# Pyrokine/LineSegmentDetector-SLAM

Measured on AMD Instinct MI355X. Metric: Mpixels/sec LSD (grad+grow+NFA), higher is better.
Workload: dtype f64; 1 GPU; 512 x 2048x2048 u8 occupancy maps per GPU tiled/rolled/flipped from 4 aisle-class fixtures (SURVEY 8d C4), full pipeline incl. lineIm, params 0.3/0.6/22.5/0.7/1024; images_total=512, images_rank0=512, parallelism=single GPU, rccl_gather_in_step=False, steps_in_flight=8, steps_in_flight_asked=8, region_waves_per_image=4, help_across_workgroups=False, last_steps_with_help=0, writeback_map=False

## Files before the change

### include/lsd_hip.h

```cpp
#ifndef LSD_HIP_H
#define LSD_HIP_H
#include <stddef.h>
#include <stdint.h>

#ifdef __cplusplus
extern "C" {
#endif

#define LSD_ABI_VERSION 1

enum {
    LSD_OK = 0,
    LSD_ERR_INVALID = 1,
    LSD_ERR_NO_DEVICE = 2,
    LSD_ERR_HIP = 3,
    LSD_ERR_UNSUPPORTED = 4,
    LSD_ERR_CAPACITY = 5,
    LSD_ERR_NOMEM = 6,
    LSD_ERR_INTERNAL = 7
};

typedef struct lsd_params {
    double sca;
    double sig;
    double angThre;
    double denThre;
    int pseBin;
} lsd_params;

typedef struct lsd_line {
    double k, b, dx, dy, x1, y1, x2, y2, len;
    int orient;
} lsd_line;

typedef struct lsd_ctx lsd_ctx;

int lsd_create(lsd_ctx **out, int device);
void lsd_destroy(lsd_ctx *ctx);
const char *lsd_strerror(int status);
const char *lsd_last_error(const lsd_ctx *ctx);
void lsd_default_params(lsd_params *p);
int lsd_abi_version(void);
void lsd_free(void *p);

int lsd_run(lsd_ctx *ctx, uint8_t *map, int cols, int rows, size_t stride, const lsd_params *p,
            uint8_t *line_im, size_t line_im_stride, lsd_line **lines_out, int *n_lines);

int lsd_run_batch(lsd_ctx *ctx, uint8_t *maps, int n, int cols, int rows, const lsd_params *p,
                  uint8_t *line_ims, lsd_line **lines_out, int *offsets_out);

int lsd_set_host_max_lines(lsd_ctx *ctx, int max_lines);

#define LSD_FLAG_WRITEBACK_MAP 1u
int lsd_enqueue_batch_device(lsd_ctx *ctx, uint8_t *d_maps, int n, int cols, int rows,
                             const lsd_params *p, unsigned flags, uint8_t *d_line_ims,
                             lsd_line *d_lines, int max_lines, int32_t *d_counts, void *stream);
int lsd_reserve(lsd_ctx *ctx, int n, int cols, int rows);
int lsd_synchronize(lsd_ctx *ctx);

void lsd_shard_range(int n_items, int world, int rank, int *lo, int *hi);
int lsd_shard_balanced(const long long *costs, int n_items, int world, int *perm);
int lsd_last_region_cycles(lsd_ctx *ctx, int n, long long *cycles_out);

int lsd_last_sensitivity(lsd_ctx *ctx, int n, int *near_ties);

typedef struct lsd_comm {
    int rank, world;
    int (*all_gather)(void *user, const void *d_send, void *d_recv, size_t bytes_per_rank, void *stream);
    void *user;
} lsd_comm;
int lsd_comm_from_rccl(void *nccl_comm, lsd_comm *out);

int lsd_gather_layout(int n_total, int world, int *per_rank, size_t *counts_words);

int lsd_gather_lines(lsd_ctx *ctx, const lsd_comm *comm, const lsd_line *d_lines, const int32_t *d_counts, int n_local, int max_lines,
                     int n_total, int cap_rows, int32_t *d_counts_all, lsd_line *d_slabs_all, void *stream);
int lsd_gather_unpack(const int32_t *counts_all, const lsd_line *slabs_all, int n_total, int world, int cap_rows, int32_t *offsets_out,
                      lsd_line *lines_out, size_t lines_cap);

int lsd_map_cache(lsd_ctx *ctx, const uint8_t *map, int cols, int rows, size_t stride, double res,
                  double z_occ_max_dis, double *out);
int lsd_enqueue_map_cache_device(lsd_ctx *ctx, const uint8_t *d_maps, int n, int cols, int rows, double res,
                                 double z_occ_max_dis, double *d_out, void *stream);

typedef struct lsd_position { double x, y, ang; } lsd_position;
typedef struct lsd_match_score { lsd_position pos; double score; } lsd_match_score;
int lsd_scan_to_map_match(lsd_ctx *ctx, const double *map_cache, int cols, int rows,
                          const lsd_line *map_lines, int n_map, const lsd_line *scan_lines, int n_scan,
                          const lsd_position *scan_im_points, int n_points, lsd_position lidar_pose, lsd_position last_pose,
                          const int *pairs, int n_pairs, double z_occ_max_dis, double max_esti_dist, lsd_match_score *out);
int lsd_enqueue_scan_to_map_match_device(lsd_ctx *ctx, const double *d_map_cache, int cols, int rows,
                                         const lsd_line *d_map_lines, const lsd_line *d_scan_lines,
                                         const lsd_position *d_scan_im_points, int n_points, lsd_position lidar_pose,
                                         lsd_position last_pose, const int *d_pairs, int n_pairs, double z_occ_max_dis,
                                         double max_esti_dist, lsd_match_score *d_out, void *stream);

typedef struct lsd_polar { double range, angle; } lsd_polar;
typedef struct lsd_map_param { int oriMapCol, oriMapRow; double mapResol, mapOriX, mapOriY; } lsd_map_param;
#define LSD_RDP_MAX_LINES 360
int lsd_feature_scan_batch(lsd_ctx *ctx, const lsd_polar *scans, const int *lens, int n_scans, int stride, lsd_map_param map_param,
                           int region_point_limit, double thre_line, double line_dist_thre_m, lsd_line *lines_out, int *n_lines,
                           lsd_position *pts_out, int pts_cap, int *n_pts, double *lidar_pos, int *im_size);
int lsd_enqueue_feature_scan_batch_device(lsd_ctx *ctx, const lsd_polar *d_scans, const int *d_lens, int n_scans, int stride,
                                          lsd_map_param map_param, int region_point_limit, double thre_line, double line_dist_thre_m,
                                          lsd_line *d_lines_out, int *d_n_lines, lsd_position *d_pts_out, int pts_cap, int *d_n_pts,
                                          double *d_lidar_pos, int *d_im_size, void *stream);

int lsd_enqueue_scan_ingest_device(lsd_ctx *ctx, const lsd_polar *d_raw, int n_scans, int n_beams, const int *d_take,
                                   lsd_polar *d_scans, int *d_lens, int stride, void *stream);
int lsd_enqueue_laserscan_ingest_device(lsd_ctx *ctx, const float *d_ranges, const float *d_angle_min_inc, int n_scans, int n_beams,
                                        const int *d_take, lsd_polar *d_scans, int *d_lens, int stride, void *stream);

typedef struct lsd_fa_state {
    double x[9];
    double P[81];
} lsd_fa_state;
enum { LSD_FA_RESET = 0, LSD_FA_FIRST = 1, LSD_FA_UKF = 2 };
typedef struct lsd_fa_report {
    lsd_position estimate;
    double score;
    lsd_position scan_pose;
    int n_pairs;
    int n_kept;
    int branch;
    int llt;
} lsd_fa_report;
void lsd_fa_initial_state(lsd_fa_state *out);
int lsd_feature_association(lsd_ctx *ctx, const double *map_cache, int cols, int rows, const lsd_line *map_lines, int n_map,
                            const lsd_line *scan_lines, int n_scan, const lsd_position *scan_im_points, int n_points,
                            lsd_position lidar_pose, lsd_position last_pose, lsd_position scan_pose, const lsd_fa_state *in,
                            lsd_fa_state *out, lsd_fa_report *report);
int lsd_enqueue_localize_device(lsd_ctx *ctx, const double *d_map_cache, int cols, int rows, const lsd_line *d_map_lines, int n_map,
                                int n_seq, int frames_pitch, const int *n_frames, const lsd_line *d_lines, const int *d_n_lines,
                                const lsd_position *d_pts, int pts_cap, const int *d_n_pts, const double *d_lidar_pos,
                                const lsd_position *d_odom, double map_resol, const lsd_fa_state *d_init, lsd_fa_state *d_states,
                                lsd_fa_report *d_reports, void *stream);
typedef struct lsd_fa_carry {
    lsd_fa_state state;
    lsd_position odom;
    double ang_sum;
    double ang_count;
    int32_t frames;
    int32_t is_offset;
} lsd_fa_carry;
void lsd_fa_carry_init(lsd_fa_carry *out, const lsd_fa_state *state, lsd_position odom0);
int lsd_enqueue_localize_resume_device(lsd_ctx *ctx, const double *d_map_cache, int cols, int rows, const lsd_line *d_map_lines,
                                       int n_map, int n_seq, int frames_pitch, const int *n_frames, const lsd_line *d_lines,
                                       const int *d_n_lines, const lsd_position *d_pts, int pts_cap, const int *d_n_pts,
                                       const double *d_lidar_pos, const lsd_position *d_odom, double map_resol, lsd_fa_carry *d_carry,
                                       lsd_fa_state *d_states, lsd_fa_report *d_reports, void *stream);
int lsd_enqueue_localize_live_map_device(lsd_ctx *ctx, const double *d_map_cache, int cols, int rows, const lsd_line *d_map_lines,
                                         int map_lines_cap, const int32_t *d_n_map, int n_seq, int frames_pitch, const int *n_frames,
                                         const lsd_line *d_lines, const int *d_n_lines, const lsd_position *d_pts, int pts_cap,
                                         const int *d_n_pts, const double *d_lidar_pos, const lsd_position *d_odom, double map_resol,
                                         const lsd_fa_state *d_init, lsd_fa_state *d_states, lsd_fa_report *d_reports, void *stream);
int lsd_enqueue_localize_resume_live_map_device(lsd_ctx *ctx, const double *d_map_cache, int cols, int rows, const lsd_line *d_map_lines,
                                                int map_lines_cap, const int32_t *d_n_map, int n_seq, int frames_pitch, const int *n_frames,
                                                const lsd_line *d_lines, const int *d_n_lines, const lsd_position *d_pts, int pts_cap,
                                                const int *d_n_pts, const double *d_lidar_pos, const lsd_position *d_odom, double map_resol,
                                                lsd_fa_carry *d_carry, lsd_fa_state *d_states, lsd_fa_report *d_reports, void *stream);
#define LSD_MAX_MAPS 64
typedef struct lsd_map_ref {
    const double   *d_map_cache;
    const lsd_line *d_map_lines;
    const int32_t  *d_n_map;
    int cols, rows, n_map;
    double mapResol, mapOriX, mapOriY;
} lsd_map_ref;
int lsd_enqueue_feature_scan_maps_device(lsd_ctx *ctx, const lsd_polar *d_scans, const int *d_lens, int n_scans, int stride,
                                         const lsd_map_ref *maps, int n_maps, const int32_t *d_map_of, int scans_per_seq,
                                         int region_point_limit, double thre_line, double line_dist_thre_m, lsd_line *d_lines_out,
                                         int *d_n_lines, lsd_position *d_pts_out, int pts_cap, int *d_n_pts, double *d_lidar_pos,
                                         int *d_im_size, void *stream);
int lsd_enqueue_localize_maps_device(lsd_ctx *ctx, const lsd_map_ref *maps, int n_maps, const int32_t *d_map_of, int n_seq,
                                     int frames_pitch, const int *n_frames, const lsd_line *d_lines, const int *d_n_lines,
                                     const lsd_position *d_pts, int pts_cap, const int *d_n_pts, const double *d_lidar_pos,
                                     const lsd_position *d_odom, const lsd_fa_state *d_init, lsd_fa_state *d_states,
                                     lsd_fa_report *d_reports, void *stream);
int lsd_enqueue_localize_resume_maps_device(lsd_ctx *ctx, const lsd_map_ref *maps, int n_maps, const int32_t *d_map_of, int n_seq,
                                            int frames_pitch, const int *n_frames, const lsd_line *d_lines, const int *d_n_lines,
                                            const lsd_position *d_pts, int pts_cap, const int *d_n_pts, const double *d_lidar_pos,
                                            const lsd_position *d_odom, lsd_fa_carry *d_carry, lsd_fa_state *d_states,
                                            lsd_fa_report *d_reports, void *stream);
typedef struct lsd_map_frame { double mapResol, mapOriX, mapOriY; } lsd_map_frame;
int lsd_enqueue_fa_carry_rebase_device(lsd_ctx *ctx, lsd_fa_carry *d_carry, int n_seq, const int32_t *d_key, int32_t key,
                                       lsd_map_frame from, lsd_map_frame to, void *stream);
int lsd_localize(lsd_ctx *ctx, const double *map_cache, int cols, int rows, const lsd_line *map_lines, int n_map, const lsd_polar *scans,
                 const int *lens, int n_frames, int stride, const lsd_position *odom, lsd_map_param map_param, const lsd_fa_state *init,
                 lsd_fa_state *states, lsd_fa_report *reports);
int lsd_debug_fa_fuse(lsd_ctx *ctx, const lsd_match_score *cands, int n, lsd_position last_pose, lsd_position scan_pose,
                      const lsd_fa_state *in, lsd_fa_state *out, lsd_fa_report *report);

int lsd_occupancy_to_map(lsd_ctx *ctx, const int8_t *grid, int cols, int rows, uint8_t *map_out, size_t map_stride);
int lsd_enqueue_occupancy_to_map_device(lsd_ctx *ctx, const int8_t *d_grid, size_t n_cells, uint8_t *d_map, void *stream);

int lsd_enqueue_map_update_device(lsd_ctx *ctx, const int8_t *d_grid, int cols, int rows, double res, double z_occ_max_dis,
                                  const lsd_params *p, uint8_t *d_map, double *d_map_cache, lsd_line *d_lines, int max_lines,
                                  int32_t *d_count, uint8_t *d_line_im, void *stream);
int lsd_reserve_map_update(lsd_ctx *ctx, int cols, int rows);

void lsd_scaled_size(int cols, int rows, double sca, int *w, int *h);

enum { LSD_STAGE_ALL = 0, LSD_STAGE_GAUSS = 1, LSD_STAGE_GRAD = 2, LSD_STAGE_SORT = 3, LSD_STAGE_REGION = 4 };
int lsd_set_stop_after(lsd_ctx *ctx, int stage);
int lsd_set_trace(lsd_ctx *ctx, int on);
int lsd_set_region_waves(lsd_ctx *ctx, int waves);
int lsd_set_region_help(lsd_ctx *ctx, int waves);
int lsd_set_cost_history(lsd_ctx *ctx, int on);
int lsd_debug_set_stamp_budget(lsd_ctx *ctx, unsigned grows);
int lsd_debug_set_tuning(lsd_ctx *ctx, const char *name, int value);

enum { LSD_DBG_GAUSS = 1, LSD_DBG_MAG, LSD_DBG_DEG, LSD_DBG_STATE, LSD_DBG_ORDER, LSD_DBG_ORDER_VAL,
       LSD_DBG_NB, LSD_DBG_MAXGRAD, LSD_DBG_RECS, LSD_DBG_SEEDS, LSD_DBG_NSEED, LSD_DBG_STATS };
int lsd_debug_fetch(lsd_ctx *ctx, int image, int what, void *out, size_t bytes);

int lsd_debug_eval_math(lsd_ctx *ctx, int fn, const double *a, const double *b, double *out0, double *out1, size_t n);

int lsd_debug_calibrate(lsd_ctx *ctx, size_t bytes);

int lsd_last_timings(lsd_ctx *ctx, float ms_out[6]);

#ifdef __cplusplus
}
#endif
#endif
```

### linesegmentdetector-slam_amd/__init__.py

```python
import ctypes as C
import os

import numpy as np

_HERE = os.path.dirname(os.path.abspath(__file__))
LIB_PATH = os.path.join(_HERE, "liblsdhip.so")

LSD_OK, LSD_ERR_INVALID, LSD_ERR_NO_DEVICE, LSD_ERR_HIP, LSD_ERR_UNSUPPORTED, LSD_ERR_CAPACITY, LSD_ERR_NOMEM, LSD_ERR_INTERNAL = range(8)
LSD_FLAG_WRITEBACK_MAP = 1
STAGE_ALL, STAGE_GAUSS, STAGE_GRAD, STAGE_SORT, STAGE_REGION = range(5)
(DBG_GAUSS, DBG_MAG, DBG_DEG, DBG_STATE, DBG_ORDER, DBG_ORDER_VAL, DBG_NB, DBG_MAXGRAD, DBG_RECS, DBG_SEEDS,
 DBG_NSEED, DBG_STATS) = range(1, 13)

lsd_sca, lsd_sig, lsd_angThre, lsd_denThre, pseBin = 0.3, 0.6, 22.5, 0.7, 1024
z_occ_max_dis = 1.0
rdp_leastPoint, rdp_threLine, rdp_leastDist = 3, 0.08, 0.5


class lsd_params(C.Structure):
    _fields_ = [("sca", C.c_double), ("sig", C.c_double), ("angThre", C.c_double), ("denThre", C.c_double),
                ("pseBin", C.c_int)]


class lsd_line(C.Structure):
    _fields_ = [(n, C.c_double) for n in ("k", "b", "dx", "dy", "x1", "y1", "x2", "y2", "len")] + [("orient", C.c_int)]


LINE_DTYPE = np.dtype([("k", "f8"), ("b", "f8"), ("dx", "f8"), ("dy", "f8"), ("x1", "f8"), ("y1", "f8"),
                       ("x2", "f8"), ("y2", "f8"), ("len", "f8"), ("orient", "i4"), ("_pad", "i4")])
SEED_DTYPE = np.dtype([("order_idx", "i4"), ("x", "i4"), ("y", "i4"), ("num", "i4"), ("outcome", "i4"),
                       ("final_num", "i4"), ("logNFA", "f8")])
assert LINE_DTYPE.itemsize == 80 == C.sizeof(lsd_line)


class lsd_map_param(C.Structure):
    _fields_ = [("oriMapCol", C.c_int), ("oriMapRow", C.c_int), ("mapResol", C.c_double), ("mapOriX", C.c_double), ("mapOriY", C.c_double)]


LSD_MAX_MAPS = 64


class lsd_map_ref(C.Structure):
    _fields_ = [("d_map_cache", C.c_void_p), ("d_map_lines", C.c_void_p), ("d_n_map", C.c_void_p), ("cols", C.c_int), ("rows", C.c_int),
                ("n_map", C.c_int), ("mapResol", C.c_double), ("mapOriX", C.c_double), ("mapOriY", C.c_double)]


MAP_REF_DTYPE = np.dtype([("d_map_cache", "u8"), ("d_map_lines", "u8"), ("d_n_map", "u8"), ("cols", "i4"), ("rows", "i4"), ("n_map", "i4"),
                          ("_pad", "i4"), ("mapResol", "f8"), ("mapOriX", "f8"), ("mapOriY", "f8")])
assert MAP_REF_DTYPE.itemsize == 64 == C.sizeof(lsd_map_ref)


class lsd_map_frame(C.Structure):
    _fields_ = [("mapResol", C.c_double), ("mapOriX", C.c_double), ("mapOriY", C.c_double)]


class lsd_position(C.Structure):
    _fields_ = [("x", C.c_double), ("y", C.c_double), ("ang", C.c_double)]


POS_DTYPE = np.dtype([("x", "f8"), ("y", "f8"), ("ang", "f8")])
SCORE_DTYPE = np.dtype([("x", "f8"), ("y", "f8"), ("ang", "f8"), ("score", "f8")])

FA_STATE_DTYPE = np.dtype([("x", "f8", (9,)), ("P", "f8", (81,))])
FA_REPORT_DTYPE = np.dtype([("estimate", POS_DTYPE), ("score", "f8"), ("scan_pose", POS_DTYPE), ("n_pairs", "i4"), ("n_kept", "i4"),
                            ("branch", "i4"), ("llt", "i4")])
assert FA_STATE_DTYPE.itemsize == 720 and FA_REPORT_DTYPE.itemsize == 72
FA_RESET, FA_FIRST, FA_UKF = range(3)
FA_CARRY_DTYPE = np.dtype([("state", FA_STATE_DTYPE), ("odom", POS_DTYPE), ("ang_sum", "f8"), ("ang_count", "f8"), ("frames", "i4"),
                           ("is_offset", "i4")])
assert FA_CARRY_DTYPE.itemsize == 768


ALL_GATHER_FN = C.CFUNCTYPE(C.c_int, C.c_void_p, C.c_void_p, C.c_void_p, C.c_size_t, C.c_void_p)


class lsd_comm(C.Structure):
    _fields_ = [("rank", C.c_int), ("world", C.c_int), ("all_gather", ALL_GATHER_FN), ("user", C.c_void_p)]


class LsdError(RuntimeError):
    def __init__(self, status, msg, partial=None):
        super().__init__("lsd_hip status %d: %s" % (status, msg))
        self.status = status
        self.partial = partial


_vp, _i, _sz, _dbl = C.c_void_p, C.c_int, C.c_size_t, C.c_double
_pi, _ppar = C.POINTER(C.c_int), C.POINTER(lsd_params)
_localize_args = [_vp, _vp, _i, _i, _vp, _i, _i, _i, _vp, _vp, _vp, _vp, _i, _vp, _vp, _vp, _dbl, _vp, _vp, _vp, _vp]
_maps_args = [_vp, _vp, _i, _vp] + _localize_args[6:16] + _localize_args[17:]
_live_map_args = _localize_args[:6] + [_vp] + _localize_args[6:]
_ABI = {
    "lsd_create": (_i, [C.POINTER(_vp), _i]),
    "lsd_destroy": (None, [_vp]),
    "lsd_strerror": (C.c_char_p, [_i]),
    "lsd_last_error": (C.c_char_p, [_vp]),
    "lsd_default_params": (None, [_ppar]),
    "lsd_abi_version": (_i, []),
    "lsd_free": (None, [_vp]),
    "lsd_run": (_i, [_vp, _vp, _i, _i, _sz, _ppar, _vp, _sz, C.POINTER(_vp), _pi]),
    "lsd_run_batch": (_i, [_vp, _vp, _i, _i, _i, _ppar, _vp, C.POINTER(_vp), _pi]),
    "lsd_enqueue_batch_device": (_i, [_vp, _vp, _i, _i, _i, _ppar, C.c_uint, _vp, _vp, _i, _vp, _vp]),
    "lsd_reserve": (_i, [_vp, _i, _i, _i]),
    "lsd_synchronize": (_i, [_vp]),
    "lsd_scaled_size": (None, [_i, _i, _dbl, _pi, _pi]),
    "lsd_set_stop_after": (_i, [_vp, _i]),
    "lsd_set_trace": (_i, [_vp, _i]),
    "lsd_set_region_waves": (_i, [_vp, _i]),
    "lsd_set_region_help": (_i, [_vp, _i]),
    "lsd_debug_set_stamp_budget": (_i, [_vp, C.c_uint]),
    "lsd_set_cost_history": (_i, [_vp, _i]),
    "lsd_debug_set_tuning": (_i, [_vp, C.c_char_p, _i]),
    "lsd_set_host_max_lines": (_i, [_vp, _i]),
    "lsd_debug_fetch": (_i, [_vp, _i, _i, _vp, _sz]),
    "lsd_last_timings": (_i, [_vp, C.POINTER(C.c_float)]),
    "lsd_map_cache": (_i, [_vp, _vp, _i, _i, _sz, _dbl, _dbl, _vp]),
    "lsd_enqueue_map_cache_device": (_i, [_vp, _vp, _i, _i, _i, _dbl, _dbl, _vp, _vp]),
    "lsd_occupancy_to_map": (_i, [_vp, _vp, _i, _i, _vp, _sz]),
    "lsd_enqueue_occupancy_to_map_device": (_i, [_vp, _vp, _sz, _vp, _vp]),
    "lsd_scan_to_map_match": (_i, [_vp, _vp, _i, _i, _vp, _i, _vp, _i, _vp, _i, lsd_position, lsd_position, _vp, _i, _dbl, _dbl, _vp]),
    "lsd_enqueue_scan_to_map_match_device": (_i, [_vp, _vp, _i, _i, _vp, _vp, _vp, _i, lsd_position, lsd_position, _vp, _i, _dbl, _dbl, _vp, _vp]),
    "lsd_feature_scan_batch": (_i, [_vp, _vp, _vp, _i, _i, lsd_map_param, _i, _dbl, _dbl, _vp, _vp, _vp, _i, _vp, _vp, _vp]),
    "lsd_enqueue_feature_scan_batch_device": (_i, [_vp, _vp, _vp, _i, _i, lsd_map_param, _i, _dbl, _dbl, _vp, _vp, _vp, _i, _vp, _vp, _vp, _vp]),
    "lsd_shard_range": (None, [_i, _i, _i, _pi, _pi]),
    "lsd_gather_layout": (_i, [_i, _i, _pi, C.POINTER(_sz)]),
    "lsd_comm_from_rccl": (_i, [_vp, C.POINTER(lsd_comm)]),
    "lsd_gather_lines": (_i, [_vp, C.POINTER(lsd_comm), _vp, _vp, _i, _i, _i, _i, _vp, _vp, _vp]),
    "lsd_gather_unpack": (_i, [_vp, _vp, _i, _i, _i, _vp, _vp, _sz]),
    "lsd_shard_balanced": (_i, [_vp, _i, _i, _vp]),
    "lsd_last_region_cycles": (_i, [_vp, _i, _vp]),
    "lsd_last_sensitivity": (_i, [_vp, _i, _vp]),
    "lsd_fa_initial_state": (None, [_vp]),
    "lsd_feature_association": (_i, [_vp, _vp, _i, _i, _vp, _i, _vp, _i, _vp, _i, lsd_position, lsd_position, lsd_position, _vp, _vp, _vp]),
    "lsd_enqueue_localize_device": (_i, _localize_args),
    "lsd_localize": (_i, [_vp, _vp, _i, _i, _vp, _i, _vp, _vp, _i, _i, _vp, lsd_map_param, _vp, _vp, _vp]),
    "lsd_debug_fa_fuse": (_i, [_vp, _vp, _i, lsd_position, lsd_position, _vp, _vp, _vp]),
    "lsd_fa_carry_init": (None, [_vp, _vp, lsd_position]),
    "lsd_enqueue_localize_resume_device": (_i, _localize_args),
    "lsd_enqueue_localize_live_map_device": (_i, _live_map_args),
    "lsd_enqueue_localize_resume_live_map_device": (_i, _live_map_args),
    "lsd_enqueue_feature_scan_maps_device": (_i, [_vp, _vp, _vp, _i, _i, _vp, _i, _vp, _i, _i, _dbl, _dbl, _vp, _vp, _vp, _i, _vp, _vp, _vp, _vp]),
    "lsd_enqueue_localize_maps_device": (_i, _maps_args),
    "lsd_enqueue_localize_resume_maps_device": (_i, _maps_args),
    "lsd_enqueue_fa_carry_rebase_device": (_i, [_vp, _vp, _i, _vp, C.c_int32, lsd_map_frame, lsd_map_frame, _vp]),
    "lsd_enqueue_map_update_device": (_i, [_vp, _vp, _i, _i, _dbl, _dbl, _ppar, _vp, _vp, _vp, _i, _vp, _vp, _vp]),
    "lsd_reserve_map_update": (_i, [_vp, _i, _i]),
    "lsd_enqueue_scan_ingest_device": (_i, [_vp, _vp, _i, _i, _vp, _vp, _vp, _i, _vp]),
    "lsd_enqueue_laserscan_ingest_device": (_i, [_vp, _vp, _vp, _i, _i, _vp, _vp, _vp, _i, _vp]),
    "lsd_debug_calibrate": (_i, [_vp, _sz]),
    "lsd_debug_eval_math": (_i, [_vp, _i, _vp, _vp, _vp, _vp, _sz]),
}
EXPORTED_SYMBOLS = list(_ABI)
del _vp, _i, _sz, _dbl, _pi, _ppar, _localize_args, _live_map_args, _maps_args

_lib = None


def load_library(path=None):
    global _lib
    if _lib is not None and path is None:
        return _lib
    p = path or os.environ.get("LSD_HIP_LIB") or LIB_PATH
    try:
        import torch
    except ImportError:
        pass
    if not os.path.exists(p):
        raise ImportError("liblsdhip.so is not built (%s); run `python -c 'import __graft_entry__ as g; g.build()'` "
                          "-- there is no CPU fallback" % p)
    L = C.CDLL(p)
    for name, (restype, argtypes) in _ABI.items():
        try:
            fn = getattr(L, name)
        except AttributeError:
            if not os.environ.get("LSD_HIP_LIB"):
                raise
            continue
        fn.restype, fn.argtypes = restype, argtypes
    if path is None:
        _lib = L
    return L


def shard_range(n_items, world, rank):
    lo, hi = C.c_int(), C.c_int()
    load_library().lsd_shard_range(n_items, world, rank, C.byref(lo), C.byref(hi))
    return lo.value, hi.value


def shard_balanced(costs, world):
    c = np.ascontiguousarray(costs, np.int64)
    perm = np.zeros(len(c), np.int32)
    st = load_library().lsd_shard_balanced(c.ctypes.data, len(c), world, perm.ctypes.data)
    if st != LSD_OK:
        raise LsdError(st, load_library().lsd_strerror(st).decode())
    return perm


def gather_layout(n_total, world):
    per, words = C.c_int(), C.c_size_t()
    st = load_library().lsd_gather_layout(n_total, world, C.byref(per), C.byref(words))
    if st != LSD_OK:
        raise LsdError(st, load_library().lsd_strerror(st).decode())
    return per.value, words.value


def gather_unpack(counts_all, slabs_all, n_total, world, cap_rows):
    L = load_library()
    ca = np.ascontiguousarray(counts_all, np.int32)
    sl = np.ascontiguousarray(slabs_all).view(np.uint8).reshape(-1, 80)
    offs = np.zeros(n_total + 1, np.int32)
    per, _ = gather_layout(n_total, world)
    total = int(ca.reshape(world, per + 2)[:, :per].sum())
    lines = np.zeros(max(total, 1), LINE_DTYPE)
    st = L.lsd_gather_unpack(ca.ctypes.data, sl.ctypes.data, n_total, world, cap_rows, offs.ctypes.data, lines.ctypes.data, len(lines))
    if st in (LSD_ERR_CAPACITY, LSD_ERR_INTERNAL):
        raise LsdError(st, L.lsd_strerror(st).decode(), partial=(offs, lines[:offs[-1]]))
    if st != LSD_OK:
        raise LsdError(st, L.lsd_strerror(st).decode())
    return offs, lines[:offs[-1]]


def make_params(sca=lsd_sca, sig=lsd_sig, angThre=lsd_angThre, denThre=lsd_denThre, pseBin=pseBin):
    return lsd_params(float(sca), float(sig), float(angThre), float(denThre), int(pseBin))


def scaled_size(cols, rows, sca=lsd_sca):
    w, h = C.c_int(), C.c_int()
    load_library().lsd_scaled_size(cols, rows, sca, C.byref(w), C.byref(h))
    return w.value, h.value


class Context:

    def __init__(self, device=0):
        self.L = load_library()
        h = C.c_void_p()
        st = self.L.lsd_create(C.byref(h), int(device))
        if st != LSD_OK:
            raise LsdError(st, self.L.lsd_strerror(st).decode())
        self.h = h
        self.device = device

    def close(self):
        if getattr(self, "h", None):
            self.L.lsd_destroy(self.h)
            self.h = None

    def __del__(self):
        try:
            self.close()
        except Exception:
            pass

    def _chk(self, st, allow=()):
        if st != LSD_OK and st not in allow:
            raise LsdError(st, self.L.lsd_strerror(st).decode() + " / " + self.L.lsd_last_error(self.h).decode())
        return st

    def _take_lines(self, lines_p, n):
        lines = np.zeros(n if lines_p else 0, LINE_DTYPE)
        if len(lines):
            C.memmove(lines.ctypes.data, lines_p, 80 * len(lines))
            lines["_pad"] = 0
        self.L.lsd_free(lines_p)
        return lines

    def run(self, map_u8, params=None, want_lineim=True):
        assert map_u8.dtype == np.uint8 and map_u8.ndim == 2
        rows, cols = map_u8.shape
        p = params or make_params()
        line_im = np.zeros((rows, cols), np.uint8) if want_lineim else None
        lines_p, n = C.c_void_p(), C.c_int()
        st = self.L.lsd_run(self.h, map_u8.ctypes.data, cols, rows, map_u8.strides[0], C.byref(p),
                            line_im.ctypes.data if want_lineim else None, cols, C.byref(lines_p), C.byref(n))
        lines = self._take_lines(lines_p, n.value)
        self._chk(st)
        return lines, line_im

    def run_batch(self, maps_u8, params=None, want_lineim=True):
        assert maps_u8.dtype == np.uint8 and maps_u8.ndim == 3 and maps_u8.flags.c_contiguous
        n, rows, cols = maps_u8.shape
        p = params or make_params()
        line_ims = np.zeros((n, rows, cols), np.uint8) if want_lineim else None
        lines_p = C.c_void_p()
        offs = (C.c_int * (n + 1))()
        st = self.L.lsd_run_batch(self.h, maps_u8.ctypes.data, n, cols, rows, C.byref(p),
                                  line_ims.ctypes.data if want_lineim else None, C.byref(lines_p), offs)
        offsets = np.frombuffer(offs, np.int32).copy()
        lines = self._take_lines(lines_p, int(offsets[-1]))
        self._chk(st)
        return lines, offsets, line_ims

    def enqueue_device(self, d_maps, n, cols, rows, d_lines, max_lines, d_counts, d_line_ims=None, params=None,
                       flags=0, stream=None):
        p = params or make_params()
        return self._chk(self.L.lsd_enqueue_batch_device(self.h, d_maps, n, cols, rows, C.byref(p), flags, d_line_ims,
                                                         d_lines, max_lines, d_counts, stream))

    def gather_lines(self, comm, d_lines, d_counts, n_local, max_lines, n_total, cap_rows, d_counts_all, d_slabs_all, stream=None):
        return self._chk(self.L.lsd_gather_lines(self.h, C.byref(comm), d_lines, d_counts, n_local, max_lines, n_total, cap_rows,
                                                 d_counts_all, d_slabs_all, stream))

    def map_cache(self, map_u8, res, z_occ_max_dis=1.0):
        assert map_u8.dtype == np.uint8 and map_u8.ndim == 2
        rows, cols = map_u8.shape
        out = np.zeros((rows, cols), np.float64)
        self._chk(self.L.lsd_map_cache(self.h, map_u8.ctypes.data, cols, rows, map_u8.strides[0], float(res),
                                       float(z_occ_max_dis), out.ctypes.data))
        return out

    def enqueue_map_cache_device(self, d_maps, n, cols, rows, res, z_occ_max_dis, d_out, stream=None):
        return self._chk(self.L.lsd_enqueue_map_cache_device(self.h, d_maps, n, cols, rows, float(res),
                                                             float(z_occ_max_dis), d_out, stream))

    def scan_to_map_match(self, map_cache, map_lines, scan_lines, scan_im_points, lidar_pose, last_pose, pairs,
                          z_occ=1.0, max_esti_dist=60.0):
        mc = np.ascontiguousarray(map_cache, np.float64)
        rows, cols = mc.shape
        ml = np.ascontiguousarray(map_lines, LINE_DTYPE); sl = np.ascontiguousarray(scan_lines, LINE_DTYPE)
        pts = np.ascontiguousarray(scan_im_points).view(np.float64).reshape(-1, 3)
        pr = np.ascontiguousarray(pairs, np.int32).reshape(-1, 2)
        out = np.zeros((len(pr), 4), SCORE_DTYPE)
        self._chk(self.L.lsd_scan_to_map_match(self.h, mc.ctypes.data, cols, rows, ml.ctypes.data, len(ml), sl.ctypes.data, len(sl),
                                               pts.ctypes.data, len(pts), _pos(lidar_pose), _pos(last_pose), pr.ctypes.data, len(pr),
                                               float(z_occ), float(max_esti_dist), out.ctypes.data))
        return out

    def feature_scan_batch(self, scans, lens, map_param, region_point_limit=rdp_leastPoint, thre_line=rdp_threLine,
                           line_dist_thre_m=rdp_leastDist, pts_cap=4096):
        sc = np.ascontiguousarray(scans, np.float64)
        n, stride = sc.shape[0], sc.shape[1]
        ln = np.ascontiguousarray(lens, np.int32)
        lines = np.zeros((n, 360), LINE_DTYPE); pts = np.zeros((n, pts_cap, 3), np.float64)
        nl = np.zeros(n, np.int32); npt = np.zeros(n, np.int32); lp = np.zeros((n, 2), np.float64); sz = np.zeros((n, 2), np.int32)
        mp = _map_param(map_param)
        st = self.L.lsd_feature_scan_batch(self.h, sc.ctypes.data, ln.ctypes.data, n, stride, mp, int(region_point_limit), float(thre_line),
                                           float(line_dist_thre_m), lines.ctypes.data, nl.ctypes.data, pts.ctypes.data, pts_cap,
                                           npt.ctypes.data, lp.ctypes.data, sz.ctypes.data)
        if st != LSD_ERR_CAPACITY:
            self._chk(st)
        out = []
        for i in range(n):
            nl[i] = min(int(nl[i]), 360)
            if npt[i] > pts_cap:
                raise RuntimeError("scan %d marks %d pixels, more than pts_cap" % (i, npt[i]))
            p = pts[i, :npt[i]].copy()
            im = np.zeros((max(int(sz[i, 1]), 0), max(int(sz[i, 0]), 0)), np.uint8)
            if len(p):
                im[p[:, 1].astype(int), p[:, 0].astype(int)] = 255
            out.append(dict(linesInfo=lines[i, :nl[i]].copy(), len_linesInfo=int(nl[i]), scanImPoint=p, lidarPos=(float(lp[i, 0]), float(lp[i, 1])),
                            lineIm=im))
        if st == LSD_ERR_CAPACITY:
            raise LsdError(st, self.L.lsd_strerror(st).decode(), partial=out)
        return out

    def enqueue_scan_ingest_device(self, d_raw, n_scans, n_beams, d_take, d_scans, d_lens, stride, stream=None):
        return self._chk(self.L.lsd_enqueue_scan_ingest_device(self.h, d_raw, int(n_scans), int(n_beams), d_take, d_scans, d_lens, int(stride),
                                                               stream))

    def enqueue_laserscan_ingest_device(self, d_ranges, d_angle_min_inc, n_scans, n_beams, d_take, d_scans, d_lens, stride, stream=None):
        return self._chk(self.L.lsd_enqueue_laserscan_ingest_device(self.h, d_ranges, d_angle_min_inc, int(n_scans), int(n_beams), d_take,
                                                                    d_scans, d_lens, int(stride), stream))

    @staticmethod
    def fa_initial_state():
        st = np.zeros(1, FA_STATE_DTYPE)
        load_library().lsd_fa_initial_state(st.ctypes.data)
        return st[0]

    def feature_association(self, map_cache, map_lines, scan_lines, scan_im_points, lidar_pose, last_pose, scan_pose, state):
        mc = np.ascontiguousarray(map_cache, np.float64)
        rows, cols = mc.shape
        ml, sl = np.ascontiguousarray(map_lines, LINE_DTYPE), np.ascontiguousarray(scan_lines, LINE_DTYPE)
        pts = np.ascontiguousarray(scan_im_points, np.float64).reshape(-1, 3)
        st_in = fa_state(state)
        st_out = np.zeros(1, FA_STATE_DTYPE); rep = np.zeros(1, FA_REPORT_DTYPE)
        self._chk(self.L.lsd_feature_association(self.h, mc.ctypes.data, cols, rows, ml.ctypes.data, len(ml), sl.ctypes.data, len(sl),
                                                 pts.ctypes.data, len(pts), _pos(lidar_pose), _pos(last_pose), _pos(scan_pose),
                                                 st_in.ctypes.data, st_out.ctypes.data, rep.ctypes.data))
        return st_out[0], rep[0]

    def debug_fa_fuse(self, cands, last_pose, scan_pose, state):
        cd = np.ascontiguousarray(np.asarray(cands, np.float64).reshape(-1, 4))
        st_in = fa_state(state)
        st_out = np.zeros(1, FA_STATE_DTYPE); rep = np.zeros(1, FA_REPORT_DTYPE)
        self._chk(self.L.lsd_debug_fa_fuse(self.h, cd.ctypes.data, len(cd), _pos(last_pose), _pos(scan_pose), st_in.ctypes.data,
                                           st_out.ctypes.data, rep.ctypes.data))
        return st_out[0], rep[0]

    def localize(self, map_cache, map_lines, scans, lens, odom, map_param, init=None):
        mc = np.ascontiguousarray(map_cache, np.float64)
        rows, cols = mc.shape
        ml = np.ascontiguousarray(map_lines, LINE_DTYPE)
        sc = np.ascontiguousarray(scans, np.float64)
        n, stride = sc.shape[0], sc.shape[1]
        ln = np.ascontiguousarray(lens, np.int32)
        od = np.ascontiguousarray(odom, np.float64).reshape(-1, 3)
        if len(od) != n + 1:
            raise LsdError(LSD_ERR_INVALID, "odom must have one row more than there are frames")
        mp = _map_param(map_param)
        ini = None if init is None else fa_state(init)
        states = np.zeros(n, FA_STATE_DTYPE); reps = np.zeros(n, FA_REPORT_DTYPE)
        self._chk(self.L.lsd_localize(self.h, mc.ctypes.data, cols, rows, ml.ctypes.data, len(ml), sc.ctypes.data, ln.ctypes.data, n, stride,
                                      od.ctypes.data, mp, None if ini is None else ini.ctypes.data, states.ctypes.data, reps.ctypes.data))
        return states, reps

    def enqueue_localize_device(self, d_map_cache, cols, rows, d_map_lines, n_map, n_seq, frames_pitch, n_frames, d_lines, d_n_lines, d_pts,
                                pts_cap, d_n_pts, d_lidar_pos, d_odom, map_resol, d_init, d_states, d_reports, stream=None):
        nf = np.ascontiguousarray(n_frames, np.int32)
        return self._chk(self.L.lsd_enqueue_localize_device(self.h, d_map_cache, cols, rows, d_map_lines, n_map, n_seq, frames_pitch,
                                                            nf.ctypes.data, d_lines, d_n_lines, d_pts, pts_cap, d_n_pts, d_lidar_pos, d_odom,
                                                            float(map_resol), d_init, d_states, d_reports, stream))

    @staticmethod
    def fa_carry_init(state=None, odom0=(0.0, 0.0, 0.0)):
        c = np.zeros(1, FA_CARRY_DTYPE)
        st = None if state is None else fa_state(state)
        load_library().lsd_fa_carry_init(c.ctypes.data, None if st is None else st.ctypes.data, _pos(odom0))
        return c[0]

    def enqueue_localize_resume_device(self, d_map_cache, cols, rows, d_map_lines, n_map, n_seq, frames_pitch, n_frames, d_lines, d_n_lines,
                                       d_pts, pts_cap, d_n_pts, d_lidar_pos, d_odom, map_resol, d_carry, d_states, d_reports, stream=None):
        nf = np.ascontiguousarray(n_frames, np.int32)
        return self._chk(self.L.lsd_enqueue_localize_resume_device(self.h, d_map_cache, cols, rows, d_map_lines, n_map, n_seq, frames_pitch,
                                                                   nf.ctypes.data, d_lines, d_n_lines, d_pts, pts_cap, d_n_pts, d_lidar_pos,
                                                                   d_odom, float(map_resol), d_carry, d_states, d_reports, stream))

    def enqueue_localize_live_map_device(self, d_map_cache, cols, rows, d_map_lines, map_lines_cap, d_n_map, n_seq, frames_pitch, n_frames,
                                         d_lines, d_n_lines, d_pts, pts_cap, d_n_pts, d_lidar_pos, d_odom, map_resol, d_init, d_states,
                                         d_reports, stream=None):
        nf = np.ascontiguousarray(n_frames, np.int32)
        return self._chk(self.L.lsd_enqueue_localize_live_map_device(self.h, d_map_cache, cols, rows, d_map_lines, map_lines_cap, d_n_map,
                                                                     n_seq, frames_pitch, nf.ctypes.data, d_lines, d_n_lines, d_pts, pts_cap,
                                                                     d_n_pts, d_lidar_pos, d_odom, float(map_resol), d_init, d_states,
                                                                     d_reports, stream))

    def enqueue_localize_resume_live_map_device(self, d_map_cache, cols, rows, d_map_lines, map_lines_cap, d_n_map, n_seq, frames_pitch,
                                                n_frames, d_lines, d_n_lines, d_pts, pts_cap, d_n_pts, d_lidar_pos, d_odom, map_resol,
                                                d_carry, d_states, d_reports, stream=None):
        nf = np.ascontiguousarray(n_frames, np.int32)
        return self._chk(self.L.lsd_enqueue_localize_resume_live_map_device(self.h, d_map_cache, cols, rows, d_map_lines, map_lines_cap,
                                                                            d_n_map, n_seq, frames_pitch, nf.ctypes.data, d_lines, d_n_lines,
                                                                            d_pts, pts_cap, d_n_pts, d_lidar_pos, d_odom, float(map_resol),
                                                                            d_carry, d_states, d_reports, stream))

    def enqueue_feature_scan_maps_device(self, d_scans, d_lens, n_scans, stride, maps, d_map_of, scans_per_seq, d_lines_out, d_n_lines,
                                         d_pts_out, pts_cap, d_n_pts, d_lidar_pos, d_im_size, region_point_limit=rdp_leastPoint,
                                         thre_line=rdp_threLine, line_dist_thre_m=rdp_leastDist, stream=None):
        tab = map_table(maps)
        return self._chk(self.L.lsd_enqueue_feature_scan_maps_device(self.h, d_scans, d_lens, int(n_scans), int(stride), tab.ctypes.data,
                                                                     len(tab), d_map_of, int(scans_per_seq), int(region_point_limit),
                                                                     float(thre_line), float(line_dist_thre_m), d_lines_out, d_n_lines,
                                                                     d_pts_out, int(pts_cap), d_n_pts, d_lidar_pos, d_im_size, stream))

    def enqueue_localize_maps_device(self, maps, d_map_of, n_seq, frames_pitch, n_frames, d_lines, d_n_lines, d_pts, pts_cap, d_n_pts,
                                     d_lidar_pos, d_odom, d_init, d_states, d_reports, stream=None):
        tab, nf = map_table(maps), np.ascontiguousarray(n_frames, np.int32)
        return self._chk(self.L.lsd_enqueue_localize_maps_device(self.h, tab.ctypes.data, len(tab), d_map_of, int(n_seq), int(frames_pitch),
                                                                 nf.ctypes.data, d_lines, d_n_lines, d_pts, int(pts_cap), d_n_pts, d_lidar_pos,
                                                                 d_odom, d_init, d_states, d_reports, stream))

    def enqueue_localize_resume_maps_device(self, maps, d_map_of, n_seq, frames_pitch, n_frames, d_lines, d_n_lines, d_pts, pts_cap, d_n_pts,
                                            d_lidar_pos, d_odom, d_carry, d_states, d_reports, stream=None):
        tab, nf = map_table(maps), np.ascontiguousarray(n_frames, np.int32)
        return self._chk(self.L.lsd_enqueue_localize_resume_maps_device(self.h, tab.ctypes.data, len(tab), d_map_of, int(n_seq),
                                                                        int(frames_pitch), nf.ctypes.data, d_lines, d_n_lines, d_pts,
                                                                        int(pts_cap), d_n_pts, d_lidar_pos, d_odom, d_carry, d_states,
                                                                        d_reports, stream))

    def enqueue_fa_carry_rebase_device(self, d_carry, n_seq, d_key, key, frame_from, frame_to, stream=None):
        f, t = map_frame(frame_from), map_frame(frame_to)
        if not d_carry or int(n_seq) <= 0:
            raise LsdError(LSD_ERR_INVALID, "a null carry, or n_seq <= 0")
        return self._chk(self.L.lsd_enqueue_fa_carry_rebase_device(self.h, d_carry, int(n_seq), d_key, int(key), f, t, stream))

    def enqueue_map_update_device(self, d_grid, cols, rows, res, z_occ_max_dis, d_map, d_map_cache, d_lines, max_lines, d_count,
                                  d_line_im=None, params=None, stream=None):
        p = params or make_params()
        return self._chk(self.L.lsd_enqueue_map_update_device(self.h, d_grid, cols, rows, float(res), float(z_occ_max_dis), C.byref(p), d_map,
                                                              d_map_cache, d_lines, max_lines, d_count, d_line_im, stream))

    def reserve_map_update(self, cols, rows):
        self._chk(self.L.lsd_reserve_map_update(self.h, cols, rows))

    def occupancy_to_map(self, grid_i8):
        assert grid_i8.dtype == np.int8 and grid_i8.ndim == 2 and grid_i8.flags.c_contiguous
        rows, cols = grid_i8.shape
        out = np.zeros((rows, cols), np.uint8)
        self._chk(self.L.lsd_occupancy_to_map(self.h, grid_i8.ctypes.data, cols, rows, out.ctypes.data, out.strides[0]))
        return out

    def enqueue_occupancy_to_map_device(self, d_grid, n_cells, d_map, stream=None):
        return self._chk(self.L.lsd_enqueue_occupancy_to_map_device(self.h, d_grid, n_cells, d_map, stream))

    def reserve(self, n, cols, rows):
        self._chk(self.L.lsd_reserve(self.h, n, cols, rows))

    def synchronize(self):
        self._chk(self.L.lsd_synchronize(self.h))

    def fetch_stats_block(self, n):
        a = np.zeros((n, 48), np.int64)
        self._chk(self.L.lsd_debug_fetch(self.h, 0, DBG_STATS, a.ctypes.data, a.nbytes))
        return a

    def last_region_cycles(self, n):
        a = np.zeros(n, np.int64)
        self._chk(self.L.lsd_last_region_cycles(self.h, n, a.ctypes.data))
        return a

    def last_sensitivity(self, n):
        a = np.zeros(n, np.int32)
        self._chk(self.L.lsd_last_sensitivity(self.h, n, a.ctypes.data))
        return a

    def timings(self):
        ms = (C.c_float * 6)()
        self._chk(self.L.lsd_last_timings(self.h, ms))
        return dict(zip(("gauss", "gradient", "sort", "region", "lines", "total"), [float(x) for x in ms]))

    def set_stop_after(self, stage):
        self._chk(self.L.lsd_set_stop_after(self.h, stage))

    def set_trace(self, on):
        self._chk(self.L.lsd_set_trace(self.h, 1 if on else 0))

    def set_host_max_lines(self, max_lines):
        self._chk(self.L.lsd_set_host_max_lines(self.h, max_lines))

    def set_cost_history(self, on):
        self._chk(self.L.lsd_set_cost_history(self.h, 1 if on else 0))

    def debug_set_tuning(self, name, value):
        self._chk(self.L.lsd_debug_set_tuning(self.h, name.encode(), int(value)))

    def debug_set_stamp_budget(self, grows):
        self._chk(self.L.lsd_debug_set_stamp_budget(self.h, grows))

    def set_region_waves(self, waves):
        self._chk(self.L.lsd_set_region_waves(self.h, waves))

    def set_region_help(self, waves):
        self._chk(self.L.lsd_set_region_help(self.h, waves))

    def fetch(self, image, what, shape_wh):
        w, h = shape_wh
        npx = w * h

        def get(kind, dtype, count):
            a = np.zeros(max(count, 1), dtype)
            self._chk(self.L.lsd_debug_fetch(self.h, image, kind, a.ctypes.data, a.nbytes))
            return a[:count]

        if what in (DBG_GAUSS, DBG_MAG, DBG_DEG):
            return get(what, np.float64, npx).reshape(h, w)
        if what == DBG_STATE:
            return get(what, np.uint32, npx).reshape(h, w)
        if what == DBG_NB:
            return int(get(what, np.int32, 1)[0])
        if what == DBG_NSEED:
            return int(get(what, np.int32, 1)[0])
        if what == DBG_MAXGRAD:
            return float(get(what, np.float64, 1)[0])
        if what == DBG_ORDER:
            return get(what, np.uint32, npx)[:self.fetch(image, DBG_NB, shape_wh)]
        if what == DBG_ORDER_VAL:
            return get(what, np.uint16, npx)[:self.fetch(image, DBG_NB, shape_wh)]
        if what == DBG_STATS:
            v = get(what, np.int64, 48)
            d = dict(zip(("grow_calls", "grown_px", "nfa_calls", "rrr_calls", "rrr_passes", "rrr_sentinel_drops",
                          "rrr_oob_reads", "cycles_refill", "cycles_total", "cycles_grow", "cycles_rect",
                          "cycles_nfa", "cycles_mark", "small_bails", "wait_noslot", "seeds", "exact_angle_evals",
                          "tile_fetches", "batches", "cycles_tiles", "spec_redos", "spec_discards", "cycles_wait", "small_steps",
                          "refill_rounds", "cycles_eval", "cycles_sums", "cycles_refine", "cycles_small", "cycles_select", "cycles_commit",
                          "wait_noseed", "requeued_ahead", "cycles_eval_at_cursor", "depth_end", "nfa_min_abs_enc", "nfa_min_gap_enc", "help_exports", "help_evals", "near_ties",
                          "wd_commit", "wd_next", "wd_nseeds", "wd_state", "wd_nbig", "wd_lock", "wd_pend", "wd_wave"),
                         [int(x) for x in v]))
            d["set_answers"], d["sets_founded"] = int(v[41]), int(v[42])
            d["cycles_nfa_count"], d["nfa_tail_iters"] = int(v[43]), int(v[44])
            d["nfa_bracket_misses"] = int(v[40])
            for k in ("nfa_min_abs", "nfa_min_gap"):
                enc = d.pop(k + "_enc")
                d[k] = float("inf") if enc == 0 else float(np.array([0x7ff0000000000000 - enc], np.uint64).view(np.float64)[0])
            return d
        if what == DBG_SEEDS:
            ns = self.fetch(image, DBG_NSEED, shape_wh)
            return get(what, SEED_DTYPE, ns)
        raise ValueError(what)

    def eval_math(self, fn, a, b=None):
        a = np.ascontiguousarray(a, np.float64)
        b = None if b is None else np.ascontiguousarray(b, np.float64)
        o0, o1 = np.zeros_like(a), np.zeros_like(a)
        self._chk(self.L.lsd_debug_eval_math(self.h, fn, a.ctypes.data, None if b is None else b.ctypes.data,
                                             o0.ctypes.data, o1.ctypes.data, a.size))
        return o0, o1

    def fetch_recs(self, image, count):
        a = np.zeros(max(count * 12, 1), np.float64)
        self._chk(self.L.lsd_debug_fetch(self.h, image, DBG_RECS, a.ctypes.data, a.nbytes))
        return a[:count * 12].reshape(count, 12)


class structLSD:

    def __init__(self, lineIm, linesInfo):
        self.lineIm = lineIm
        self.linesInfo = linesInfo
        self.len_linesInfo = len(linesInfo)


_default_ctx = None


def default_context():
    global _default_ctx
    if _default_ctx is None:
        _default_ctx = Context(0)
    return _default_ctx


def myLineSegmentDetector(MapGray, oriMapCol, oriMapRow, sca, sig, angThre, denThre, pseBin, ctx=None):
    if MapGray.shape != (oriMapRow, oriMapCol):
        raise LsdError(LSD_ERR_INVALID, "MapGray must be oriMapRow x oriMapCol")
    ctx = ctx or default_context()
    lines, line_im = ctx.run(MapGray, make_params(sca, sig, angThre, denThre, pseBin))
    return structLSD(line_im, lines)


def createMapCache(MapGray, res, ctx=None):
    return (ctx or default_context()).map_cache(MapGray, res, z_occ_max_dis)


ignoreScanLength, scanToMapDiff, maxEstiDist = 40, 0.35, 60


def match_pairs(map_lines, scan_lines):
    pairs = []
    for cs in range(len(scan_lines)):
        ls = float(scan_lines["len"][cs])
        if ls < ignoreScanLength:
            continue
        ld = ls * scanToMapDiff
        for cm in range(len(map_lines)):
            lm = float(map_lines["len"][cm])
            if lm < ls - ld or lm > ls + ld:
                continue
            pairs.append((cm, cs))
    return np.array(pairs, np.int32).reshape(-1, 2)


def FeatureScan(mapParam, lidarPointPolar, RegionPointLimitNumber=rdp_leastPoint, threLine=rdp_threLine, lineDistThreM=rdp_leastDist, ctx=None):
    own = ctx is None
    ctx = ctx or Context(0)
    try:
        sc = np.ascontiguousarray(lidarPointPolar, np.float64).reshape(1, -1, 2)
        return ctx.feature_scan_batch(sc, [sc.shape[1]], mapParam, RegionPointLimitNumber, threLine, lineDistThreM)[0]
    finally:
        if own:
            ctx.close()


def ScanToMapMatch(mapCache, mapLinesInfo, scanLinesInfo, scanImPoint, lidarPose, lastPose, ctx=None):
    pairs = match_pairs(mapLinesInfo, scanLinesInfo)
    if len(pairs) == 0:
        return np.zeros(0, SCORE_DTYPE)
    sc = (ctx or default_context()).scan_to_map_match(mapCache, mapLinesInfo, scanLinesInfo, scanImPoint, lidarPose, lastPose, pairs,
                                                      z_occ_max_dis, maxEstiDist).ravel()
    keep = sc[sc["score"] < 3]
    return keep[np.argsort(keep["score"], kind="stable")]


def _pos(p):
    return lsd_position(float(p[0]), float(p[1]), float(p[2]) if len(p) > 2 else 0.0)


def _map_param(mp):
    return lsd_map_param(int(mp[0]), int(mp[1]), float(mp[2]), float(mp[3]), float(mp[4]))


def map_frame(frame):
    if isinstance(frame, lsd_map_frame):
        v = (frame.mapResol, frame.mapOriX, frame.mapOriY)
    else:
        v = tuple(float(x) for x in frame)
        if len(v) == 5:
            v = v[2:]
    if len(v) != 3:
        raise LsdError(LSD_ERR_INVALID, "a map frame is (mapResol, mapOriX, mapOriY)")
    if not (np.isfinite(v[0]) and v[0] > 0 and np.isfinite(v[1]) and np.isfinite(v[2])):
        raise LsdError(LSD_ERR_INVALID, "a map frame needs a finite mapResol > 0 and a finite origin, not %r" % (v,))
    return lsd_map_frame(*v)


def map_ref(d_map_cache, cols, rows, d_map_lines, n_map, map_param, d_n_map=0):
    r = np.zeros(1, MAP_REF_DTYPE)[0]
    r["d_map_cache"], r["d_map_lines"], r["d_n_map"] = int(d_map_cache or 0), int(d_map_lines or 0), int(d_n_map or 0)
    r["cols"], r["rows"], r["n_map"] = int(cols), int(rows), int(n_map)
    r["mapResol"], r["mapOriX"], r["mapOriY"] = float(map_param[2]), float(map_param[3]), float(map_param[4])
    return r


def map_table(maps):
    if isinstance(maps, np.ndarray) and maps.dtype == MAP_REF_DTYPE:
        return np.ascontiguousarray(maps).reshape(-1)
    return np.array(list(maps), MAP_REF_DTYPE).reshape(-1)


def fa_state(state):
    if isinstance(state, np.void) or (isinstance(state, np.ndarray) and state.dtype == FA_STATE_DTYPE):
        return np.ascontiguousarray(np.asarray(state, FA_STATE_DTYPE).reshape(1))
    x, P = state
    st = np.zeros(1, FA_STATE_DTYPE)
    st["x"][0] = np.asarray(x, np.float64).reshape(9)
    st["P"][0] = np.asarray(P, np.float64).reshape(9, 9).ravel(order="F")
    return st


def load_odom(path_or_rows):
    rows = np.loadtxt(path_or_rows).reshape(-1, 3) if isinstance(path_or_rows, str) else np.asarray(path_or_rows, np.float64).reshape(-1, 3)
    od = np.concatenate([rows, rows[-1:]], 0)
    od[0, 0] = 0.0
    return od


def lidar_frames(lidar):
    lid = np.asarray(lidar, np.float64)
    scans = np.zeros_like(lid)
    lens = np.zeros(len(lid), np.int32)
    for f in range(len(lid)):
        keep = lid[f][lid[f, :, 0] != np.inf]
        scans[f, :len(keep)] = keep
        lens[f] = len(keep)
    return scans, lens


def FeatureAssociation(mapCache, mapLinesInfo, scanLinesInfo, scanImPoint, lidarPose, lastPose, kalman_x, kalman_P, ScanPose, ctx=None):
    st, rep = (ctx or default_context()).feature_association(mapCache, mapLinesInfo, scanLinesInfo, scanImPoint, lidarPose, lastPose, ScanPose,
                                                             (kalman_x, kalman_P))
    return st["x"].copy(), st["P"].reshape(9, 9, order="F").copy(), rep


def replay_log(map_u8, map_param, lidar, odom, ctx=None):
    cx = ctx or default_context()
    m = np.ascontiguousarray(map_u8, np.uint8).copy()
    mapCache = cx.map_cache(m, float(map_param[2]), z_occ_max_dis)
    LSD = myLineSegmentDetector(m, m.shape[1], m.shape[0], lsd_sca, lsd_sig, lsd_angThre, lsd_denThre, pseBin, ctx=cx)
    scans, lens = lidar_frames(lidar)
    return cx.localize(mapCache, LSD.linesInfo, scans, lens, odom, map_param)


def lidar_frames_batch(lidar):
    lid = np.asarray(lidar, np.float64)
    keep = lid[..., 0] != np.inf
    order = np.argsort(~keep, axis=-1, kind="stable")
    scans = np.take_along_axis(lid, order[..., None], axis=-2)
    lens = keep.sum(-1).astype(np.int32)
    scans[np.arange(lid.shape[-2]) >= lens[..., None]] = 0.0
    return scans, lens


def _cuda_stream(stream):
    import torch
    if stream is None:
        return torch.cuda.current_stream()
    if not isinstance(stream, torch.cuda.Stream):
        raise LsdError(LSD_ERR_INVALID, "stream must be a torch.cuda.Stream (or None: the current stream)")
    return stream


def _occupancy_grid(d_grid, cols, rows, device):
    import torch
    if not isinstance(d_grid, torch.Tensor) or not d_grid.is_cuda or d_grid.dtype != torch.int8:
        raise LsdError(LSD_ERR_INVALID, "d_grid must be a CUDA int8 tensor")
    if d_grid.device.index != int(device):
        raise LsdError(LSD_ERR_INVALID, "d_grid is on cuda:%d, the context on device %d" % (d_grid.device.index, int(device)))
    if cols <= 0 or rows <= 0 or tuple(d_grid.shape) not in ((rows * cols,), (rows, cols)):
        raise LsdError(LSD_ERR_INVALID, "d_grid must hold oriMapRow x oriMapCol cells, flat or [rows, cols]")
    return d_grid.contiguous()


class _MapSlot:

    def __init__(self):
        self.cells = self.cap_lines = 0
        self.map = self.mc = self.lines = self.count = None
        self.cols = self.rows = 0
        self.lines_cap = 0
        self.n_host = None
        self.map_param = None
        self.grid = None
        self.ready = None
        self.waited = set()
        self.last_stream = None
        self.idle = None


class _MapPair:

    def __init__(self):
        self.slots, self.cur = (_MapSlot(), _MapSlot()), 1

    @property
    def current(self):
        return self.slots[self.cur]

    @staticmethod
    def fit(slot, cells, n_lines, keep=False):
        import torch
        if slot.cells >= cells and slot.cap_lines >= n_lines:
            return
        for ev in (slot.idle, slot.ready):
            if ev is not None:
                ev.synchronize()
        if slot.last_stream is not None:
            slot.last_stream.synchronize()
        cells, n_lines = max(cells, slot.cells), max(n_lines, slot.cap_lines)
        z = lambda count, dt: torch.zeros(count, dtype=dt, device="cuda")
        new = (z(cells, torch.uint8), z(cells, torch.float64), z(n_lines * 80, torch.uint8), z(1, torch.int32))
        if keep and slot.cells:
            for dst, src in zip(new, (slot.map, slot.mc, slot.lines, slot.count)):
                dst[:src.numel()].copy_(src)
        torch.cuda.current_stream().synchronize()
        slot.map, slot.mc, slot.lines, slot.count = new
        slot.cells, slot.cap_lines = cells, n_lines

    def target(self, stream, cells, n_lines):
        slot = self.slots[1 - self.cur]
# ... 577 lines not shown
```

### linesegmentdetector-slam_amd/csrc/k_gauss.hip

```cpp
#include "lsd_internal.h"
#include "k1_lds.h"
#include <algorithm>

namespace lsdhip {

constexpr int TW = kK1TileW, TH = kK1TileH, NT = 256;

__device__ __forceinline__ int reflect_idx(int j, int lim) {
    const int dou = 2 * lim;
    while (j < 0) j += dou;
    while (j >= dou) j -= dou;
    if (j >= lim) j = dou - j - 1;
    return j;
}


template <int HS>
__global__ __launch_bounds__(NT) void k_gauss(const uint8_t* __restrict__ in, double* __restrict__ out,
                                              const double* __restrict__ taps_g, const int* __restrict__ centre_of, int W, int H, int w, int h, int gp,
                                              int tapR, int IWp, int IHmax, unsigned gx, unsigned gy, unsigned tiles,
                                              uint8_t* __restrict__ clr) {
    extern __shared__ __align__(16) unsigned char smem[];
    const int hSize = HS > 0 ? HS : 2 * tapR + 1;
    double* aux = reinterpret_cast<double*>(smem);
    double* taps = aux + (size_t)IHmax * TW;
    uint8_t* tile = reinterpret_cast<uint8_t*>(taps + 3 * hSize);

    const int tid = threadIdx.x;
    const unsigned per = (tiles + 7u) >> 3;
    const unsigned t = (blockIdx.x & 7u) * per + (blockIdx.x >> 3);
    if (t >= tiles) return;
    const unsigned bx = t % gx, tq = t / gx, by = tq % gy;
    const int X0 = (int)bx * TW, Y0 = (int)by * TH;
    const size_t img = tq / gy;
    const uint8_t* src = in + img * (size_t)W * H;
    double* dst = out + img * (size_t)gp * h;

    if (clr) {
        typedef uint32_t u32x4 __attribute__((ext_vector_type(4)));
        const unsigned tpi = gx * gy, ti = t % tpi;
        const size_t units = ((size_t)W * H) >> 4;
        const size_t a = units * ti / tpi, e = units * (ti + 1) / tpi;
        u32x4* const v = reinterpret_cast<u32x4*>(clr + img * (size_t)W * H);
        const u32x4 z = {0u, 0u, 0u, 0u};
        for (size_t u = a + tid; u < e; u += NT) __builtin_nontemporal_store(z, &v[u]);
    }
    const int Xl = min(X0 + TW - 1, w - 1), Yl = min(Y0 + TH - 1, h - 1);
    const int c0 = centre_of[X0] - tapR, c1 = centre_of[Xl] + tapR;
    const int r0 = centre_of[Y0] - tapR, r1 = centre_of[Yl] + tapR;
    const int IH = r1 - r0 + 1;

    for (int i = tid; i < 3 * hSize; i += NT) taps[i] = taps_g[i];

    const int a0 = c0 - (((c0 % 4) + 4) % 4);
    auto remap4 = [](uint32_t x, uint32_t keep) -> uint32_t {
        uint32_t t1 = x ^ 0x01010101u, t2 = ~x;
        t1 = ~(((t1 & 0x7f7f7f7fu) + 0x7f7f7f7fu) | t1 | 0x7f7f7f7fu);
        t2 = ~(((t2 & 0x7f7f7f7fu) + 0x7f7f7f7fu) | t2 | 0x7f7f7f7fu);
        const uint32_t m1 = (t1 | (t1 - (t1 >> 7))) & ~keep, m255 = (t2 | (t2 - (t2 >> 7))) & ~keep;
        return (x | m1) & ~m255;
    };
    uint32_t wany = 0u;
    {
        const int DW = (c1 - a0 + 4) >> 2;
        uint32_t* tile32 = reinterpret_cast<uint32_t*>(tile);
        const int DWp = IWp >> 2;
        const int tx = tid & 31, ty = tid >> 5;
        const bool plain = a0 >= 4 && a0 + 4 * DW <= W && r0 >= 1 && r1 < H && (W & 3) == 0 && (reinterpret_cast<uintptr_t>(src) & 3) == 0;
        if (plain) {
            const int nfull = IH >> 3, tail = IH & 7;
            const uint8_t* const sb = src + (size_t)r0 * W + a0;
            for (int cw = tx; cw < DW; cw += 32) {
                const uint32_t voff = (uint32_t)ty * (uint32_t)W + 4u * (uint32_t)cw;
                uint32_t* const t0 = tile32 + ty * DWp + cw;
                for (int g0 = 0; g0 < nfull; g0 += 16) {
                    uint32_t v[16];
                    #pragma unroll
                    for (int j = 0; j < 16; j++) {
                        v[j] = 0u;
                        if (g0 + j < nfull) v[j] = *reinterpret_cast<const uint32_t*>(sb + (size_t)(g0 + j) * 8u * (size_t)W + voff);
                    }
                    #pragma unroll
                    for (int j = 0; j < 16; j++) {
                        if (g0 + j < nfull) { const uint32_t rm = __ballot(v[j] + 1u > 1u) != 0ull ? remap4(v[j], 0u) : 0u; t0[(g0 + j) * 8 * DWp] = rm; wany |= rm; }
                    }
                }
                if (ty < tail) { const uint32_t rm = remap4(*reinterpret_cast<const uint32_t*>(sb + (size_t)nfull * 8u * (size_t)W + voff), 0u); t0[nfull * 8 * DWp] = rm; wany |= rm; }
            }
        } else
        for (int cw = tx; cw < DW; cw += 32) {
            const int gx0 = a0 + 4 * cw;
            const bool fast_col = gx0 >= 0 && gx0 + 3 < W;
            int gxr[4];
            uint32_t colkeep = 0u;
            #pragma unroll
            for (int k2 = 0; k2 < 4; k2++) {
                gxr[k2] = reflect_idx(gx0 + k2, W);
                if (gxr[k2] == 0) colkeep |= 0xffu << (8 * k2);
            }
            for (int rb = 0; rb < IH; rb += 8 * 16) {
                uint32_t v[16];
                #pragma unroll
                for (int j = 0; j < 16; j++) {
                    const int r = rb + ty + 8 * j;
                    v[j] = 0u;
                    if (r < IH) {
                        const int gy = reflect_idx(r0 + r, H);
                        const size_t off = (size_t)gy * W + gx0;
                        if (fast_col && (off & 3) == 0) v[j] = *reinterpret_cast<const uint32_t*>(src + off);
                        else {
                            const uint8_t* row = src + (size_t)gy * W;
                            v[j] = (uint32_t)row[gxr[0]] | ((uint32_t)row[gxr[1]] << 8) | ((uint32_t)row[gxr[2]] << 16) | ((uint32_t)row[gxr[3]] << 24);
                        }
                    }
                }
                #pragma unroll
                for (int j = 0; j < 16; j++) {
                    const int r = rb + ty + 8 * j;
                    if (r < IH) {
                        const uint32_t x = v[j];
                        const uint32_t rm = x != 0u ? remap4(x, reflect_idx(r0 + r, H) == 0 ? 0xffffffffu : colkeep) : 0u;
                        tile32[r * DWp + cw] = rm; wany |= rm;
                    }
                }
            }
        }
    }
    const int X = tid & (TW - 1);
    const int gX = X0 + X;
    if (!__syncthreads_or((int)(wany != 0u))) {
        if (gX < w)
            for (int Y = tid / TW; Y < TH && Y0 + Y < h; Y += NT / TW) dst[(size_t)(Y0 + Y) * gp + gX] = 0.0;
        return;
    }
    {
        const int cb = (gX < w ? centre_of[gX] : 0) - tapR - a0;
        const double* ker = taps + (gX % 3) * hSize;
        if (gX < w) {
            if (HS > 0) {
                static_assert(HS <= 17, "the x-pass reads 5 words = 17 bytes at any byte offset");
                double kr[HS > 0 ? HS : 1];
                #pragma unroll
                for (int i = 0; i < HS; i++) kr[i] = ker[i];
                const uint32_t* trow = reinterpret_cast<const uint32_t*>(tile) + (cb >> 2);
                const uint32_t sh = (uint32_t)(cb & 3);
                const int DWp = IWp >> 2;
                for (int r = tid / TW; r < IH; r += NT / TW) {
                    const uint32_t* t4 = trow + r * DWp;
                    const uint32_t d0 = t4[0], d1 = t4[1], d2 = t4[2], d3 = t4[3], d4 = t4[4];
                    if (__ballot((d0 | d1 | d2 | d3 | d4) != 0u) == 0ull) { aux[r * TW + X] = 0.0; continue; }
                    uint32_t wv[5];
                    wv[0] = __builtin_amdgcn_alignbyte(d1, d0, sh); wv[1] = __builtin_amdgcn_alignbyte(d2, d1, sh);
                    wv[2] = __builtin_amdgcn_alignbyte(d3, d2, sh); wv[3] = __builtin_amdgcn_alignbyte(d4, d3, sh);
                    wv[4] = d4 >> (8u * sh);
                    double v = 0;
                    #pragma unroll
                    for (int i = 0; i < HS; i++) v += (double)(int)((wv[i >> 2] >> (8 * (i & 3))) & 0xffu) * kr[i];

                    aux[r * TW + X] = v;
                }
            } else {
                for (int r = tid / TW; r < IH; r += NT / TW) {
                    const uint8_t* t = tile + r * IWp + cb;
                    double v = 0;
                    for (int i = 0; i < hSize; i++) v += (double)(int)t[i] * ker[i];
                    aux[r * TW + X] = v;
                }
            }
        }
    }
    __syncthreads();

    if (gX < w) {
        for (int Y = tid / TW; Y < TH; Y += NT / TW) {
            const int gY = Y0 + Y;
            if (gY >= h) break;
            const int rb = centre_of[gY] - tapR - r0;
            const double* ker = taps + (gY % 3) * hSize;
            double v = 0;
            if (HS > 0) {
                double a[HS > 0 ? HS : 1];
                uint32_t bits = 0u;
                #pragma unroll
                for (int i = 0; i < HS; i++) { a[i] = aux[(rb + i) * TW + X]; bits |= (uint32_t)__double2hiint(a[i]) | (uint32_t)__double2loint(a[i]); }
                if (__ballot(bits != 0u) != 0ull) {
                    #pragma unroll
                    for (int i = 0; i < HS; i++) v += a[i] * ker[i];
                }
            } else {
                for (int i = 0; i < hSize; i++) v += aux[(rb + i) * TW + X] * ker[i];
            }
            dst[(size_t)gY * gp + gX] = v;
        }
    }
}

__device__ __forceinline__ uint32_t remap_word(uint32_t x, uint32_t keep) {
    uint32_t t1 = x ^ 0x01010101u, t2 = ~x;
    t1 = ~(((t1 & 0x7f7f7f7fu) + 0x7f7f7f7fu) | t1 | 0x7f7f7f7fu);
    t2 = ~(((t2 & 0x7f7f7f7fu) + 0x7f7f7f7fu) | t2 | 0x7f7f7f7fu);
    const uint32_t m1 = (t1 | (t1 - (t1 >> 7))) & ~keep, m255 = (t2 | (t2 - (t2 >> 7))) & ~keep;
    return (x | m1) & ~m255;
}
__global__ __launch_bounds__(256) void k_remap_inplace16(uint8_t* __restrict__ img, uint32_t W, uint32_t H, size_t units) {
    typedef uint32_t u32x4 __attribute__((ext_vector_type(4)));
    u32x4* const v = reinterpret_cast<u32x4*>(img);
    const uint32_t upr = W >> 4;
    const size_t stride = (size_t)gridDim.x * blockDim.x;
    for (size_t u = (size_t)blockIdx.x * blockDim.x + threadIdx.x; u < units; u += stride) {
        const u32x4 x = v[u];
        if ((x.x | x.y | x.z | x.w) == 0u) continue;
        const uint32_t row = (uint32_t)(u / upr), col = (uint32_t)(u - (size_t)row * upr);
        if (row % H == 0u) continue;
        u32x4 r;
        r.x = remap_word(x.x, col == 0u ? 0xffu : 0u);
        r.y = remap_word(x.y, 0u); r.z = remap_word(x.z, 0u); r.w = remap_word(x.w, 0u);
        if ((r.x ^ x.x) | (r.y ^ x.y) | (r.z ^ x.z) | (r.w ^ x.w)) v[u] = r;
    }
}
__global__ __launch_bounds__(256) void k_remap_inplace(uint8_t* __restrict__ img, int W, int H, size_t total) {
    size_t i = (size_t)blockIdx.x * blockDim.x + threadIdx.x;
    const size_t stride = (size_t)gridDim.x * blockDim.x;
    const size_t per = (size_t)W * H;
    for (; i < total; i += stride) {
        const size_t p = i % per;
        const int y = (int)(p / W), x = (int)(p % W);
        if (y >= 1 && x >= 1) {
            uint8_t v = img[i];
            if (v == 1) img[i] = 255; else if (v == 255) img[i] = 0;
        }
    }
}

static auto gauss_kernel(const Geom& g) { return 2 * g.tapR + 1 == 17 ? k_gauss<17> : k_gauss<0>; }

hipError_t prepare_gauss(const Geom& g) {
    const K1Lds L = k1_lds(g.sca, g.tapR);
    if (L.bytes <= 64 * 1024) return hipSuccess;
    return hipFuncSetAttribute(reinterpret_cast<const void*>(gauss_kernel(g)), hipFuncAttributeMaxDynamicSharedMemorySize, (int)L.bytes);
}

void launch_gauss(const Geom& g, const Buffers& b, int n, uint8_t* clr, hipStream_t s) {
    const K1Lds L = k1_lds(g.sca, g.tapR);
    const unsigned gx = (g.w + TW - 1) / TW, gy = (g.h + TH - 1) / TH, tiles = gx * gy * (unsigned)n;
    hipLaunchKernelGGL(gauss_kernel(g), dim3(((tiles + 7u) >> 3) * 8u), dim3(NT), L.bytes, s, b.in, b.gauss, b.taps, b.centres, g.W, g.H, g.w, g.h, g.gp,
                       g.tapR, L.IWp, L.IHmax, gx, gy, tiles, clr);
}

void launch_remap_writeback(const Geom& g, const Buffers& b, int n, hipStream_t s) {
    if (!b.in_rw) return;
    const size_t total = (size_t)n * g.W * g.H;
    if ((g.W & 15) == 0 && (reinterpret_cast<uintptr_t>(b.in_rw) & 15) == 0) {
        const size_t units = total >> 4;
        const int blocks = (int)std::min<size_t>((units + 255) / 256, 16384);
        hipLaunchKernelGGL(k_remap_inplace16, dim3(blocks), dim3(256), 0, s, b.in_rw, (uint32_t)g.W, (uint32_t)g.H, units);
        return;
    }
    int blocks = (int)((total + 255) / 256);
    if (blocks > 8192) blocks = 8192;
    hipLaunchKernelGGL(k_remap_inplace, dim3(blocks), dim3(256), 0, s, b.in_rw, g.W, g.H, total);
}

}
```

### linesegmentdetector-slam_amd/csrc/k_grad.hip

```cpp
#include "lsd_internal.h"
#include "devmath.h"

namespace lsdhip {

constexpr int GX = 64;
constexpr int GR = 8;

__device__ __forceinline__ uint32_t pack_pw(double d, uint32_t code) {
    return (__float_as_uint(__double2float_rn(d)) & ~3u) | code;
}

constexpr int CAP = 256;

__global__ __launch_bounds__(GX) void k_gradient(const double* __restrict__ gauss, double* __restrict__ mag,
                                                 double* __restrict__ deg, double2* __restrict__ sc,
                                                 uint32_t* __restrict__ pw,
                                                 unsigned long long* __restrict__ maxbits, int32_t* __restrict__ ties, int w, int h, int gp,
                                                 double gradThre, unsigned gx, unsigned gy, unsigned strips) {
    __shared__ uint32_t l_px[CAP];
    __shared__ double2 l_g[CAP];
    const unsigned per = (strips + 7u) >> 3;
    const unsigned t = (blockIdx.x & 7u) * per + (blockIdx.x >> 3);
    if (t >= strips) return;
    const unsigned bx = t % gx, tq = t / gx, by = tq % gy;
    const size_t img = tq / gy;
    const size_t base = img * (size_t)w * h;
    const double* __restrict__ gim = gauss + img * (size_t)gp * h;
    const int lane = threadIdx.x;
    const int x = (int)bx * GX + lane, y0 = (int)by * GR;
    const bool colok = x < w;
    const unsigned long long ltmask = (1ull << lane) - 1ull;
    int cnt = 0;
    double mx = 0;
    double rowD[GR];
    uint32_t rowU[GR];
    int rowSlot[GR];

    auto flush = [&]() {
        for (int i = lane; i < cnt; i += GX) {
            const uint32_t e = l_px[i];
            const double2 gr = l_g[i];
            double d;
            if (!crm::atan2_fast(gr.x, -gr.y, d)) d = atan2_g(gr.x, -gr.y);
            if (fabs(fabs(d - kPi) - 0.000001) <= 1e-14) atomicAdd(&ties[img], 1);
            if (fabs(d - kPi) < 0.000001) d = 0;
            l_g[i] = make_double2(d, 0.0);
            if (e & 1u) {
                const int lt = (int)(e >> 1);
                const size_t p = base + (size_t)(y0 + lt / GX) * w + ((int)bx * GX + lt % GX);
                double sv, cv;
                if (!crm::sincos_fast(d, sv, cv)) sincos_g(d, sv, cv);
                sc[p] = make_double2(sv, cv);
            }
        }
        #pragma unroll
        for (int r = 0; r < GR; r++)
            if (rowSlot[r] >= 0) { rowD[r] = l_g[rowSlot[r]].x; rowSlot[r] = -1; }
        cnt = 0;
    };

    double up = 0, upl = 0;
    if (y0 >= 1 && colok) {
        up = gim[(size_t)(y0 - 1) * gp + x];
        if (lane == 0 && x >= 1) upl = gim[(size_t)(y0 - 1) * gp + x - 1];
    }
    {
        const double t = __shfl_up(up, 1);
        if (lane != 0) upl = t;
    }
    double rowA[GR], rowB0[GR];
    #pragma unroll
    for (int r = 0; r < GR; r++) {
        const int y = y0 + r;
        rowA[r] = 0; rowB0[r] = 0;
        if (colok && y < h) {
            rowA[r] = gim[(size_t)y * gp + x];
            if (lane == 0 && x >= 1) rowB0[r] = gim[(size_t)y * gp + x - 1];
        }
    }
    #pragma unroll
    for (int r = 0; r < GR; r++) {
        const int y = y0 + r;
        rowD[r] = 0; rowU[r] = 0; rowSlot[r] = -1;
        if (y >= h) continue;
        const double A = rowA[r];
        double B = rowB0[r];
        {
            const double t = __shfl_up(A, 1);
            if (lane != 0) B = t;
        }
        const double C = up, D = upl;
        double m = 0, d = 0, gradX = 0, gradY = 0;
        uint32_t u = 0;
        bool heavy = false;
        if (colok && x >= 1 && y >= 1) {
            gradX = (B + D - A - C) / 2.0;
            gradY = (C + D - A - B) / 2.0;
            m = sqrt(gradX * gradX + gradY * gradY);
            if (m < gradThre) u = 1;
            if (gradX == 0.0 && gradY == 0.0) {
                if (signbit(-gradY)) d = signbit(gradX) ? -kPi : 0.0;
                else d = gradX;
            } else heavy = true;
        }
        if (colok) {
            const size_t p = base + (size_t)y * w + x;
            mag[p] = m;
            if (!heavy && u == 0) sc[p] = make_double2(0.0, 1.0);
        }
        rowD[r] = d; rowU[r] = u;
        const unsigned long long hm = __ballot(heavy);
        if (heavy) {
            const int slot = cnt + __builtin_popcountll(hm & ltmask);
            l_px[slot] = ((uint32_t)(r * GX + lane) << 1) | (u == 0 ? 1u : 0u);
            l_g[slot] = make_double2(gradX, gradY);
            rowSlot[r] = slot;
        }
        cnt += __builtin_popcountll(hm);
        mx = fmax(mx, m);
        up = A; upl = B;
        if (cnt > CAP - GX) flush();
    }
    unsigned long long bits = (unsigned long long)__double_as_longlong(mx);
    for (int off = 32; off >= 1; off >>= 1) {
        unsigned long long o = __shfl_xor(bits, off);
        bits = o > bits ? o : bits;
    }
    if (lane == 0 && bits != 0ull) atomicMax(&maxbits[img], bits);

    flush();
    if (colok) {
        #pragma unroll
        for (int r = 0; r < GR; r++) {
            const int y = y0 + r;
            if (y < h) {
                const size_t p = base + (size_t)y * w + x;
                deg[p] = rowD[r];
                pw[p] = pack_pw(rowD[r], rowU[r]);
            }
        }
    }
}

void launch_gradient(const Geom& g, const Buffers& b, int n, hipStream_t s) {
    const unsigned gx = (g.w + GX - 1) / GX, gy = (g.h + GR - 1) / GR, strips = gx * gy * (unsigned)n;
    hipLaunchKernelGGL(k_gradient, dim3(((strips + 7u) >> 3) * 8u), dim3(GX), 0, s, b.gauss, b.mag, b.deg, b.sc, b.pw, b.maxbits, b.ties,
                       g.w, g.h, g.gp, g.gradThre, gx, gy, strips);
}

}
```

### linesegmentdetector-slam_amd/csrc/lsd_ctx.hip

```cpp
#include <math.h>
#include <stddef.h>
#include <stdio.h>
#include <stdlib.h>
#include <string.h>

#include <algorithm>
#include <mutex>
#include <string>
#include <vector>

#include "lsd_devbuf.h"
#include "lsd_internal.h"
#include "k1_lds.h"

using namespace lsdhip;

struct Workspace {
    size_t cap_gpx = 0;
    size_t cap_n = 0, cap_npx = 0, cap_ws = 0;
    int cap_max_lines = 0;
    DevBuf<double> gauss, mag, deg, recs, recs_scaled;
    DevBuf<double2> sc;
    DevBuf<uint32_t> order;
    DevBuf<uint32_t> sets;
    DevBuf<uint32_t> pw, epochmap, ord, spill, gcopy, stamps, seedidx, seedpos, tepoch;
    uint32_t run_id = 0;
    DevBuf<uint32_t> slist;
    DevBuf<double> pend;
    DevBuf<float4> wmeta;
    DevBuf<int> rnum;
    DevBuf<uint32_t> xq;
    DevBuf<unsigned long long> maxbits;
    DevBuf<int32_t> nb, nseed;
    DevBuf<long long> stats;
    DevBuf<SeedRec> seeds;
    int32_t* ties() const { return reinterpret_cast<int32_t*>(maxbits.get() + cap_n); }
};

struct lsd_ctx {
    int device = 0;
    int num_cus = 256;
    size_t max_lds = 0;
    uint32_t id_budget = 0xFFFF0u;
    int tun_soft = 0, tun_claim = 0, tun_feed = 3, tun_big = 0;
    int tun_help = -1;
    int tun_gate = 12000;
    int tun_share = 0;
    int pool_max_images = 4;
    int tun_early = 0, tun_wb = 10, tun_up = 32, tun_down = 96, tun_requeue = 1, tun_xpoll = 20000, tun_linger = 1000000, tun_stop = 0;
    int region_waves_mode = 0;
    bool prefer4 = false;
    hipStream_t stream = nullptr;
    hipStream_t last_stream = nullptr;
    std::string err;
    Workspace ws;
    int mcap = 16384;
    int gcap = 8192;
    DevBuf<uint8_t> h_in, h_lineim;
    DevBuf<lsd_line> h_lines, h_flat;
    DevBuf<int32_t> h_counts, h_offs;
    uint8_t* pin[2] = {nullptr, nullptr};
    hipEvent_t pin_ev[2] = {nullptr, nullptr};
    bool pin_used[2] = {false, false};
    hipStream_t copy_stream = nullptr;
    size_t hcap_n = 0, hcap_wh = 0;
    int hcap_max_lines = 0;
    bool hcap_lineim = false;
    DevBuf<double> d_taps, d_lgamma, d_ptab;
    DevBuf<int> d_centres;
    bool cost_history = false;
    int hist_n = 0;
    lsd_params tab_params{};
    bool tab_valid = false;
    int tapR = 0;
    DevBuf<unsigned long long> mc_claim;
    DevBuf<uint32_t> mc_fa, mc_fb;
    DevBuf<int> mc_ctl;
    DevBuf<uint8_t> mc_in;
    DevBuf<double> mc_out;
    DevBuf<uint8_t> oc_in, oc_out;
    DevBuf<uint8_t> stage;
    DevBuf<uint8_t> fa_buf;
    std::vector<int> fa_nf;
    std::vector<lsd_map_ref> map_tab_host = std::vector<lsd_map_ref>(2 * LSD_MAX_MAPS);
    DevBuf<lsd_map_ref> map_tab;
    int fa_lds_bound = kFaLdsMax;
    DevBuf<int32_t> ga_cnt;
    DevBuf<lsd_line> ga_slab;
    hipEvent_t ga_ev = nullptr;
    bool ga_ev_valid = false;
    int stop_after = 0;
    int tun_groups = -1;
    DevBuf<int> pcount;
    bool trace = false;
    int host_max_lines = 8192;
    Geom geom{};
    int last_n = 0;
    int last_max_lines = 0;
    int32_t* last_counts = nullptr;
    hipEvent_t ev[7]{};
    bool ev_valid = false;
    hipEvent_t ev_done = nullptr;
    bool done_valid = false;
    hipStream_t done_stream = nullptr;
};

constexpr size_t kPinBytes = 32u << 20;

#define HIPCHK(ctx, call)                                                                         \
    do {                                                                                          \
        hipError_t e_ = (call);                                                                   \
        if (e_ != hipSuccess) {                                                                   \
            (ctx)->err = std::string(#call) + ": " + hipGetErrorString(e_);                       \
            return e_ == hipErrorOutOfMemory ? LSD_ERR_NOMEM : LSD_ERR_HIP;                       \
        }                                                                                         \
    } while (0)

static int tap_radius(double sca, double sig) {
    const int prec = 3;
    if (sca < 1) sig = sig / sca;
    return cvt_x86(ceil(sig * sqrt(2 * prec * log(10))));
}

static void gauss_taps(double sca, double sig, int h, std::vector<double>& t) {
    if (sca < 1) sig = sig / sca;
    const int hSize = 1 + 2 * h;
    t.assign((size_t)3 * hSize, 0.0);
    double s1 = 0, s2 = 0, s3 = 0;
    for (int k = 0; k < hSize; k++) {
        const double a = (k - h) / sig, b = (k - h - 1.0 / 3) / sig, c = (k - h + 1.0 / 3) / sig;
        t[0 * hSize + k] = exp(-0.5 * (a * a));
        t[1 * hSize + k] = exp(-0.5 * (b * b));
        t[2 * hSize + k] = exp(-0.5 * (c * c));
        s1 += t[0 * hSize + k]; s2 += t[1 * hSize + k]; s3 += t[2 * hSize + k];
    }
    for (int k = 0; k < hSize; k++) {
        t[0 * hSize + k] /= s1; t[1 * hSize + k] /= s2; t[2 * hSize + k] /= s3;
    }
}

static double log_gamma_host(int x) {
    if (x > 15)
        return 0.918938533204673 + (x - 0.5) * log(x) - x + 0.5 * x * log(x * sinh(1.0 / x) + 1.0 / (810 * pow(x, 6)));
    static const double q[7] = {75122.6331530, 80916.6278952, 36308.2951477, 8687.24529705,
                                1168.92649479, 83.8676043424, 2.50662827511};
    double a = (x + 0.5) * log(x + 5.5) - (x + 5.5), b = 0;
    for (int i = 0; i < 7; i++) { a -= log(x + i); b += q[i] * pow(x, i); }
    return a + log(b);
}

static std::mutex g_lg_mu;
static const double* log_gamma_table(int count) {
    static std::vector<double> tab;
    if ((int)tab.size() < count) {
        const int from = (int)tab.size();
        tab.resize(count);
        for (int i = from; i < count; i++) tab[i] = i >= 1 ? log_gamma_host(i) : 0.0;
    }
    return tab.data();
}

static int make_geom(lsd_ctx* c, const lsd_params* p, int cols, int rows, Geom* g) {
    if (!p || cols <= 0 || rows <= 0) return LSD_ERR_INVALID;
    if (!(p->sca > 0) || !(p->sig > 0) || !(p->angThre > 0) || p->pseBin < 1) return LSD_ERR_INVALID;
    if (p->pseBin > 1024) return LSD_ERR_UNSUPPORTED;
    if (cols > 65535 || rows > 65535) return LSD_ERR_UNSUPPORTED;
    g->W = cols; g->H = rows;
    g->w = cvt_x86(floor(cols * p->sca));
    g->h = cvt_x86(floor(rows * p->sca));
    if (g->w < 2 || g->h < 2) return LSD_ERR_INVALID;
    if (g->w > 32766 || g->h > 32766) return LSD_ERR_UNSUPPORTED;
    if ((long long)g->w * g->h > (1ll << 30)) return LSD_ERR_UNSUPPORTED;
    g->npx = g->w * g->h;
    g->gp = (g->w + 15) & ~15;
    g->sca = p->sca;
    g->tapR = tap_radius(p->sca, p->sig);
    if (g->tapR < 0 || g->tapR > kMaxTapRadius) return LSD_ERR_UNSUPPORTED;
    const size_t k1_bytes = k1_lds(p->sca, g->tapR).bytes;
    if (k1_bytes > c->max_lds) {
        char msg[200];
        snprintf(msg, sizeof msg, "sca = %g, sig = %g: the Gaussian's window needs %zu bytes of LDS per workgroup, the device has %zu",
                 p->sca, p->sig, k1_bytes, c->max_lds);
        c->err = msg;
        return LSD_ERR_UNSUPPORTED;
    }
    g->pseBin = p->pseBin;
    g->degThre = p->angThre / 180.0 * kPi;
    g->gradThre = 2.0 / sin(g->degThre);
    g->logNT = 5 * (log10(g->h) + log10(g->w)) / 2.0;
    g->regThre = -g->logNT / log10(p->angThre / 180.0);
    g->aliPro = p->angThre / 180.0;
    g->denThre = p->denThre;
    return LSD_OK;
}

static int ensure_tables(lsd_ctx* c, const lsd_params* p, const Geom& g, hipStream_t s) {
    const int lg_need = (int)std::min<long long>(std::max<long long>((long long)g.npx + 2, kLgTable), kLgTableMax);
    if ((int)c->d_lgamma.capacity() < lg_need) {
        HIPCHK(c, hipStreamSynchronize(s));
        if (c->done_valid) HIPCHK(c, hipEventSynchronize(c->ev_done));
        std::lock_guard<std::mutex> lk(g_lg_mu);
        const double* tab = log_gamma_table(lg_need);
        HIPCHK(c, c->d_lgamma.resize(lg_need));
        const hipError_t e = hipMemcpy(c->d_lgamma.get(), tab, sizeof(double) * lg_need, hipMemcpyHostToDevice);
        if (e != hipSuccess) (void)c->d_lgamma.resize(0);
        HIPCHK(c, e);
    }
    if (c->tab_valid && memcmp(&c->tab_params, p, sizeof(lsd_params)) == 0) return LSD_OK;
    if (!c->d_ptab.get()) {
        HIPCHK(c, c->d_ptab.resize(kPTable * 3));
        HIPCHK(c, c->d_taps.resize(3 * (2 * kMaxTapRadius + 1)));
        HIPCHK(c, c->d_centres.resize(kCentreCount));
    }
    std::vector<double> taps;
    gauss_taps(p->sca, p->sig, g.tapR, taps);
    std::vector<int> centres(kCentreCount);
    for (int x = 0; x < kCentreCount; x++) centres[x] = cvt_x86(floor(x / p->sca + 0.5));
    double pt[kPTable * 3];
    double pr = g.aliPro;
    for (int k = 0; k < kPTable; k++) {
        pt[k * 3 + 0] = log(pr); pt[k * 3 + 1] = log10(pr); pt[k * 3 + 2] = log(1 - pr);
        pr /= 2.0;
    }
    HIPCHK(c, hipStreamSynchronize(s));
    if (c->done_valid) HIPCHK(c, hipEventSynchronize(c->ev_done));
    HIPCHK(c, hipMemcpy(c->d_taps.get(), taps.data(), sizeof(double) * taps.size(), hipMemcpyHostToDevice));
    HIPCHK(c, hipMemcpy(c->d_ptab.get(), pt, sizeof(pt), hipMemcpyHostToDevice));
    HIPCHK(c, hipMemcpy(c->d_centres.get(), centres.data(), sizeof(int) * kCentreCount, hipMemcpyHostToDevice));
    c->tab_params = *p;
    c->tab_valid = true;
    c->tapR = g.tapR;
    return LSD_OK;
}

static int waves_for(const lsd_ctx* c, int n) {
    if (c->region_waves_mode == 8 || (c->region_waves_mode == 0 && !c->prefer4 && n <= 4 * c->num_cus)) return 8;
    return 4;
}

constexpr int kPoolHelpMax = 64;
static int pool_for(const lsd_ctx* c, int n, int help) {
    if (help < 0) help = 24;
    if (help > kPoolHelpMax) help = kPoolHelpMax;
    if (help <= 0 || c->trace || n > c->pool_max_images) return 0;
    const int nw = waves_for(c, n);
    const long long free_slots = (long long)(nw == 8 ? 1 : 3) * c->num_cus - n;
    const long long want = ((long long)n * help + nw - 1) / nw;
    const long long p = free_slots < want ? free_slots : want;
    return p > 0 ? (int)p : 0;
}
static int pool_for(const lsd_ctx* c, int n) { return pool_for(c, n, c->tun_help); }
static int pool_reserve_for(const lsd_ctx* c, int n) {
    const int now = c->tun_help < 0 ? 24 : c->tun_help;
    return pool_for(c, n, now > 24 ? now : 24);
}

static size_t tm_words(size_t npx) { return npx / 16 + 4 * 8200; }

static int ensure_workspace_impl(lsd_ctx* c, size_t n, size_t npx, size_t gpx, int max_lines, bool trace) {
    Workspace& w = c->ws;
    const size_t need_ws = (n + (size_t)pool_reserve_for(c, (int)n)) * (size_t)waves_for(c, (int)n);
    const bool grow_main = n > w.cap_n || npx > w.cap_npx || gpx > w.cap_gpx || need_ws > w.cap_ws;
    if (grow_main) {
        const size_t nn = n > w.cap_n ? n : w.cap_n, pp = npx > w.cap_npx ? npx : w.cap_npx;
        const size_t gg = gpx > w.cap_gpx ? gpx : w.cap_gpx;
        const size_t ws = need_ws > w.cap_ws ? need_ws : w.cap_ws;
        HIPCHK(c, hipDeviceSynchronize());
        const size_t tot = nn * pp;
        HIPCHK(c, w.gauss.resize(nn * gg)); HIPCHK(c, w.mag.resize(tot)); HIPCHK(c, w.deg.resize(tot));
        HIPCHK(c, w.sc.resize(tot));
        HIPCHK(c, w.pw.resize(tot)); HIPCHK(c, w.epochmap.resize(tot)); HIPCHK(c, w.ord.resize(tot));
        HIPCHK(c, w.spill.resize(ws * pp)); HIPCHK(c, w.gcopy.resize(ws * pp)); HIPCHK(c, w.wmeta.resize(ws * (size_t)c->mcap));
        HIPCHK(c, w.stamps.resize(ws * tm_words(pp))); HIPCHK(c, w.seedidx.resize(tot)); HIPCHK(c, w.seedpos.resize(tot)); HIPCHK(c, w.tepoch.resize(nn * (pp / 16 + 4096)));
        HIPCHK(c, hipMemset(w.stamps.get(), 0, ws * tm_words(pp) * sizeof(uint32_t)));
        HIPCHK(c, hipMemset(w.epochmap.get(), 0, tot * sizeof(uint32_t)));
        w.run_id = 0;
        const size_t gs = ws * (size_t)region_slots();
        HIPCHK(c, w.slist.resize(gs * (size_t)c->gcap));
        HIPCHK(c, w.pend.resize(gs * 24));
        HIPCHK(c, w.order.resize(nn));
        HIPCHK(c, w.sets.resize(nn * 256));
        HIPCHK(c, w.xq.resize(nn * (size_t)(kXStride + 1) + kXHdr));
        HIPCHK(c, w.maxbits.resize(nn + (nn + 1) / 2)); HIPCHK(c, w.nb.resize(nn)); HIPCHK(c, w.nseed.resize(nn));
        HIPCHK(c, w.stats.resize(nn * kStatWords)); HIPCHK(c, w.rnum.resize(nn * (size_t)region_ring() * 2));
        HIPCHK(c, w.seeds.resize(0));
        if (nn != w.cap_n) { w.cap_max_lines = 0; }
        w.cap_n = nn; w.cap_npx = pp; w.cap_gpx = gg; w.cap_ws = ws;
    }
    if (max_lines > w.cap_max_lines) {
        HIPCHK(c, hipDeviceSynchronize());
        HIPCHK(c, w.recs.resize(w.cap_n * (size_t)max_lines * 12));
        HIPCHK(c, w.recs_scaled.resize(w.cap_n * (size_t)max_lines * 4));
        w.cap_max_lines = max_lines;
    }
    if (trace && !w.seeds.get()) {
        HIPCHK(c, hipDeviceSynchronize());
        HIPCHK(c, w.seeds.resize(w.cap_n * w.cap_npx));
    }
    return LSD_OK;
}

static int ensure_workspace(lsd_ctx* c, size_t n, size_t npx, size_t gpx, int max_lines, bool trace) {
    int st = ensure_workspace_impl(c, n, npx, gpx, max_lines, trace);
    if (st != LSD_OK) {
        (void)hipGetLastError();
        c->ws = Workspace{};
        if (st == LSD_ERR_NOMEM && c->region_waves_mode == 0 && !c->prefer4 && waves_for(c, (int)n) == 8) {
            c->prefer4 = true;
            return ensure_workspace(c, n, npx, gpx, max_lines, trace);
        }
    }
    return st;
}

struct Tuning { const char* name; int lo, hi; int lsd_ctx::*field; bool shipped; };
static const Tuning kTunings[] = {
    {"HELP", -1, 4096, &lsd_ctx::tun_help, true},
    {"POOL", 0, 16, &lsd_ctx::pool_max_images, true},
    {"SOFT", 0, 1 << 20, &lsd_ctx::tun_soft, false},
    {"CLAIM", 0, 1 << 20, &lsd_ctx::tun_claim, false},
    {"FEED", 1, 8, &lsd_ctx::tun_feed, false},
    {"BIG", 0, 16, &lsd_ctx::tun_big, false},
    {"EARLY", 0, 4096, &lsd_ctx::tun_early, false},
    {"WB", 0, 100, &lsd_ctx::tun_wb, false},
    {"GATE", 0, 1 << 22, &lsd_ctx::tun_gate, false},
    {"SHARE", 0, 100, &lsd_ctx::tun_share, false},
    {"UP", 0, 1 << 16, &lsd_ctx::tun_up, false},
    {"DOWN", 0, 1 << 16, &lsd_ctx::tun_down, false},
    {"REQUEUE", 0, 1, &lsd_ctx::tun_requeue, false},
    {"XPOLL", 100, 1 << 30, &lsd_ctx::tun_xpoll, false},
    {"LINGER", 1, 1 << 30, &lsd_ctx::tun_linger, false},
    {"GROUPS", -1, 1 << 20, &lsd_ctx::tun_groups, false},
    {"STOP", 0, 1 << 30, &lsd_ctx::tun_stop, false},
    {"FA_LDS", 0, kFaLdsMax, &lsd_ctx::fa_lds_bound, false},
};

extern "C" {

int lsd_abi_version(void) { return LSD_ABI_VERSION; }

const char* lsd_strerror(int st) {
    switch (st) {
        case LSD_OK: return "ok";
        case LSD_ERR_INVALID: return "invalid argument";
        case LSD_ERR_NO_DEVICE: return "no usable HIP device (this library has no CPU fallback)";
        case LSD_ERR_HIP: return "HIP runtime error";
        case LSD_ERR_UNSUPPORTED: return "parameter outside the implemented range";
        case LSD_ERR_CAPACITY: return "line capacity exceeded";
        case LSD_ERR_NOMEM: return "out of memory (host or device)";
        case LSD_ERR_INTERNAL: return "the region stage gave an image up (its watchdog; see lsd_last_error)";
        default: return "unknown status";
    }
}

void lsd_default_params(lsd_params* p) {
    if (!p) return;
    p->sca = 0.3; p->sig = 0.6; p->angThre = 22.5; p->denThre = 0.7; p->pseBin = 1024;
}

void lsd_scaled_size(int cols, int rows, double sca, int* w, int* h) {
    if (w) *w = cvt_x86(floor(cols * sca));
    if (h) *h = cvt_x86(floor(rows * sca));
}

int lsd_create(lsd_ctx** out, int device) {
    if (!out) return LSD_ERR_INVALID;
    *out = nullptr;
    int ndev = 0;
    if (hipGetDeviceCount(&ndev) != hipSuccess || ndev <= 0) return LSD_ERR_NO_DEVICE;
    if (device < 0 || device >= ndev) return LSD_ERR_NO_DEVICE;
    if (hipSetDevice(device) != hipSuccess) return LSD_ERR_NO_DEVICE;
    lsd_ctx* c = new (std::nothrow) lsd_ctx();
    if (!c) return LSD_ERR_NOMEM;
    c->device = device;
    {
        int cus = 0;
        if (hipDeviceGetAttribute(&cus, hipDeviceAttributeMultiprocessorCount, device) == hipSuccess && cus > 0) c->num_cus = cus;
    }
    {
        int lds = 0;
        if (hipDeviceGetAttribute(&lds, hipDeviceAttributeMaxSharedMemoryPerBlock, device) != hipSuccess || lds <= 0) { delete c; return LSD_ERR_HIP; }
        c->max_lds = (size_t)lds;
    }
    if (hipStreamCreateWithFlags(&c->stream, hipStreamNonBlocking) != hipSuccess) { delete c; return LSD_ERR_HIP; }
    for (auto& e : c->ev)
        if (hipEventCreate(&e) != hipSuccess) { delete c; return LSD_ERR_HIP; }
    if (hipEventCreateWithFlags(&c->ev_done, hipEventDisableTiming) != hipSuccess) { delete c; return LSD_ERR_HIP; }
    if (hipStreamCreateWithFlags(&c->copy_stream, hipStreamNonBlocking) != hipSuccess) { delete c; return LSD_ERR_HIP; }
    for (int k = 0; k < 2; k++)
        if (hipHostMalloc((void**)&c->pin[k], kPinBytes, hipHostMallocDefault) != hipSuccess ||
            hipEventCreateWithFlags(&c->pin_ev[k], hipEventDisableTiming) != hipSuccess) { delete c; return LSD_ERR_NOMEM; }
    c->last_stream = c->stream;
    for (const Tuning& t : kTunings) {
        const std::string name = std::string("LSD_REGION_") + t.name;
        const char* e = getenv(name.c_str());
        if (!e || !*e) continue;
#ifndef LSD_DEVELOPER_KNOBS
        if (!t.shipped) {
            static bool warned = false;
            if (!warned) fprintf(stderr, "liblsdhip: %s is set but only read by the developer builds (make stats / exp, LSD_HIP_LIB=...); "
                                         "use lsd_debug_set_tuning() with the shipped library\n", name.c_str());
            warned = true;
            continue;
        }
#endif
        char* end = nullptr;
        const long v = strtol(e, &end, 10);
        if (end == e) continue;
        c->*(t.field) = (int)(v < t.lo ? t.lo : v > t.hi ? t.hi : v);
    }
    *out = c;
    return LSD_OK;
}

void lsd_destroy(lsd_ctx* c) {
    if (!c) return;
    (void)hipSetDevice(c->device);
    (void)hipDeviceSynchronize();
    for (auto& e : c->ev) if (e) (void)hipEventDestroy(e);
    if (c->ev_done) (void)hipEventDestroy(c->ev_done);
    if (c->ga_ev) (void)hipEventDestroy(c->ga_ev);
    for (int k = 0; k < 2; k++) { if (c->pin[k]) (void)hipHostFree(c->pin[k]); if (c->pin_ev[k]) (void)hipEventDestroy(c->pin_ev[k]); }
    if (c->copy_stream) (void)hipStreamDestroy(c->copy_stream);
    if (c->stream) (void)hipStreamDestroy(c->stream);
    delete c;
}

const char* lsd_last_error(const lsd_ctx* c) { return c ? c->err.c_str() : ""; }
void lsd_free(void* p) { free(p); }

int lsd_set_stop_after(lsd_ctx* c, int stage) {
    if (!c || stage < 0 || stage > LSD_STAGE_REGION) return LSD_ERR_INVALID;
    c->stop_after = stage;
    return LSD_OK;
}
int lsd_set_region_waves(lsd_ctx* c, int waves) {
    if (!c || (waves != 0 && waves != 4 && waves != 8)) return LSD_ERR_INVALID;
    c->region_waves_mode = waves;
    return LSD_OK;
}

int lsd_set_region_help(lsd_ctx* c, int waves) {
    if (!c || waves < -1 || waves > 4096) return LSD_ERR_INVALID;
    c->tun_help = waves;
    return LSD_OK;
}

int lsd_set_cost_history(lsd_ctx* c, int on) {
    if (!c) return LSD_ERR_INVALID;
    c->cost_history = on != 0;
    return LSD_OK;
}

int lsd_debug_set_tuning(lsd_ctx* c, const char* name, int value) {
    if (!c || !name) return LSD_ERR_INVALID;
    for (const Tuning& t : kTunings)
        if (strcmp(name, t.name) == 0) {
            c->*(t.field) = value < t.lo ? t.lo : value > t.hi ? t.hi : value;
            return LSD_OK;
        }
    return LSD_ERR_INVALID;
}

int lsd_debug_set_stamp_budget(lsd_ctx* c, unsigned grows) {
    if (!c || grows < 2u || grows > 0xFFFF0u) return LSD_ERR_INVALID;
    c->id_budget = grows;
    return LSD_OK;
}

int lsd_set_trace(lsd_ctx* c, int on) {
    if (!c) return LSD_ERR_INVALID;
    c->trace = on != 0;
    return LSD_OK;
}

int lsd_reserve(lsd_ctx* c, int n, int cols, int rows) {
    if (!c || n <= 0) return LSD_ERR_INVALID;
    lsd_params p; lsd_default_params(&p);
    Geom g;
    int st = make_geom(c, &p, cols, rows, &g);
    if (st != LSD_OK) return st;
    HIPCHK(c, hipSetDevice(c->device));
    st = ensure_workspace(c, (size_t)n, (size_t)g.npx, (size_t)g.gp * g.h, c->ws.cap_max_lines, c->trace);
    if (st != LSD_OK) return st;
    return ensure_tables(c, &p, g, nullptr);
}

int lsd_enqueue_batch_device(lsd_ctx* c, uint8_t* d_maps, int n, int cols, int rows, const lsd_params* p,
                             unsigned flags, uint8_t* d_line_ims, lsd_line* d_lines, int max_lines, int32_t* d_counts,
                             void* stream) {
    if (!c || !d_maps || n <= 0 || !d_lines || !d_counts || max_lines <= 0) return LSD_ERR_INVALID;
    Geom g;
    int st = make_geom(c, p, cols, rows, &g);
    if (st != LSD_OK) return st;
    HIPCHK(c, hipSetDevice(c->device));
    hipStream_t s = (hipStream_t)stream;
    st = ensure_workspace(c, (size_t)n, (size_t)g.npx, (size_t)g.gp * g.h, max_lines, c->trace);
    if (st != LSD_OK) return st;
    st = ensure_tables(c, p, g, s);
    if (st != LSD_OK) return st;
    HIPCHK(c, prepare_gauss(g));
    if (c->done_valid && c->last_stream != s) HIPCHK(c, hipStreamWaitEvent(s, c->ev_done, 0));

    Workspace& w = c->ws;
    Buffers b{};
    b.in = d_maps;
    b.in_rw = (flags & LSD_FLAG_WRITEBACK_MAP) ? d_maps : nullptr;
    b.gauss = w.gauss.get(); b.mag = w.mag.get(); b.deg = w.deg.get(); b.sc = w.sc.get(); b.pw = w.pw.get(); b.epochmap = w.epochmap.get(); b.sets = w.sets.get(); b.maxbits = w.maxbits.get(); b.nb = w.nb.get(); b.ties = w.ties();
    b.ord = w.ord.get(); b.spill = w.spill.get(); b.gcopy = w.gcopy.get(); b.wmeta = w.wmeta.get(); b.mcap = c->mcap; b.stamps = w.stamps.get(); b.seedidx = w.seedidx.get(); b.seedpos = w.seedpos.get(); b.tepoch = w.tepoch.get();
    b.tm_stride = 4 * ((g.w + 7) >> 3) * ((g.h + 7) >> 3);
    b.order = w.order.get(); b.slist = w.slist.get(); b.gcap = c->gcap; b.id_budget = c->id_budget; b.pend = w.pend.get(); b.rnum = w.rnum.get();
    b.recs = w.recs.get(); b.recs_scaled = w.recs_scaled.get(); b.counts = d_counts; b.lines = d_lines; b.line_im = d_line_ims;
    b.max_lines = max_lines;
    {
        const int nw = waves_for(c, n);
        b.tun_soft = c->tun_soft > 0 ? c->tun_soft : 48 * nw;
        b.tun_claim = c->tun_claim > 0 ? c->tun_claim : 192 * nw;
        b.tun_feed = c->tun_feed;
        b.tun_big = c->tun_big > 0 ? c->tun_big : 3;
        b.tun_help = c->tun_help >= 0 ? c->tun_help : 0;
        b.tun_early = c->tun_early; b.tun_wb = c->tun_wb; b.tun_gate = c->tun_gate; b.tun_share = c->tun_share; b.tun_up = c->tun_up; b.tun_down = c->tun_down; b.tun_requeue = c->tun_requeue;
        b.tun_xpoll = c->tun_xpoll; b.tun_linger = c->tun_linger; b.tun_stop = c->tun_stop;
        b.xq = (b.tun_help > 0 && !c->trace) ? w.xq.get() : nullptr;
        b.npool = b.xq ? pool_for(c, n) : 0;
    }
    b.taps = c->d_taps.get(); b.centres = c->d_centres.get(); b.lgamma = c->d_lgamma.get(); b.lg_count = (int)c->d_lgamma.capacity(); b.ptab = c->d_ptab.get();
    b.seeds = c->trace ? w.seeds.get() : nullptr; b.nseed = w.nseed.get(); b.stats = w.stats.get();

    HIPCHK(c, hipMemsetAsync(w.maxbits.get(), 0, sizeof(unsigned long long) * w.cap_n + sizeof(int32_t) * (size_t)n, s));
    const bool full_region = c->stop_after == 0 || c->stop_after >= LSD_STAGE_REGION;
    if (!full_region) HIPCHK(c, hipMemsetAsync(d_counts, 0, sizeof(int32_t) * n, s));
    if (c->stop_after != 0 && c->stop_after < LSD_STAGE_SORT) HIPCHK(c, hipMemsetAsync(w.nb.get(), 0, sizeof(int32_t) * (size_t)n, s));

    HIPCHK(c, hipEventRecord(c->ev[0], s));
    const bool fused_clear = d_line_ims && (((size_t)cols * rows) & 15) == 0 && (reinterpret_cast<uintptr_t>(d_line_ims) & 15) == 0;
    if (d_line_ims && !fused_clear) launch_clear(d_line_ims, (size_t)n * cols * rows, c->num_cus, s);
    launch_gauss(g, b, n, fused_clear ? d_line_ims : nullptr, s);
    if (b.in_rw) launch_remap_writeback(g, b, n, s);
    HIPCHK(c, hipEventRecord(c->ev[1], s));
    if (c->stop_after == 0 || c->stop_after >= LSD_STAGE_GRAD) launch_gradient(g, b, n, s);
    HIPCHK(c, hipEventRecord(c->ev[2], s));
    if (c->stop_after == 0 || c->stop_after >= LSD_STAGE_SORT) { launch_sort(g, b, n, s); launch_order(b, n, g.npx, (c->cost_history && c->hist_n == n && !c->trace) ? w.stats.get() : nullptr, s); }
    HIPCHK(c, hipEventRecord(c->ev[3], s));
    hipStream_t sr = s;
    if (c->stop_after == 0 || c->stop_after >= LSD_STAGE_REGION) {
        if (++w.run_id >= 1023u) {
            HIPCHK(c, hipMemsetAsync(w.stamps.get(), 0, w.cap_ws * tm_words(w.cap_npx) * sizeof(uint32_t), sr));
            HIPCHK(c, hipMemsetAsync(w.epochmap.get(), 0, w.cap_n * w.cap_npx * sizeof(uint32_t), sr));
            w.run_id = 1;
        }
        if (b.xq) HIPCHK(c, hipMemsetAsync(b.xq, 0, sizeof(uint32_t) * ((size_t)n * (kXStride + 1) + kXHdr), sr));
        const bool wide = waves_for(c, n) == 8;
        int grid = n;
        const int groups = c->tun_groups >= 0 ? c->tun_groups : c->num_cus;
        if (wide && groups > 0 && groups < n && !b.xq && !c->trace) {
            if (!c->pcount.get()) HIPCHK(c, c->pcount.resize(16));
            HIPCHK(c, hipMemsetAsync(c->pcount.get(), 0, sizeof(int), sr));
            b.pcount = c->pcount.get(); b.nimg = n; b.npool = 0;
            grid = groups;
        }
        if (wide) launch_region_w8(g, b, grid, w.run_id << 20, sr);
        else launch_region_w4(g, b, grid, w.run_id << 20, sr);
    }
    HIPCHK(c, hipEventRecord(c->ev[4], s));
    if (c->stop_after == 0) launch_lines(g, b, n, s);
    HIPCHK(c, hipEventRecord(c->ev[5], s));
    HIPCHK(c, hipEventRecord(c->ev_done, s));
    c->done_valid = true; c->done_stream = s;
    HIPCHK(c, hipGetLastError());
    c->ev_valid = true;
    c->hist_n = (c->stop_after == 0 || c->stop_after >= LSD_STAGE_REGION) ? n : 0;
    c->geom = g; c->last_n = n; c->last_max_lines = max_lines; c->last_counts = d_counts; c->last_stream = s;
    return LSD_OK;
}

int lsd_synchronize(lsd_ctx* c) {
    if (!c) return LSD_ERR_INVALID;
    HIPCHK(c, hipSetDevice(c->device));
    HIPCHK(c, hipStreamSynchronize(c->last_stream));
    return LSD_OK;
}

int lsd_last_timings(lsd_ctx* c, float ms[6]) {
    if (!c || !ms || !c->ev_valid) return LSD_ERR_INVALID;
    HIPCHK(c, hipSetDevice(c->device));
    HIPCHK(c, hipEventSynchronize(c->ev[5]));
    for (int i = 0; i < 5; i++) HIPCHK(c, hipEventElapsedTime(&ms[i], c->ev[i], c->ev[i + 1]));
    HIPCHK(c, hipEventElapsedTime(&ms[5], c->ev[0], c->ev[5]));
    return LSD_OK;
}

static int h2d_staged(lsd_ctx* c, void* dst, const void* src, size_t bytes, hipStream_t s) {
    size_t off = 0;
    for (int k = 0; off < bytes; k++) {
        const int b = k & 1;
        const size_t len = bytes - off < kPinBytes ? bytes - off : kPinBytes;
        if (c->pin_used[b]) HIPCHK(c, hipEventSynchronize(c->pin_ev[b]));
        memcpy(c->pin[b], (const uint8_t*)src + off, len);
        HIPCHK(c, hipMemcpyAsync((uint8_t*)dst + off, c->pin[b], len, hipMemcpyHostToDevice, s));
        HIPCHK(c, hipEventRecord(c->pin_ev[b], s));
        c->pin_used[b] = true;
        off += len;
    }
    return LSD_OK;
}
static int d2h_staged(lsd_ctx* c, void* dst, const void* src, size_t bytes, hipStream_t s) {
    size_t off = 0, prev_off = 0, prev_len = 0;
    for (int k = 0; off < bytes; k++) {
        const int b = k & 1;
        const size_t len = bytes - off < kPinBytes ? bytes - off : kPinBytes;
        if (c->pin_used[b] && k < 2) HIPCHK(c, hipEventSynchronize(c->pin_ev[b]));
        HIPCHK(c, hipMemcpyAsync(c->pin[b], (const uint8_t*)src + off, len, hipMemcpyDeviceToHost, s));
        HIPCHK(c, hipEventRecord(c->pin_ev[b], s));
        c->pin_used[b] = true;
        if (prev_len) {
            HIPCHK(c, hipEventSynchronize(c->pin_ev[b ^ 1]));
            memcpy((uint8_t*)dst + prev_off, c->pin[b ^ 1], prev_len);
        }
        prev_off = off; prev_len = len;
        off += len;
        if (off >= bytes) {
            HIPCHK(c, hipEventSynchronize(c->pin_ev[b]));
            memcpy((uint8_t*)dst + prev_off, c->pin[b], prev_len);
        }
    }
    return LSD_OK;
}

static int ensure_host_staging(lsd_ctx* c, size_t n, size_t wh, int max_lines, bool lineim) {
    if (n > c->hcap_n || wh > c->hcap_wh || max_lines > c->hcap_max_lines || (lineim && !c->hcap_lineim)) {
        const size_t nn = n > c->hcap_n ? n : c->hcap_n, ww = wh > c->hcap_wh ? wh : c->hcap_wh;
        const int ml = max_lines > c->hcap_max_lines ? max_lines : c->hcap_max_lines;
        const bool li = lineim || c->hcap_lineim;
        c->hcap_n = 0; c->hcap_wh = 0; c->hcap_max_lines = 0; c->hcap_lineim = false;
        HIPCHK(c, hipDeviceSynchronize());
        HIPCHK(c, c->h_in.resize(nn * ww));
        HIPCHK(c, c->h_lineim.resize(li ? nn * ww : 0));
        HIPCHK(c, c->h_lines.resize(nn * (size_t)ml)); HIPCHK(c, c->h_flat.resize(nn * (size_t)ml));
        HIPCHK(c, c->h_counts.resize(nn)); HIPCHK(c, c->h_offs.resize(nn + 3));
        c->hcap_n = nn; c->hcap_wh = ww; c->hcap_max_lines = ml; c->hcap_lineim = li;
    }
    return LSD_OK;
}

int lsd_run_batch(lsd_ctx* c, uint8_t* maps, int n, int cols, int rows, const lsd_params* p, uint8_t* line_ims,
                  lsd_line** lines_out, int* offsets_out) {
    if (!c || !maps || n <= 0 || !lines_out || !offsets_out) return LSD_ERR_INVALID;
    *lines_out = nullptr;
    Geom g;
    int st = make_geom(c, p, cols, rows, &g);
    if (st != LSD_OK) return st;
    HIPCHK(c, hipSetDevice(c->device));
    const size_t wh = (size_t)cols * rows;
    const int ml = c->host_max_lines;
    if ((long long)n * ml >= (1ll << 31) / 10) return LSD_ERR_UNSUPPORTED;
    st = ensure_host_staging(c, (size_t)n, wh, ml, line_ims != nullptr);
    if (st != LSD_OK) return st;
    hipStream_t s = c->stream;
    st = h2d_staged(c, c->h_in.get(), maps, (size_t)n * wh, s);
    if (st != LSD_OK) return st;
    st = lsd_enqueue_batch_device(c, c->h_in.get(), n, cols, rows, p, LSD_FLAG_WRITEBACK_MAP, line_ims ? c->h_lineim.get() : nullptr,
                                  c->h_lines.get(), ml, c->h_counts.get(), s);
    if (st != LSD_OK) return st;
    launch_compact_lines(c->h_lines.get(), c->h_counts.get(), ml, n, c->h_flat.get(), c->h_offs.get(), s);
    HIPCHK(c, hipStreamWaitEvent(c->copy_stream, c->ev[1], 0));
    st = d2h_staged(c, maps, c->h_in.get(), (size_t)n * wh, c->copy_stream);
    if (st != LSD_OK) return st;
    std::vector<int32_t> offs((size_t)n + 3);
    st = d2h_staged(c, offs.data(), c->h_offs.get(), sizeof(int32_t) * (size_t)(n + 3), s);
    if (st != LSD_OK) return st;
    memcpy(offsets_out, offs.data(), sizeof(int32_t) * (size_t)(n + 1));
    const int total = offsets_out[n];
    lsd_line* out = (lsd_line*)calloc(total > 0 ? total : 1, sizeof(lsd_line));
    if (!out) return LSD_ERR_NOMEM;
    st = total > 0 ? d2h_staged(c, out, c->h_flat.get(), sizeof(lsd_line) * (size_t)total, s) : LSD_OK;
    if (st == LSD_OK && line_ims) st = d2h_staged(c, line_ims, c->h_lineim.get(), (size_t)n * wh, s);
    if (st != LSD_OK) { free(out); return st; }
    *lines_out = out;
    if (offs[(size_t)n + 2] > 0) {
        c->err = "region stage gave up image " + std::to_string(offs[(size_t)n + 2] - 1) + " of the batch (watchdog; counts = -1)";
        return LSD_ERR_INTERNAL;
    }
    return offs[(size_t)n + 1] > 0 ? LSD_ERR_CAPACITY : LSD_OK;
}

int lsd_set_host_max_lines(lsd_ctx* c, int max_lines) {
    if (!c || max_lines < 1 || max_lines > (1 << 20)) return LSD_ERR_INVALID;
    c->host_max_lines = max_lines;
    return LSD_OK;
}

int lsd_run(lsd_ctx* c, uint8_t* map, int cols, int rows, size_t stride, const lsd_params* p, uint8_t* line_im,
            size_t line_im_stride, lsd_line** lines_out, int* n_lines) {
    if (!c || !map || !lines_out || !n_lines || cols <= 0 || rows <= 0) return LSD_ERR_INVALID;
    if (stride < (size_t)cols || (line_im && line_im_stride < (size_t)cols)) return LSD_ERR_INVALID;
    *n_lines = 0;
    const bool packed = stride == (size_t)cols && (!line_im || line_im_stride == (size_t)cols);
    int offs[2] = {0, 0};
    if (packed) {
        int st = lsd_run_batch(c, map, 1, cols, rows, p, line_im, lines_out, offs);
        *n_lines = offs[1];
        return st;
    }
    std::vector<uint8_t> tmp((size_t)cols * rows), tim(line_im ? (size_t)cols * rows : 0);
    for (int y = 0; y < rows; y++) memcpy(&tmp[(size_t)y * cols], map + (size_t)y * stride, cols);
    int st = lsd_run_batch(c, tmp.data(), 1, cols, rows, p, line_im ? tim.data() : nullptr, lines_out, offs);
    for (int y = 0; y < rows; y++) memcpy(map + (size_t)y * stride, &tmp[(size_t)y * cols], cols);
    if (line_im)
        for (int y = 0; y < rows; y++) memcpy(line_im + (size_t)y * line_im_stride, &tim[(size_t)y * cols], cols);
    *n_lines = offs[1];
    return st;
}

int lsd_last_region_cycles(lsd_ctx* c, int n, long long* cycles_out) {
    if (!c || !cycles_out || n <= 0 || n > c->last_n || n > c->hist_n) return LSD_ERR_INVALID;
    HIPCHK(c, hipSetDevice(c->device));
    HIPCHK(c, hipStreamSynchronize(c->last_stream));
    HIPCHK(c, hipMemcpy2D(cycles_out, sizeof(long long), c->ws.stats.get() + kStatTotalWord, sizeof(long long) * kStatWords, sizeof(long long), (size_t)n,
                          hipMemcpyDeviceToHost));
    return LSD_OK;
}

int lsd_last_sensitivity(lsd_ctx* c, int n, int* near_ties) {
    if (!c || !near_ties || n <= 0 || n > c->last_n || n > c->hist_n) return LSD_ERR_INVALID;
    HIPCHK(c, hipSetDevice(c->device));
    HIPCHK(c, hipStreamSynchronize(c->last_stream));
    std::vector<long long> reg((size_t)n);
    std::vector<int32_t> grad((size_t)n);
    HIPCHK(c, hipMemcpy2D(reg.data(), sizeof(long long), c->ws.stats.get() + kStatTiesWord, sizeof(long long) * kStatWords, sizeof(long long), (size_t)n,
                          hipMemcpyDeviceToHost));
    HIPCHK(c, hipMemcpy(grad.data(), c->ws.ties(), sizeof(int32_t) * (size_t)n, hipMemcpyDeviceToHost));
    for (int i = 0; i < n; i++) {
        const long long v = reg[(size_t)i] + grad[(size_t)i];
        near_ties[i] = v > 0x7fffffffll ? 0x7fffffff : (int)v;
    }
    return LSD_OK;
}

int lsd_debug_fetch(lsd_ctx* c, int image, int what, void* out, size_t bytes) {
    if (!c || !out || image < 0 || image >= c->last_n) return LSD_ERR_INVALID;
    HIPCHK(c, hipSetDevice(c->device));
    HIPCHK(c, hipStreamSynchronize(c->last_stream));
    const Workspace& w = c->ws;
    const size_t npx = (size_t)c->geom.npx, off = (size_t)image * npx;
    const void* src = nullptr;
    size_t need = 0;
    int32_t nbv = 0, cnt = 0, nseed = 0;
    switch (what) {
        case LSD_DBG_GAUSS:
            if (bytes < npx * 8) return LSD_ERR_INVALID;
            HIPCHK(c, hipMemcpy2D(out, (size_t)c->geom.w * 8, w.gauss.get() + (size_t)image * c->geom.gp * c->geom.h, (size_t)c->geom.gp * 8,
                                  (size_t)c->geom.w * 8, (size_t)c->geom.h, hipMemcpyDeviceToHost));
            return LSD_OK;
        case LSD_DBG_MAG: src = w.mag.get() + off; need = npx * 8; break;
        case LSD_DBG_DEG: src = w.deg.get() + off; need = npx * 8; break;
        case LSD_DBG_STATE: src = w.pw.get() + off; need = npx * 4; break;
        case LSD_DBG_ORDER:
        case LSD_DBG_ORDER_VAL:
            HIPCHK(c, hipMemcpy(&nbv, w.nb.get() + image, 4, hipMemcpyDeviceToHost));
            if (what == LSD_DBG_ORDER) { src = w.ord.get() + off; need = (size_t)nbv * 4; }
            else {
                if (bytes < (size_t)nbv * 2) return LSD_ERR_INVALID;
                DevBuf<uint16_t> tmp;
                HIPCHK(c, tmp.resize((size_t)(nbv > 0 ? nbv : 1)));
                launch_ordv(w.mag.get() + off, w.maxbits.get() + image, w.ord.get() + off, tmp.get(), nbv, c->geom.pseBin, c->last_stream);
                HIPCHK(c, hipStreamSynchronize(c->last_stream));
                if (nbv > 0) HIPCHK(c, hipMemcpy(out, tmp.get(), (size_t)nbv * 2, hipMemcpyDeviceToHost));
                return LSD_OK;
            }
            break;
        case LSD_DBG_NB: src = w.nb.get() + image; need = 4; break;
        case LSD_DBG_MAXGRAD: src = w.maxbits.get() + image; need = 8; break;
        case LSD_DBG_RECS:
            HIPCHK(c, hipMemcpy(&cnt, c->last_counts + image, 4, hipMemcpyDeviceToHost));
            if (cnt > c->last_max_lines) cnt = c->last_max_lines;
            src = w.recs.get() + (size_t)image * c->last_max_lines * 12; need = (size_t)cnt * 12 * 8;
            break;
        case LSD_DBG_NSEED: src = w.nseed.get() + image; need = 4; break;
        case LSD_DBG_SEEDS:
            if (!w.seeds.get()) return LSD_ERR_INVALID;
            HIPCHK(c, hipMemcpy(&nseed, w.nseed.get() + image, 4, hipMemcpyDeviceToHost));
            src = w.seeds.get() + off; need = (size_t)nseed * sizeof(SeedRec);
            break;
        case LSD_DBG_STATS:
            src = w.stats.get() + (size_t)image * kStatWords; need = 8 * kStatWords;
            if (bytes > need) { const size_t all = (size_t)(c->last_n - image) * need; need = bytes < all ? bytes / need * need : all; }
            break;
        default: return LSD_ERR_INVALID;
    }
    if (bytes < need) return LSD_ERR_INVALID;
    if (need) HIPCHK(c, hipMemcpy(out, src, need, hipMemcpyDeviceToHost));
    if (what == LSD_DBG_STATE) {
        uint32_t* o = static_cast<uint32_t*>(out);
        for (size_t i = 0; i < npx; i++) o[i] = pw_used(o[i]);
    }
    return LSD_OK;
}

static int reserve_map_cache(lsd_ctx* c, size_t n, size_t cells) {
    const size_t need = n * cells;
    HIPCHK(c, c->mc_claim.reserve(need)); HIPCHK(c, c->mc_fa.reserve(need * 2)); HIPCHK(c, c->mc_fb.reserve(need * 2));
    HIPCHK(c, c->mc_ctl.reserve(n * (2 + 64)));
    return LSD_OK;
}

int lsd_enqueue_map_cache_device(lsd_ctx* c, const uint8_t* d_maps, int n, int cols, int rows, double res,
                                 double z_occ_max_dis, double* d_out, void* stream) {
    if (!c || !d_maps || !d_out || n <= 0 || cols <= 0 || rows <= 0 || !(res > 0) || !(z_occ_max_dis >= 0)) return LSD_ERR_INVALID;
    if ((long long)cols * rows >= (1ll << 31)) return LSD_ERR_UNSUPPORTED;
    HIPCHK(c, hipSetDevice(c->device));
    hipStream_t s = (hipStream_t)stream;
    const int rs = reserve_map_cache(c, (size_t)n, (size_t)cols * rows);
    if (rs != LSD_OK) return rs;
    const int cell_radius = cvt_x86(floor(z_occ_max_dis / res));
    int G = (2 * c->num_cus) / n;
    if (G > 64) G = 64;
    if (G >= 4)
        launch_mapcache_spread(d_maps, d_out, c->mc_claim.get(), c->mc_fa.get(), c->mc_fb.get(), c->mc_ctl.get(), c->mc_ctl.get() + 2 * (size_t)n, n, G, cols, rows, res,
                               z_occ_max_dis, cell_radius, s);
    else
        launch_mapcache(d_maps, d_out, c->mc_claim.get(), c->mc_fa.get(), c->mc_fb.get(), n, cols, rows, res, z_occ_max_dis, cell_radius, s);
    HIPCHK(c, hipGetLastError());
    c->last_stream = s;
    return LSD_OK;
}

int lsd_map_cache(lsd_ctx* c, const uint8_t* map, int cols, int rows, size_t stride, double res, double z_occ_max_dis,
                  double* out) {
    if (!c || !map || !out || cols <= 0 || rows <= 0 || stride < (size_t)cols) return LSD_ERR_INVALID;
    HIPCHK(c, hipSetDevice(c->device));
    const size_t wh = (size_t)cols * rows;
    HIPCHK(c, c->mc_in.reserve(wh)); HIPCHK(c, c->mc_out.reserve(wh));
    int st;
    if (stride == (size_t)cols) { st = h2d_staged(c, c->mc_in.get(), map, wh, c->stream); if (st != LSD_OK) return st; }
    else HIPCHK(c, hipMemcpy2DAsync(c->mc_in.get(), cols, map, stride, cols, rows, hipMemcpyHostToDevice, c->stream));
    st = lsd_enqueue_map_cache_device(c, c->mc_in.get(), 1, cols, rows, res, z_occ_max_dis, c->mc_out.get(), c->stream);
    if (st != LSD_OK) return st;
    return d2h_staged(c, out, c->mc_out.get(), wh * sizeof(double), c->stream);
}

int lsd_enqueue_occupancy_to_map_device(lsd_ctx* c, const int8_t* d_grid, size_t n_cells, uint8_t* d_map, void* stream) {
    if (!c || !d_grid || !d_map || n_cells == 0) return LSD_ERR_INVALID;
    if ((reinterpret_cast<uintptr_t>(d_grid) | reinterpret_cast<uintptr_t>(d_map)) & 15u) return LSD_ERR_INVALID;
    HIPCHK(c, hipSetDevice(c->device));
    hipStream_t s = (hipStream_t)stream;
    launch_occ_to_map(reinterpret_cast<const uint8_t*>(d_grid), d_map, n_cells, s);
    HIPCHK(c, hipGetLastError());
    c->last_stream = s;
    return LSD_OK;
}

int lsd_occupancy_to_map(lsd_ctx* c, const int8_t* grid, int cols, int rows, uint8_t* map_out, size_t map_stride) {
    if (!c || !grid || !map_out || cols <= 0 || rows <= 0 || map_stride < (size_t)cols) return LSD_ERR_INVALID;
    HIPCHK(c, hipSetDevice(c->device));
    const size_t wh = (size_t)cols * rows;
    HIPCHK(c, c->oc_in.reserve(wh)); HIPCHK(c, c->oc_out.reserve(wh));
    HIPCHK(c, hipMemcpyAsync(c->oc_in.get(), grid, wh, hipMemcpyHostToDevice, c->stream));
    const int st = lsd_enqueue_occupancy_to_map_device(c, reinterpret_cast<const int8_t*>(c->oc_in.get()), wh, c->oc_out.get(), c->stream);
    if (st != LSD_OK) return st;
    HIPCHK(c, hipMemcpy2DAsync(map_out, map_stride, c->oc_out.get(), cols, cols, rows, hipMemcpyDeviceToHost, c->stream));
    HIPCHK(c, hipStreamSynchronize(c->stream));
    return LSD_OK;
}

int lsd_reserve_map_update(lsd_ctx* c, int cols, int rows) {
    if (!c || cols <= 0 || rows <= 0) return LSD_ERR_INVALID;
    if ((long long)cols * rows >= (1ll << 31)) return LSD_ERR_UNSUPPORTED;
    int st = lsd_reserve(c, 1, cols, rows);
    if (st != LSD_OK) return st;
    Geom g;
    lsd_params p; lsd_default_params(&p);
    st = make_geom(c, &p, cols, rows, &g);
    if (st != LSD_OK) return st;
    st = ensure_workspace(c, 1, (size_t)g.npx, (size_t)g.gp * g.h, std::max(c->ws.cap_max_lines, c->host_max_lines), c->trace);
    if (st != LSD_OK) return st;
    return reserve_map_cache(c, 1, (size_t)cols * rows);
}

int lsd_enqueue_map_update_device(lsd_ctx* c, const int8_t* d_grid, int cols, int rows, double res, double z_occ_max_dis, const lsd_params* p,
                                  uint8_t* d_map, double* d_map_cache, lsd_line* d_lines, int max_lines, int32_t* d_count, uint8_t* d_line_im,
                                  void* stream) {
    if (!c || !d_grid || !d_map || !d_map_cache || !d_lines || !d_count || max_lines <= 0 || cols <= 0 || rows <= 0 || !(res > 0) ||
        !(z_occ_max_dis >= 0))
        return LSD_ERR_INVALID;
    if ((reinterpret_cast<uintptr_t>(d_grid) | reinterpret_cast<uintptr_t>(d_map)) & 15u) {
        c->err = "map update: d_grid and d_map must be 16-byte aligned";
        return LSD_ERR_INVALID;
    }
    if ((long long)cols * rows >= (1ll << 31)) return LSD_ERR_UNSUPPORTED;
    Geom g;
    int st = make_geom(c, p, cols, rows, &g);
    if (st != LSD_OK) return st;
    HIPCHK(c, hipSetDevice(c->device));
    hipStream_t s = (hipStream_t)stream;
    if (c->done_valid && c->done_stream != s) HIPCHK(c, hipStreamWaitEvent(s, c->ev_done, 0));
    const size_t cells = (size_t)cols * rows;
    st = lsd_enqueue_occupancy_to_map_device(c, d_grid, cells, d_map, s);
    if (st != LSD_OK) return st;
    st = lsd_enqueue_map_cache_device(c, d_map, 1, cols, rows, res, z_occ_max_dis, d_map_cache, s);
    if (st != LSD_OK) return st;
    return lsd_enqueue_batch_device(c, d_map, 1, cols, rows, p, LSD_FLAG_WRITEBACK_MAP, d_line_im, d_lines, max_lines, d_count, s);
}

int lsd_enqueue_scan_to_map_match_device(lsd_ctx* c, const double* d_map_cache, int cols, int rows, const lsd_line* d_map_lines,
                                         const lsd_line* d_scan_lines, const lsd_position* d_pts, int n_points,
                                         lsd_position lidar, lsd_position last, const int* d_pairs, int n_pairs,
                                         double z_occ_max_dis, double max_esti_dist, lsd_match_score* d_out, void* stream) {
    if (!c || !d_map_cache || !d_map_lines || !d_scan_lines || !d_pairs || !d_out || cols <= 0 || rows <= 0 || n_pairs <= 0 ||
        n_points < 0 || (n_points > 0 && !d_pts))
        return LSD_ERR_INVALID;
    if (n_pairs > (1 << 28)) return LSD_ERR_UNSUPPORTED;
    HIPCHK(c, hipSetDevice(c->device));
    hipStream_t s = (hipStream_t)stream;
    launch_match(d_map_cache, cols, rows, d_map_lines, d_scan_lines, reinterpret_cast<const double*>(d_pts), n_points, lidar.x,
                 lidar.y, last.x, last.y, d_pairs, n_pairs, z_occ_max_dis, max_esti_dist, reinterpret_cast<double*>(d_out), s);
    HIPCHK(c, hipGetLastError());
    c->last_stream = s;
    return LSD_OK;
}

int lsd_scan_to_map_match(lsd_ctx* c, const double* map_cache, int cols, int rows, const lsd_line* map_lines, int n_map,
                          const lsd_line* scan_lines, int n_scan, const lsd_position* pts, int n_points, lsd_position lidar,
                          lsd_position last, const int* pairs, int n_pairs, double z_occ_max_dis, double max_esti_dist,
                          lsd_match_score* out) {
    if (!c || !map_cache || !map_lines || !scan_lines || !pairs || !out || cols <= 0 || rows <= 0 || n_map <= 0 || n_scan <= 0 ||
        n_pairs <= 0 || n_points < 0 || (n_points > 0 && !pts))
        return LSD_ERR_INVALID;
    for (int p = 0; p < n_pairs; p++)
        if (pairs[2 * p] < 0 || pairs[2 * p] >= n_map || pairs[2 * p + 1] < 0 || pairs[2 * p + 1] >= n_scan) return LSD_ERR_INVALID;
    HIPCHK(c, hipSetDevice(c->device));
    const size_t n_mc = (size_t)cols * rows, n_pr = (size_t)n_pairs * 2, n_out = (size_t)n_pairs * 4;
    double* d_mc; lsd_line *d_ml, *d_sl; lsd_position* d_pt; int* d_pr; lsd_match_score* d_out;
    auto regions = [&](Carver& k) { k(d_mc, n_mc); k(d_ml, n_map); k(d_sl, n_scan); k(d_pt, n_points); k(d_pr, n_pr); k(d_out, n_out); };
    HIPCHK(c, carve(c->stage, regions));
    HIPCHK(c, hipMemcpyAsync(d_mc, map_cache, n_mc * sizeof(double), hipMemcpyHostToDevice, c->stream));
    HIPCHK(c, hipMemcpyAsync(d_ml, map_lines, (size_t)n_map * sizeof(lsd_line), hipMemcpyHostToDevice, c->stream));
    HIPCHK(c, hipMemcpyAsync(d_sl, scan_lines, (size_t)n_scan * sizeof(lsd_line), hipMemcpyHostToDevice, c->stream));
    if (n_points > 0) HIPCHK(c, hipMemcpyAsync(d_pt, pts, (size_t)n_points * sizeof(lsd_position), hipMemcpyHostToDevice, c->stream));
    HIPCHK(c, hipMemcpyAsync(d_pr, pairs, n_pr * sizeof(int), hipMemcpyHostToDevice, c->stream));
    const int st = lsd_enqueue_scan_to_map_match_device(c, d_mc, cols, rows, d_ml, d_sl, d_pt, n_points, lidar, last, d_pr, n_pairs,
                                                        z_occ_max_dis, max_esti_dist, d_out, c->stream);
    if (st != LSD_OK) return st;
    HIPCHK(c, hipMemcpyAsync(out, d_out, n_out * sizeof(lsd_match_score), hipMemcpyDeviceToHost, c->stream));
    HIPCHK(c, hipStreamSynchronize(c->stream));
    return LSD_OK;
}

int lsd_enqueue_feature_scan_batch_device(lsd_ctx* c, const lsd_polar* d_scans, const int* d_lens, int n_scans, int stride,
                                          lsd_map_param mp, int region_point_limit, double thre_line, double line_dist_thre_m,
                                          lsd_line* d_lines_out, int* d_n_lines, lsd_position* d_pts_out, int pts_cap, int* d_n_pts,
                                          double* d_lidar_pos, int* d_im_size, void* stream) {
    if (!c || !d_scans || !d_lens || n_scans <= 0 || stride <= 0 || !d_lines_out || !d_n_lines || !d_n_pts || !d_lidar_pos || !d_im_size ||
        pts_cap < 0 || (pts_cap > 0 && !d_pts_out) || !(mp.mapResol > 0))
        return LSD_ERR_INVALID;
    if (stride > rdp_max_len()) return LSD_ERR_UNSUPPORTED;
    HIPCHK(c, hipSetDevice(c->device));
    hipStream_t s = (hipStream_t)stream;
    launch_rdp(reinterpret_cast<const double*>(d_scans), d_lens, n_scans, stride, mp.oriMapCol, mp.oriMapRow, mp.mapResol, mp.mapOriX, mp.mapOriY,
               region_point_limit, thre_line, line_dist_thre_m, d_lines_out, d_n_lines, reinterpret_cast<double*>(d_pts_out), pts_cap, d_n_pts,
               d_lidar_pos, d_im_size, s);
    HIPCHK(c, hipGetLastError());
    c->last_stream = s;
    return LSD_OK;
}

static_assert(sizeof(lsd_map_ref) == 64 && offsetof(lsd_map_ref, d_map_cache) == 0 && offsetof(lsd_map_ref, d_map_lines) == 8 &&
              offsetof(lsd_map_ref, d_n_map) == 16 && offsetof(lsd_map_ref, cols) == 24 && offsetof(lsd_map_ref, rows) == 28 &&
              offsetof(lsd_map_ref, n_map) == 32 && offsetof(lsd_map_ref, mapResol) == 40 && offsetof(lsd_map_ref, mapOriX) == 48 &&
              offsetof(lsd_map_ref, mapOriY) == 56,
              "lsd_map_ref has the layout the Python mirror (MAP_REF_DTYPE) assumes");

static int map_table_check(const lsd_map_ref* maps, int n_maps, const int32_t* d_map_of, int* max_n_map) {
    if (!maps || n_maps <= 0 || !d_map_of) return LSD_ERR_INVALID;
    if (n_maps > LSD_MAX_MAPS) return LSD_ERR_UNSUPPORTED;
    int mx = 0;
    for (int i = 0; i < n_maps; i++) {
        const lsd_map_ref& m = maps[i];
        if (!m.d_map_cache || m.cols <= 0 || m.rows <= 0 || m.n_map < 0 || (m.n_map > 0 && !m.d_map_lines) || !(m.mapResol > 0))
            return LSD_ERR_INVALID;
        mx = std::max(mx, m.n_map);
    }
    if (max_n_map) *max_n_map = mx;
    return LSD_OK;
}

static int map_table_upload(lsd_ctx* c, int half, const lsd_map_ref* maps, int n_maps, hipStream_t s, const lsd_map_ref** d_tab) {
    HIPCHK(c, c->map_tab.reserve(2 * LSD_MAX_MAPS));
    lsd_map_ref* h = c->map_tab_host.data() + (size_t)half * LSD_MAX_MAPS;
    lsd_map_ref* d = c->map_tab.get() + (size_t)half * LSD_MAX_MAPS;
    std::copy(maps, maps + n_maps, h);
    HIPCHK(c, hipMemcpyAsync(d, h, sizeof(lsd_map_ref) * (size_t)n_maps, hipMemcpyHostToDevice, s));
    *d_tab = d;
    return LSD_OK;
}

int lsd_enqueue_feature_scan_maps_device(lsd_ctx* c, const lsd_polar* d_scans, const int* d_lens, int n_scans, int stride,
                                         const lsd_map_ref* maps, int n_maps, const int32_t* d_map_of, int scans_per_seq,
                                         int region_point_limit, double thre_line, double line_dist_thre_m, lsd_line* d_lines_out,
                                         int* d_n_lines, lsd_position* d_pts_out, int pts_cap, int* d_n_pts, double* d_lidar_pos,
                                         int* d_im_size, void* stream) {
    if (!c || !d_scans || !d_lens || n_scans <= 0 || stride <= 0 || !d_lines_out || !d_n_lines || !d_n_pts || !d_lidar_pos || !d_im_size ||
        pts_cap < 0 || (pts_cap > 0 && !d_pts_out) || scans_per_seq <= 0)
        return LSD_ERR_INVALID;
    const int r = map_table_check(maps, n_maps, d_map_of, nullptr);
    if (r != LSD_OK) return r;
    if (stride > rdp_max_len()) return LSD_ERR_UNSUPPORTED;
    HIPCHK(c, hipSetDevice(c->device));
    hipStream_t s = (hipStream_t)stream;
    const lsd_map_ref* d_tab;
    const int u = map_table_upload(c, 0, maps, n_maps, s, &d_tab);
    if (u != LSD_OK) return u;
    launch_rdp_maps(reinterpret_cast<const double*>(d_scans), d_lens, n_scans, stride, d_tab, n_maps, d_map_of, scans_per_seq,
                    region_point_limit, thre_line, line_dist_thre_m, d_lines_out, d_n_lines, reinterpret_cast<double*>(d_pts_out), pts_cap,
                    d_n_pts, d_lidar_pos, d_im_size, s);
    HIPCHK(c, hipGetLastError());
    c->last_stream = s;
    return LSD_OK;
}

static int enqueue_ingest(lsd_ctx* c, const lsd_polar* d_raw, const float* d_ranges, const float* d_min_inc, int n_scans, int n_beams,
                          const int* d_take, lsd_polar* d_scans, int* d_lens, int stride, void* stream) {
    if (!c || n_scans <= 0 || n_beams <= 0 || stride <= 0 || !d_scans || !d_lens || n_beams > stride) return LSD_ERR_INVALID;
    if (stride > rdp_max_len()) return LSD_ERR_UNSUPPORTED;
    if ((reinterpret_cast<uintptr_t>(d_raw) | reinterpret_cast<uintptr_t>(d_scans)) & 15) {
        c->err = "scan ingest: d_raw and d_scans must be 16-byte aligned";
        return LSD_ERR_INVALID;
    }
    HIPCHK(c, hipSetDevice(c->device));
    hipStream_t s = (hipStream_t)stream;
    launch_ingest(d_raw, d_ranges, d_min_inc, n_scans, n_beams, d_take, d_scans, d_lens, stride, s);
    HIPCHK(c, hipGetLastError());
    c->last_stream = s;
    return LSD_OK;
}

int lsd_enqueue_scan_ingest_device(lsd_ctx* c, const lsd_polar* d_raw, int n_scans, int n_beams, const int* d_take, lsd_polar* d_scans,
                                   int* d_lens, int stride, void* stream) {
    if (!d_raw) return LSD_ERR_INVALID;
    return enqueue_ingest(c, d_raw, nullptr, nullptr, n_scans, n_beams, d_take, d_scans, d_lens, stride, stream);
}

int lsd_enqueue_laserscan_ingest_device(lsd_ctx* c, const float* d_ranges, const float* d_angle_min_inc, int n_scans, int n_beams,
                                        const int* d_take, lsd_polar* d_scans, int* d_lens, int stride, void* stream) {
    if (!d_ranges || !d_angle_min_inc) return LSD_ERR_INVALID;
    return enqueue_ingest(c, nullptr, d_ranges, d_angle_min_inc, n_scans, n_beams, d_take, d_scans, d_lens, stride, stream);
}

int lsd_feature_scan_batch(lsd_ctx* c, const lsd_polar* scans, const int* lens, int n_scans, int stride, lsd_map_param mp,
                           int region_point_limit, double thre_line, double line_dist_thre_m, lsd_line* lines_out, int* n_lines,
                           lsd_position* pts_out, int pts_cap, int* n_pts, double* lidar_pos, int* im_size) {
    if (!c || !scans || !lens || n_scans <= 0 || stride <= 0 || !lines_out || !n_lines || !n_pts || !lidar_pos || !im_size || pts_cap < 0 ||
        (pts_cap > 0 && !pts_out))
        return LSD_ERR_INVALID;
    for (int i = 0; i < n_scans; i++) if (lens[i] < 0 || lens[i] > stride) return LSD_ERR_INVALID;
    HIPCHK(c, hipSetDevice(c->device));
    const size_t ns = (size_t)n_scans, b_sc = ns * stride * sizeof(lsd_polar), b_len = ns * sizeof(int), b_li = ns * LSD_RDP_MAX_LINES * sizeof(lsd_line);
    lsd_polar* d_sc; int *d_len, *d_nl, *d_np, *d_sz; lsd_line* d_li; lsd_position* d_pt; double* d_lp;
    auto regions = [&](Carver& k) {
        k(d_sc, ns * stride); k(d_len, ns); k(d_li, ns * LSD_RDP_MAX_LINES); k(d_pt, ns * pts_cap);
        k(d_nl, ns); k(d_np, ns); k(d_lp, ns * 2); k(d_sz, ns * 2);
    };
    HIPCHK(c, carve(c->stage, regions));
    HIPCHK(c, hipMemcpyAsync(d_sc, scans, b_sc, hipMemcpyHostToDevice, c->stream));
    HIPCHK(c, hipMemcpyAsync(d_len, lens, b_len, hipMemcpyHostToDevice, c->stream));
    const int st = lsd_enqueue_feature_scan_batch_device(c, d_sc, d_len, n_scans, stride, mp, region_point_limit, thre_line, line_dist_thre_m,
                                                         d_li, d_nl, d_pt, pts_cap, d_np, d_lp, d_sz, c->stream);
    if (st != LSD_OK) return st;
    HIPCHK(c, hipMemcpyAsync(lines_out, d_li, b_li, hipMemcpyDeviceToHost, c->stream));
    if (pts_cap > 0) HIPCHK(c, hipMemcpyAsync(pts_out, d_pt, ns * pts_cap * sizeof(lsd_position), hipMemcpyDeviceToHost, c->stream));
    HIPCHK(c, hipMemcpyAsync(n_lines, d_nl, b_len, hipMemcpyDeviceToHost, c->stream));
    HIPCHK(c, hipMemcpyAsync(n_pts, d_np, b_len, hipMemcpyDeviceToHost, c->stream));
    HIPCHK(c, hipMemcpyAsync(lidar_pos, d_lp, ns * 2 * sizeof(double), hipMemcpyDeviceToHost, c->stream));
    HIPCHK(c, hipMemcpyAsync(im_size, d_sz, ns * 2 * sizeof(int), hipMemcpyDeviceToHost, c->stream));
    HIPCHK(c, hipStreamSynchronize(c->stream));
    for (int i = 0; i < n_scans; i++)
        if (n_lines[i] > LSD_RDP_MAX_LINES) return LSD_ERR_CAPACITY;
    return LSD_OK;
}

int lsd_gather_lines(lsd_ctx* c, const lsd_comm* comm, const lsd_line* d_lines, const int32_t* d_counts, int n_local, int max_lines,
                     int n_total, int cap_rows, int32_t* d_counts_all, lsd_line* d_slabs_all, void* stream) {
    if (!c || !comm || !comm->all_gather || comm->world <= 0 || comm->rank < 0 || comm->rank >= comm->world || n_total <= 0 || n_local < 0 ||
        max_lines <= 0 || cap_rows <= 0 || !d_counts_all || !d_slabs_all || (n_local > 0 && (!d_lines || !d_counts)))
        return LSD_ERR_INVALID;
    int lo, hi, per;
    lsd_shard_range(n_total, comm->world, comm->rank, &lo, &hi);
    if (hi - lo != n_local) return LSD_ERR_INVALID;
    lsd_gather_layout(n_total, comm->world, &per, nullptr);
    HIPCHK(c, hipSetDevice(c->device));
    hipStream_t s = (hipStream_t)stream;
    const size_t need_cnt = (size_t)(per + 2) + (size_t)(n_local > 0 ? n_local : 1);
    HIPCHK(c, c->ga_cnt.reserve(need_cnt));
    HIPCHK(c, c->ga_slab.reserve((size_t)cap_rows));
    if (c->ga_ev_valid) HIPCHK(c, hipStreamWaitEvent(s, c->ga_ev, 0));
    HIPCHK(c, hipMemsetAsync(c->ga_slab.get(), 0, sizeof(lsd_line) * (size_t)cap_rows, s));
    launch_pack_lines(d_lines, d_counts, n_local, max_lines, per, cap_rows, c->ga_cnt.get(), c->ga_cnt.get() + (per + 2), c->ga_slab.get(), s);
    HIPCHK(c, hipGetLastError());
    if (comm->all_gather(comm->user, c->ga_cnt.get(), d_counts_all, sizeof(int32_t) * (size_t)(per + 2), s) != 0 ||
        comm->all_gather(comm->user, c->ga_slab.get(), d_slabs_all, sizeof(lsd_line) * (size_t)cap_rows, s) != 0) {
        c->err = "lsd_gather_lines: the communicator's all_gather failed";
        return LSD_ERR_HIP;
    }
    if (!c->ga_ev) HIPCHK(c, hipEventCreateWithFlags(&c->ga_ev, hipEventDisableTiming));
    HIPCHK(c, hipEventRecord(c->ga_ev, s));
    c->ga_ev_valid = true;
    c->last_stream = s;
    return LSD_OK;
}

static int fa_workspace(lsd_ctx* c, int n_seq, int pair_cap, FaArgs& a) {
    const size_t ns = (size_t)n_seq, pc = (size_t)pair_cap;
    auto regions = [&](Carver& k) {
        k(a.pairs, ns * pc * 2); k(a.n_pairs, ns); k(a.n_cand, ns); k(a.n_frames, ns);
        k(a.cand, ns * pc * 16); k(a.scratch, ns * pc * 8); k(a.ctl, ns * kFaCtl); k(a.aux, ns * kFaAux);
    };
    HIPCHK(c, carve(c->fa_buf, regions));
    a.pair_cap = pair_cap;
    a.lds_bound = c->fa_lds_bound;
    return LSD_OK;
}

void lsd_fa_initial_state(lsd_fa_state* o) {
    if (!o) return;
    memset(o, 0, sizeof(*o));
    o->x[0] = -1; o->x[1] = -1;
    const double d[9] = {100, 100, 100, 1, 1, 1, 0.1, 0.1, 0.1};
    for (int i = 0; i < 9; i++) o->P[i * 10] = d[i];
}

int lsd_feature_association(lsd_ctx* c, const double* map_cache, int cols, int rows, const lsd_line* map_lines, int n_map,
                            const lsd_line* scan_lines, int n_scan, const lsd_position* pts, int n_points, lsd_position lidar,
                            lsd_position last, lsd_position sp, const lsd_fa_state* in, lsd_fa_state* out, lsd_fa_report* report) {
    if (!c || !map_cache || cols <= 0 || rows <= 0 || n_map < 0 || n_scan < 0 || n_points < 0 || (n_map > 0 && !map_lines) ||
        (n_scan > 0 && !scan_lines) || (n_points > 0 && !pts) || !in || !out || !report)
        return LSD_ERR_INVALID;
    if ((long long)n_map * n_scan > (1 << 26)) return LSD_ERR_UNSUPPORTED;
    HIPCHK(c, hipSetDevice(c->device));
    const size_t n_mc = (size_t)cols * rows;
    double *d_mc, *d_sc;
    lsd_line *d_ml, *d_sl; lsd_position* d_pts; lsd_fa_state* d_st; lsd_fa_report* d_rep;
    auto regions = [&](Carver& k) { k(d_mc, n_mc); k(d_ml, n_map); k(d_sl, n_scan); k(d_pts, n_points); k(d_st, 2); k(d_rep, 1); k(d_sc, 8); };
    HIPCHK(c, carve(c->stage, regions));
    FaArgs a{};
    const int pair_cap = std::max(1, n_map * n_scan);
    const int r = fa_workspace(c, 1, pair_cap, a);
    if (r != LSD_OK) return r;
    const double sc[8] = {lidar.x, lidar.y, last.x, last.y, last.ang, sp.x, sp.y, sp.ang};
    hipStream_t s = c->stream;
    HIPCHK(c, hipMemcpyAsync(d_mc, map_cache, n_mc * sizeof(double), hipMemcpyHostToDevice, s));
    if (n_map) HIPCHK(c, hipMemcpyAsync(d_ml, map_lines, (size_t)n_map * sizeof(lsd_line), hipMemcpyHostToDevice, s));
    if (n_scan) HIPCHK(c, hipMemcpyAsync(d_sl, scan_lines, (size_t)n_scan * sizeof(lsd_line), hipMemcpyHostToDevice, s));
    if (n_points) HIPCHK(c, hipMemcpyAsync(d_pts, pts, (size_t)n_points * sizeof(lsd_position), hipMemcpyHostToDevice, s));
    HIPCHK(c, hipMemcpyAsync(d_st, in, sizeof(lsd_fa_state), hipMemcpyHostToDevice, s));
    HIPCHK(c, hipMemcpyAsync(d_sc, sc, sizeof(sc), hipMemcpyHostToDevice, s));
    a.map_cache = d_mc; a.cols = cols; a.rows = rows;
    a.map_lines = d_ml; a.n_map = n_map;
    a.scan_lines = d_sl; a.n_lines = nullptr; a.n_scan_given = n_scan; a.line_pitch = std::max(n_scan, 1);
    a.pts = reinterpret_cast<const double*>(d_pts); a.n_pts = nullptr; a.n_pts_given = n_points; a.pts_pitch = std::max(n_points, 1);
    a.lidar_pos = d_sc; a.given = d_sc + 2;
    a.n_frames = nullptr; a.frames_pitch = 1; a.t = 0;
    a.odom = nullptr; a.map_resol = 1;
    a.init = d_st; a.state_in = d_st; a.states = d_st + 1; a.reports = d_rep;
    launch_fa_frame(a, 1, true, s);
    HIPCHK(c, hipGetLastError());
    HIPCHK(c, hipMemcpyAsync(out, d_st + 1, sizeof(lsd_fa_state), hipMemcpyDeviceToHost, s));
    HIPCHK(c, hipMemcpyAsync(report, d_rep, sizeof(lsd_fa_report), hipMemcpyDeviceToHost, s));
    HIPCHK(c, hipStreamSynchronize(s));
    c->last_stream = s;
    return LSD_OK;
}

int lsd_debug_fa_fuse(lsd_ctx* c, const lsd_match_score* cands, int n, lsd_position last, lsd_position sp, const lsd_fa_state* in,
                      lsd_fa_state* out, lsd_fa_report* report) {
    if (!c || n < 0 || (n > 0 && !cands) || !in || !out || !report) return LSD_ERR_INVALID;
    if (n > (1 << 26)) return LSD_ERR_UNSUPPORTED;
    HIPCHK(c, hipSetDevice(c->device));
    lsd_fa_state* d_st; lsd_fa_report* d_rep;
// ... 227 lines not shown
```

### linesegmentdetector-slam_amd/csrc/lsd_internal.h

```cpp
#pragma once
#include <hip/hip_runtime.h>
#include <stdint.h>
#include "../../include/lsd_hip.h"

namespace lsdhip {

constexpr double kPi = 3.14159265358979323846;
constexpr int kCentreCount = 32768;
constexpr int kMaxTapRadius = 40;
constexpr int kLgTable = 16384;
constexpr int kLgTableMax = 1 << 23;
constexpr int kStatWords = 48;
constexpr int kStatTiesWord = 39;
constexpr int kStatTotalWord = 8;
constexpr int kPTable = 16;
constexpr int kXStride = 768, kXReq = 64, kXHdr = 16;

struct Geom {
    int W, H;
    int w, h;
    int npx;
    int gp;
    double sca;
    int tapR;
    int pseBin;
    double degThre;
    double gradThre;
    double logNT;
    double regThre;
    double aliPro;
    double denThre;
};

constexpr uint32_t kPwFree = 0u, kPwStatic = 1u, kPwRejected = 2u, kPwLine = 3u;
__host__ __device__ inline uint32_t pw_used(uint32_t w) { return (w & 3u) == 3u ? 1u : (w & 3u); }

struct Buffers {
    const uint8_t* in;
    uint8_t* in_rw;
    double* gauss;
    double* mag;
    double* deg;
    double2* sc;
    uint32_t* pw;
    uint32_t* epochmap;
    uint32_t* sets;
    uint32_t* tepoch;
    unsigned long long* maxbits;
    int32_t* nb;
    int32_t* ties;
    uint32_t* ord;
    uint32_t* stamps;
    int tm_stride;
    uint32_t* spill;
    uint32_t* gcopy;
    float4* wmeta;
    int mcap;
    int* rnum;
    uint32_t* order;
    uint32_t* seedidx;
    uint32_t* seedpos;
    uint32_t* slist;
    int gcap;
    uint32_t id_budget;
    int tun_soft, tun_claim, tun_feed, tun_big;
    uint32_t* xq;
    int tun_help;
    int* pcount;
    int nimg;
    int npool;
    int tun_early;
    int tun_wb;
    int tun_gate;
    int tun_share;
    int tun_up, tun_down;
    int tun_requeue;
    int tun_xpoll;
    int tun_linger;
    int tun_stop;
    double* pend;
    double* recs;
    double* recs_scaled;
    int32_t* counts;
    lsd_line* lines;
    uint8_t* line_im;
    int max_lines;
    const double* taps;
    const int* centres;
    const double* lgamma;
    int lg_count;
    const double* ptab;
    void* seeds;
    int32_t* nseed;
    long long* stats;
};

struct SeedRec {
    int order_idx, x, y, num, outcome, final_num;
    double logNFA;
};

hipError_t prepare_gauss(const Geom& g);
void launch_gauss(const Geom& g, const Buffers& b, int n, uint8_t* clr, hipStream_t s);
void launch_remap_writeback(const Geom& g, const Buffers& b, int n, hipStream_t s);
void launch_gradient(const Geom& g, const Buffers& b, int n, hipStream_t s);
void launch_sort(const Geom& g, const Buffers& b, int n, hipStream_t s);
void launch_ordv(const double* mag, const unsigned long long* maxbits, const uint32_t* ord, uint16_t* out, int count, int pseBin, hipStream_t s);
void launch_order(const Buffers& b, int n, int npx, const long long* hist, hipStream_t s);
void launch_region_w4(const Geom& g, const Buffers& b, int n, uint32_t id_base, hipStream_t s);
void launch_region_w8(const Geom& g, const Buffers& b, int n, uint32_t id_base, hipStream_t s);
int region_slots();
int region_waves();
int region_ring();
void launch_calib(double* buf, size_t n, hipStream_t s);
void launch_match(const double* map_cache, int cols, int rows, const lsd_line* map_lines, const lsd_line* scan_lines,
                  const double* pts, int n_points, double lidx, double lidy, double lastx, double lasty, const int* pairs,
                  int n_pairs, double zmax, double max_esti_dist, double* out, hipStream_t s);
void launch_occ_to_map(const uint8_t* in, uint8_t* out, size_t n, hipStream_t s);
void launch_mapcache_spread(const uint8_t* maps, double* out, unsigned long long* claim, uint32_t* fr_a, uint32_t* fr_b, int* ctl,
                            int* cnt, int n, int G, int W, int H, double res, double zmax, int cell_radius, hipStream_t s);
void launch_mapcache(const uint8_t* maps, double* out, unsigned long long* claim, uint32_t* fr_a, uint32_t* fr_b, int n,
                     int W, int H, double res, double zmax, int cell_radius, hipStream_t s);
void launch_lines(const Geom& g, const Buffers& b, int n, hipStream_t s);
void launch_clear(uint8_t* p, size_t bytes, int num_cus, hipStream_t s);
void launch_compact_lines(const lsd_line* lines, const int32_t* counts, int max_lines, int n, lsd_line* flat, int32_t* offsets, hipStream_t s);
void launch_rdp(const double* scans, const int* lens, int n, int stride, int oriMapCol, int oriMapRow, double mapResol, double mapOriX,
                double mapOriY, int region_point_limit, double thre_line, double line_dist_thre_m, lsd_line* lines_out, int* n_lines,
                double* pts_out, int pts_cap, int* n_pts, double* lidar_pos, int* im_size, hipStream_t s);
void launch_rdp_maps(const double* scans, const int* lens, int n, int stride, const lsd_map_ref* maps, int n_maps, const int32_t* map_of,
                     int scans_per_seq, int region_point_limit, double thre_line, double line_dist_thre_m, lsd_line* lines_out, int* n_lines,
                     double* pts_out, int pts_cap, int* n_pts, double* lidar_pos, int* im_size, hipStream_t s);
int rdp_max_len();
void launch_ingest(const lsd_polar* raw, const float* ranges, const float* min_inc, int n, int n_beams, const int* take, lsd_polar* scans,
                   int* lens, int stride, hipStream_t s);
void launch_pack_lines(const lsd_line* lines, const int32_t* counts, int n_local, int max_lines, int per, int cap_rows, int32_t* cpad,
                       int32_t* offs, lsd_line* slab, hipStream_t s);
constexpr int kFaCtl = 8, kFaAux = 4, kFaLdsMax = 1024;
struct FaArgs {
    const double* map_cache; int cols, rows;
    const lsd_line* map_lines; int n_map; const int32_t* d_n_map;
    const lsd_line* scan_lines; const int* n_lines; int n_scan_given; int line_pitch;
    const double* pts; const int* n_pts; int n_pts_given; int pts_pitch;
    const double* lidar_pos;
    const int* n_frames; int frames_pitch, t;
    const lsd_position* odom;
    lsd_fa_carry* carry;
    const double* given;
    double map_resol;
    const lsd_map_ref* maps; const int32_t* map_of; int n_maps;
    const lsd_fa_state* init; const lsd_fa_state* state_in;
    lsd_fa_state* states; lsd_fa_report* reports;
    int* pairs; int* n_pairs; int* n_cand; int pair_cap;
    double* cand; int* scratch; double* ctl; double* aux;
    int lds_bound;
};
void launch_fa_frame(const FaArgs& a, int n_seq, bool prepare, hipStream_t s);
void launch_fa_rebase(lsd_fa_carry* carry, int n_seq, const int32_t* key_of, int32_t key, double sc, double tx, double ty, hipStream_t s);
void launch_dbgmath(int fn, const double* a, const double* b, double* o0, double* o1, size_t n, hipStream_t s);

__host__ __device__ inline int cvt_x86(double v) {
    if (!(v > -2147483649.0 && v < 2147483648.0)) return (int)0x80000000;
    return (int)v;
}

}
```

Before: 67380 Mpix/s.

## Fuse Gaussian blur and gradient into a single tiled front kernel

Adds a k_front kernel that stages each tile's source window in LDS, runs the separable 17-tap Gaussian in shared memory, and computes gradient magnitude, angle, sin/cos and packed words directly. The intermediate Gaussian image is no longer written to or read from global memory, and the separate gradient launch is dropped. The fused path is on by default when the LDS footprint fits, and the debug gauss fetch recomputes the blur on demand. The cost is a halo recompute per tile and higher LDS use, which may lower occupancy.

```diff
diff --git a/include/lsd_hip.h b/include/lsd_hip.h
--- a/include/lsd_hip.h
+++ b/include/lsd_hip.h
@@ -204,6 +204,7 @@
 enum { LSD_STAGE_ALL = 0, LSD_STAGE_GAUSS = 1, LSD_STAGE_GRAD = 2, LSD_STAGE_SORT = 3, LSD_STAGE_REGION = 4 };
 int lsd_set_stop_after(lsd_ctx *ctx, int stage);
 int lsd_set_trace(lsd_ctx *ctx, int on);
+int lsd_set_fused_front(lsd_ctx *ctx, int on);
 int lsd_set_region_waves(lsd_ctx *ctx, int waves);
 int lsd_set_region_help(lsd_ctx *ctx, int waves);
 int lsd_set_cost_history(lsd_ctx *ctx, int on);
diff --git a/linesegmentdetector-slam_amd/__init__.py b/linesegmentdetector-slam_amd/__init__.py
--- a/linesegmentdetector-slam_amd/__init__.py
+++ b/linesegmentdetector-slam_amd/__init__.py
@@ -106,6 +106,7 @@
     "lsd_scaled_size": (None, [_i, _i, _dbl, _pi, _pi]),
     "lsd_set_stop_after": (_i, [_vp, _i]),
     "lsd_set_trace": (_i, [_vp, _i]),
+    "lsd_set_fused_front": (_i, [_vp, _i]),
     "lsd_set_region_waves": (_i, [_vp, _i]),
     "lsd_set_region_help": (_i, [_vp, _i]),
     "lsd_debug_set_stamp_budget": (_i, [_vp, C.c_uint]),
@@ -525,6 +526,9 @@
 
     def set_trace(self, on):
         self._chk(self.L.lsd_set_trace(self.h, 1 if on else 0))
+
+    def set_fused_front(self, on):
+        self._chk(self.L.lsd_set_fused_front(self.h, 1 if on else 0))
 
     def set_host_max_lines(self, max_lines):
         self._chk(self.L.lsd_set_host_max_lines(self.h, max_lines))
diff --git a/linesegmentdetector-slam_amd/csrc/grad_px.h b/linesegmentdetector-slam_amd/csrc/grad_px.h
--- /dev/null
+++ b/linesegmentdetector-slam_amd/csrc/grad_px.h
@@ -0,0 +1,41 @@
+#pragma once
+#include "lsd_internal.h"
+#include "devmath.h"
+
+namespace lsdhip {
+
+__device__ __forceinline__ uint32_t pack_pw(double d, uint32_t code) {
+    return (__float_as_uint(__double2float_rn(d)) & ~3u) | code;
+}
+
+struct GradPx { double m, d, gradX, gradY; uint32_t u; bool heavy; };
+__device__ __forceinline__ GradPx grad_pixel(double A, double B, double C, double D, bool interior, double gradThre) {
+    GradPx p{0, 0, 0, 0, 0u, false};
+    if (interior) {
+        p.gradX = (B + D - A - C) / 2.0;
+        p.gradY = (C + D - A - B) / 2.0;
+        p.m = sqrt(p.gradX * p.gradX + p.gradY * p.gradY);
+        if (p.m < gradThre) p.u = 1;
+        if (p.gradX == 0.0 && p.gradY == 0.0) {
+            if (signbit(-p.gradY)) p.d = signbit(p.gradX) ? -kPi : 0.0;
+            else p.d = p.gradX;
+        } else p.heavy = true;
+    }
+    return p;
+}
+
+__device__ __forceinline__ double grad_angle(double gradX, double gradY, int32_t* tie) {
+    double d;
+    if (!crm::atan2_fast(gradX, -gradY, d)) d = atan2_g(gradX, -gradY);
+    if (fabs(fabs(d - kPi) - 0.000001) <= 1e-14) atomicAdd(tie, 1);
+    if (fabs(d - kPi) < 0.000001) d = 0;
+    return d;
+}
+
+__device__ __forceinline__ double2 grad_sincos(double d) {
+    double sv, cv;
+    if (!crm::sincos_fast(d, sv, cv)) sincos_g(d, sv, cv);
+    return make_double2(sv, cv);
+}
+
+}
diff --git a/linesegmentdetector-slam_amd/csrc/k1_stage.h b/linesegmentdetector-slam_amd/csrc/k1_stage.h
--- /dev/null
+++ b/linesegmentdetector-slam_amd/csrc/k1_stage.h
@@ -0,0 +1,106 @@
+#pragma once
+#include <hip/hip_runtime.h>
+#include <stdint.h>
+
+namespace lsdhip {
+
+__device__ __forceinline__ int reflect_idx(int j, int lim) {
+    const int dou = 2 * lim;
+    while (j < 0) j += dou;
+    while (j >= dou) j -= dou;
+    if (j >= lim) j = dou - j - 1;
+    return j;
+}
+
+__device__ __forceinline__ uint32_t remap4(uint32_t x, uint32_t keep) {
+    uint32_t t1 = x ^ 0x01010101u, t2 = ~x;
+    t1 = ~(((t1 & 0x7f7f7f7fu) + 0x7f7f7f7fu) | t1 | 0x7f7f7f7fu);
+    t2 = ~(((t2 & 0x7f7f7f7fu) + 0x7f7f7f7fu) | t2 | 0x7f7f7f7fu);
+    const uint32_t m1 = (t1 | (t1 - (t1 >> 7))) & ~keep, m255 = (t2 | (t2 - (t2 >> 7))) & ~keep;
+    return (x | m1) & ~m255;
+}
+
+__device__ __forceinline__ uint32_t stage_window(const uint8_t* __restrict__ src, uint8_t* tile, int W, int H, int r0, int r1, int a0, int c1,
+                                                 int IWp, int tid, uint32_t keep_all) {
+    uint32_t wany = 0u;
+    const int IH = r1 - r0 + 1;
+    const int DW = (c1 - a0 + 4) >> 2;
+    uint32_t* tile32 = reinterpret_cast<uint32_t*>(tile);
+    const int DWp = IWp >> 2;
+    const int tx = tid & 31, ty = tid >> 5;
+    const bool plain = a0 >= 4 && a0 + 4 * DW <= W && r0 >= 1 && r1 < H && (W & 3) == 0 && (reinterpret_cast<uintptr_t>(src) & 3) == 0;
+    if (plain) {
+        const int nfull = IH >> 3, tail = IH & 7;
+        const uint8_t* const sb = src + (size_t)r0 * W + a0;
+        for (int cw = tx; cw < DW; cw += 32) {
+            const uint32_t voff = (uint32_t)ty * (uint32_t)W + 4u * (uint32_t)cw;
+            uint32_t* const t0 = tile32 + ty * DWp + cw;
+            for (int g0 = 0; g0 < nfull; g0 += 16) {
+                uint32_t v[16];
+                #pragma unroll
+                for (int j = 0; j < 16; j++) {
+                    v[j] = 0u;
+                    if (g0 + j < nfull) v[j] = *reinterpret_cast<const uint32_t*>(sb + (size_t)(g0 + j) * 8u * (size_t)W + voff);
+                }
+                #pragma unroll
+                for (int j = 0; j < 16; j++) {
+                    if (g0 + j < nfull) { const uint32_t rm = __ballot(v[j] + 1u > 1u) != 0ull ? remap4(v[j], keep_all) : (keep_all & v[j]); t0[(g0 + j) * 8 * DWp] = rm; wany |= rm; }
+                }
+            }
+            if (ty < tail) { const uint32_t rm = remap4(*reinterpret_cast<const uint32_t*>(sb + (size_t)nfull * 8u * (size_t)W + voff), keep_all); t0[nfull * 8 * DWp] = rm; wany |= rm; }
+        }
+    } else
+    for (int cw = tx; cw < DW; cw += 32) {
+        const int gx0 = a0 + 4 * cw;
+        const bool fast_col = gx0 >= 0 && gx0 + 3 < W;
+        int gxr[4];
+        uint32_t colkeep = keep_all;
+        #pragma unroll
+        for (int k2 = 0; k2 < 4; k2++) {
+            gxr[k2] = reflect_idx(gx0 + k2, W);
+            if (gxr[k2] == 0) colkeep |= 0xffu << (8 * k2);
+        }
+        for (int rb = 0; rb < IH; rb += 8 * 16) {
+            uint32_t v[16];
+            #pragma unroll
+            for (int j = 0; j < 16; j++) {
+                const int r = rb + ty + 8 * j;
+                v[j] = 0u;
+                if (r < IH) {
+                    const int gy = reflect_idx(r0 + r, H);
+                    const size_t off = (size_t)gy * W + gx0;
+                    if (fast_col && (off & 3) == 0) v[j] = *reinterpret_cast<const uint32_t*>(src + off);
+                    else {
+                        const uint8_t* row = src + (size_t)gy * W;
+                        v[j] = (uint32_t)row[gxr[0]] | ((uint32_t)row[gxr[1]] << 8) | ((uint32_t)row[gxr[2]] << 16) | ((uint32_t)row[gxr[3]] << 24);
+                    }
+                }
+            }
+            #pragma unroll
+            for (int j = 0; j < 16; j++) {
+                const int r = rb + ty + 8 * j;
+                if (r < IH) {
+                    const uint32_t x = v[j];
+                    const uint32_t rm = x != 0u ? remap4(x, reflect_idx(r0 + r, H) == 0 ? 0xffffffffu : colkeep) : 0u;
+                    tile32[r * DWp + cw] = rm; wany |= rm;
+                }
+            }
+        }
+    }
+    return wany;
+}
+
+__device__ __forceinline__ double xpass17(const uint32_t* t4, uint32_t sh, const double (&kr)[17]) {
+    const uint32_t d0 = t4[0], d1 = t4[1], d2 = t4[2], d3 = t4[3], d4 = t4[4];
+    if (__ballot((d0 | d1 | d2 | d3 | d4) != 0u) == 0ull) return 0.0;
+    uint32_t wv[5];
+    wv[0] = __builtin_amdgcn_alignbyte(d1, d0, sh); wv[1] = __builtin_amdgcn_alignbyte(d2, d1, sh);
+    wv[2] = __builtin_amdgcn_alignbyte(d3, d2, sh); wv[3] = __builtin_amdgcn_alignbyte(d4, d3, sh);
+    wv[4] = d4 >> (8u * sh);
+    double v = 0;
+    #pragma unroll
+    for (int i = 0; i < 17; i++) v += (double)(int)((wv[i >> 2] >> (8 * (i & 3))) & 0xffu) * kr[i];
+    return v;
+}
+
+}
diff --git a/linesegmentdetector-slam_amd/csrc/k_front.hip b/linesegmentdetector-slam_amd/csrc/k_front.hip
--- /dev/null
+++ b/linesegmentdetector-slam_amd/csrc/k_front.hip
@@ -0,0 +1,209 @@
+#include "lsd_internal.h"
+#include "k_front_lds.h"
+#include "k1_stage.h"
+#include "grad_px.h"
+
+namespace lsdhip {
+
+constexpr int TW = kK1TileW, TH = kK1TileH, NT = 256;
+constexpr int GW = kFrontGW, GH = kFrontGH;
+constexpr int HS = 17, TAPR = 8;
+constexpr int PPT = TW * TH / NT;
+static_assert(TW == 32 && TW * TH % NT == 0, "a thread keeps its column and walks down the tile NT / TW rows at a time");
+
+__global__ __launch_bounds__(NT, 4) void k_front(const uint8_t* __restrict__ in, double* __restrict__ mag, double* __restrict__ deg,
+                                                 double2* __restrict__ sc, uint32_t* __restrict__ pw, unsigned long long* __restrict__ maxbits,
+                                                 int32_t* __restrict__ ties, const double* __restrict__ taps_g, const int* __restrict__ centre_of,
+                                                 int W, int H, int w, int h, double gradThre, int IWp, unsigned strip_bytes, unsigned gx,
+                                                 unsigned gy, unsigned tiles, uint8_t* __restrict__ clr) {
+    extern __shared__ __align__(16) unsigned char smem[];
+    double* aux = reinterpret_cast<double*>(smem);
+    double* taps = reinterpret_cast<double*>(smem + strip_bytes);
+    uint8_t* tile = reinterpret_cast<uint8_t*>(taps + 3 * HS);
+    double* Gt = reinterpret_cast<double*>(tile);
+    int* l_cnt = reinterpret_cast<int*>(Gt + GW * GH);
+    unsigned long long* l_max = reinterpret_cast<unsigned long long*>(l_cnt + 2);
+    double2* l_g = reinterpret_cast<double2*>(smem);
+    uint32_t* l_px = reinterpret_cast<uint32_t*>(l_g + kFrontList);
+
+    const int tid = threadIdx.x;
+    const unsigned per = (tiles + 7u) >> 3;
+    const unsigned t = (blockIdx.x & 7u) * per + (blockIdx.x >> 3);
+    if (t >= tiles) return;
+    const unsigned bx = t % gx, tq = t / gx, by = tq % gy;
+    const int X0 = (int)bx * TW, Y0 = (int)by * TH;
+    const size_t img = tq / gy;
+    const uint8_t* src = in + img * (size_t)W * H;
+    const size_t base = img * (size_t)w * h;
+
+    if (clr) {
+        typedef uint32_t u32x4 __attribute__((ext_vector_type(4)));
+        const unsigned tpi = gx * gy, ti = t % tpi;
+        const size_t units = ((size_t)W * H) >> 4;
+        const size_t a = units * ti / tpi, e = units * (ti + 1) / tpi;
+        u32x4* const v = reinterpret_cast<u32x4*>(clr + img * (size_t)W * H);
+        const u32x4 z = {0u, 0u, 0u, 0u};
+        for (size_t u = a + tid; u < e; u += NT) __builtin_nontemporal_store(z, &v[u]);
+    }
+    const int Xf = max(X0 - 1, 0), Yf = max(Y0 - 1, 0);
+    const int Xl = min(X0 + TW - 1, w - 1), Yl = min(Y0 + TH - 1, h - 1);
+    const int c0 = centre_of[Xf] - TAPR, c1 = centre_of[Xl] + TAPR;
+    const int r0 = centre_of[Yf] - TAPR, r1 = centre_of[Yl] + TAPR;
+    const int IH = r1 - r0 + 1;
+
+    for (int i = tid; i < 3 * HS; i += NT) taps[i] = taps_g[i];
+
+    const int a0 = c0 - (((c0 % 4) + 4) % 4);
+    const uint32_t wany = stage_window(src, tile, W, H, r0, r1, a0, c1, IWp, tid, 0u);
+
+    const int X = tid & (TW - 1), Yt = tid / TW;
+    const int gX = X0 + X;
+    if (!__syncthreads_or((int)(wany != 0u))) {
+        if (gX < w) {
+            #pragma unroll
+            for (int k = 0; k < PPT; k++) {
+                const int gY = Y0 + Yt + k * (NT / TW);
+                if (gY >= h) break;
+                const GradPx px = grad_pixel(0.0, 0.0, 0.0, 0.0, gX >= 1 && gY >= 1, gradThre);
+                const size_t p = base + (size_t)gY * w + gX;
+                mag[p] = px.m;
+                if (!px.heavy && px.u == 0) sc[p] = make_double2(0.0, 1.0);
+                deg[p] = px.d;
+                pw[p] = pack_pw(px.d, px.u);
+            }
+        }
+        return;
+    }
+    const int DWp = IWp >> 2;
+    if (gX < w) {
+        const int cb = centre_of[gX] - TAPR - a0;
+        const double* ker = taps + (gX % 3) * HS;
+        double kr[HS];
+        #pragma unroll
+        for (int i = 0; i < HS; i++) kr[i] = ker[i];
+        const uint32_t* trow = reinterpret_cast<const uint32_t*>(tile) + (cb >> 2);
+        const uint32_t sh = (uint32_t)(cb & 3);
+        for (int r = Yt; r < IH; r += NT / TW) aux[r * GW + 1 + X] = xpass17(trow + r * DWp, sh, kr);
+    }
+    if (X0 >= 1 && tid < IH) {
+        const int cb = centre_of[X0 - 1] - TAPR - a0;
+        const double* ker = taps + ((X0 - 1) % 3) * HS;
+        double kr[HS];
+        #pragma unroll
+        for (int i = 0; i < HS; i++) kr[i] = ker[i];
+        const uint32_t* trow = reinterpret_cast<const uint32_t*>(tile) + (cb >> 2);
+        for (int r = tid; r < IH; r += NT) aux[r * GW] = xpass17(trow + r * DWp, (uint32_t)(cb & 3), kr);
+    }
+    __syncthreads();
+    if (tid == 0) *l_cnt = 0;
+
+    for (int idx = tid; idx < GW * GH; idx += NT) {
+        const int Yh = idx / GW, Xh = idx - Yh * GW;
+        const int gYh = Y0 - 1 + Yh, gXh = X0 - 1 + Xh;
+        const bool ok = gYh >= 0 && gYh < h && gXh >= 0 && gXh < w;
+        double v = 0;
+        if (ok) {
+            const int rb = centre_of[gYh] - TAPR - r0;
+            const double* ker = taps + (gYh % 3) * HS;
+            double a[HS];
+            uint32_t bits = 0u;
+            #pragma unroll
+            for (int i = 0; i < HS; i++) { a[i] = aux[(rb + i) * GW + Xh]; bits |= (uint32_t)__double2hiint(a[i]) | (uint32_t)__double2loint(a[i]); }
+            if (__ballot(bits != 0u) != 0ull) {
+                #pragma unroll
+                for (int i = 0; i < HS; i++) v += a[i] * ker[i];
+            }
+        }
+        Gt[idx] = v;
+    }
+    __syncthreads();
+
+    const int lane = tid & 63, wave = tid >> 6;
+    const unsigned long long ltmask = (1ull << lane) - 1ull;
+    double mx = 0;
+    double rowD[PPT];
+    uint32_t rowU[PPT];
+    int rowSlot[PPT];
+    #pragma unroll
+    for (int k = 0; k < PPT; k++) {
+        const int Y = Yt + k * (NT / TW), gY = Y0 + Y;
+        const bool valid = gX < w && gY < h;
+        const double* g1 = Gt + (Y + 1) * GW + X;
+        const GradPx px = grad_pixel(g1[1], g1[0], g1[1 - GW], g1[-GW], valid && gX >= 1 && gY >= 1, gradThre);
+        if (valid) {
+            const size_t p = base + (size_t)gY * w + gX;
+            mag[p] = px.m;
+            if (!px.heavy && px.u == 0) sc[p] = make_double2(0.0, 1.0);
+        }
+        rowD[k] = px.d; rowU[k] = px.u; rowSlot[k] = -1;
+        const unsigned long long hm = __ballot(px.heavy);
+        if (hm != 0ull) {
+            int b0 = 0;
+            if (lane == 0) b0 = atomicAdd(l_cnt, __builtin_popcountll(hm));
+            b0 = __builtin_amdgcn_readfirstlane(b0);
+            if (px.heavy) {
+                const int slot = b0 + __builtin_popcountll(hm & ltmask);
+                l_px[slot] = ((uint32_t)(Y * TW + X) << 1) | (px.u == 0 ? 1u : 0u);
+                l_g[slot] = make_double2(px.gradX, px.gradY);
+                rowSlot[k] = slot;
+            }
+        }
+        mx = fmax(mx, px.m);
+    }
+    {
+        unsigned long long bits = (unsigned long long)__double_as_longlong(mx);
+        for (int off = 32; off >= 1; off >>= 1) {
+            const unsigned long long o = __shfl_xor(bits, off);
+            bits = o > bits ? o : bits;
+        }
+        if (lane == 0) l_max[wave] = bits;
+    }
+    __syncthreads();
+    if (tid == 0) {
+        unsigned long long bits = l_max[0];
+        #pragma unroll
+        for (int i = 1; i < NT / 64; i++) bits = l_max[i] > bits ? l_max[i] : bits;
+        if (bits != 0ull) atomicMax(&maxbits[img], bits);
+    }
+
+    const int cnt = *l_cnt;
+    for (int i = tid; i < cnt; i += NT) {
+        const uint32_t e = l_px[i];
+        const double2 gr = l_g[i];
+        const double d = grad_angle(gr.x, gr.y, &ties[img]);
+        l_g[i] = make_double2(d, 0.0);
+        if (e & 1u) {
+            const int lt = (int)(e >> 1);
+            sc[base + (size_t)(Y0 + lt / TW) * w + (X0 + lt % TW)] = grad_sincos(d);
+        }
+    }
+    __syncthreads();
+
+    if (gX < w) {
+        #pragma unroll
+        for (int k = 0; k < PPT; k++) {
+            const int gY = Y0 + Yt + k * (NT / TW);
+            if (gY < h) {
+                const double d = rowSlot[k] >= 0 ? l_g[rowSlot[k]].x : rowD[k];
+                const size_t p = base + (size_t)gY * w + gX;
+                deg[p] = d;
+                pw[p] = pack_pw(d, rowU[k]);
+            }
+        }
+    }
+}
+
+bool front_fits(const Geom& g, size_t max_lds) {
+    if (2 * g.tapR + 1 != HS) return false;
+    const size_t need = k_front_lds(g.sca, g.tapR).bytes;
+    return need <= 64 * 1024 && need <= max_lds;
+}
+
+void launch_front(const Geom& g, const Buffers& b, int n, uint8_t* clr, hipStream_t s) {
+    const KFrontLds L = k_front_lds(g.sca, g.tapR);
+    const unsigned gx = (g.w + TW - 1) / TW, gy = (g.h + TH - 1) / TH, tiles = gx * gy * (unsigned)n;
+    hipLaunchKernelGGL(k_front, dim3(((tiles + 7u) >> 3) * 8u), dim3(NT), L.bytes, s, b.in, b.mag, b.deg, b.sc, b.pw, b.maxbits, b.ties, b.taps,
+                       b.centres, g.W, g.H, g.w, g.h, g.gradThre, L.IWp, (unsigned)L.strip, gx, gy, tiles, clr);
+}
+
+}
diff --git a/linesegmentdetector-slam_amd/csrc/k_front_lds.h b/linesegmentdetector-slam_amd/csrc/k_front_lds.h
--- /dev/null
+++ b/linesegmentdetector-slam_amd/csrc/k_front_lds.h
@@ -0,0 +1,35 @@
+#pragma once
+#include <math.h>
+#include <stddef.h>
+#include "k1_lds.h"
+
+namespace lsdhip {
+
+constexpr int kFrontGW = kK1TileW + 1, kFrontGH = kK1TileH + 1;
+constexpr int kFrontList = kK1TileW * kK1TileH;
+
+struct KFrontLds {
+    int IWp;
+    int IHmax;
+    size_t strip;
+    size_t window;
+    size_t bytes;
+};
+
+inline KFrontLds k_front_lds(double sca, int tapR) {
+    KFrontLds r;
+    const int span = (int)floor(kK1TileW / sca) + 2;
+    const int IWmax = span + 2 * tapR + 1;
+    r.IWp = ((IWmax + 3) & ~3) + 8;
+    if (((r.IWp >> 2) & 1) == 0) r.IWp += 4;
+    r.IHmax = (int)floor(kK1TileH / sca) + 2 + 2 * tapR + 1;
+    const int hSize = 2 * tapR + 1;
+    const size_t sums = (size_t)r.IHmax * kFrontGW * sizeof(double), list = (size_t)kFrontList * (16 + 4);
+    const size_t win = ((size_t)r.IHmax * r.IWp + 7) & ~(size_t)7, post = (size_t)kFrontGW * kFrontGH * sizeof(double) + 8 + 4 * 8;
+    r.strip = ((sums > list ? sums : list) + 15) & ~(size_t)15;
+    r.window = win > post ? win : post;
+    r.bytes = r.strip + 3 * (size_t)hSize * sizeof(double) + r.window;
+    return r;
+}
+
+}
diff --git a/linesegmentdetector-slam_amd/csrc/k_gauss.hip b/linesegmentdetector-slam_amd/csrc/k_gauss.hip
--- a/linesegmentdetector-slam_amd/csrc/k_gauss.hip
+++ b/linesegmentdetector-slam_amd/csrc/k_gauss.hip
@@ -1,25 +1,18 @@
 #include "lsd_internal.h"
 #include "k1_lds.h"
+#include "k1_stage.h"
 #include <algorithm>
 
 namespace lsdhip {
 
 constexpr int TW = kK1TileW, TH = kK1TileH, NT = 256;
 
-__device__ __forceinline__ int reflect_idx(int j, int lim) {
-    const int dou = 2 * lim;
-    while (j < 0) j += dou;
-    while (j >= dou) j -= dou;
-    if (j >= lim) j = dou - j - 1;
-    return j;
-}
-
 
 template <int HS>
 __global__ __launch_bounds__(NT) void k_gauss(const uint8_t* __restrict__ in, double* __restrict__ out,
                                               const double* __restrict__ taps_g, const int* __restrict__ centre_of, int W, int H, int w, int h, int gp,
                                               int tapR, int IWp, int IHmax, unsigned gx, unsigned gy, unsigned tiles,
-                                              uint8_t* __restrict__ clr) {
+                                              uint8_t* __restrict__ clr, uint32_t keep_all) {
     extern __shared__ __align__(16) unsigned char smem[];
     const int hSize = HS > 0 ? HS : 2 * tapR + 1;
     double* aux = reinterpret_cast<double*>(smem);
@@ -53,79 +46,7 @@
     for (int i = tid; i < 3 * hSize; i += NT) taps[i] = taps_g[i];
 
     const int a0 = c0 - (((c0 % 4) + 4) % 4);
-    auto remap4 = [](uint32_t x, uint32_t keep) -> uint32_t {
-        uint32_t t1 = x ^ 0x01010101u, t2 = ~x;
-        t1 = ~(((t1 & 0x7f7f7f7fu) + 0x7f7f7f7fu) | t1 | 0x7f7f7f7fu);
-        t2 = ~(((t2 & 0x7f7f7f7fu) + 0x7f7f7f7fu) | t2 | 0x7f7f7f7fu);
-        const uint32_t m1 = (t1 | (t1 - (t1 >> 7))) & ~keep, m255 = (t2 | (t2 - (t2 >> 7))) & ~keep;
-        return (x | m1) & ~m255;
-    };
-    uint32_t wany = 0u;
-    {
-        const int DW = (c1 - a0 + 4) >> 2;
-        uint32_t* tile32 = reinterpret_cast<uint32_t*>(tile);
-        const int DWp = IWp >> 2;
-        const int tx = tid & 31, ty = tid >> 5;
-        const bool plain = a0 >= 4 && a0 + 4 * DW <= W && r0 >= 1 && r1 < H && (W & 3) == 0 && (reinterpret_cast<uintptr_t>(src) & 3) == 0;
-        if (plain) {
-            const int nfull = IH >> 3, tail = IH & 7;
-            const uint8_t* const sb = src + (size_t)r0 * W + a0;
-            for (int cw = tx; cw < DW; cw += 32) {
-                const uint32_t voff = (uint32_t)ty * (uint32_t)W + 4u * (uint32_t)cw;
-                uint32_t* const t0 = tile32 + ty * DWp + cw;
-                for (int g0 = 0; g0 < nfull; g0 += 16) {
-                    uint32_t v[16];
-                    #pragma unroll
-                    for (int j = 0; j < 16; j++) {
-                        v[j] = 0u;
-                        if (g0 + j < nfull) v[j] = *reinterpret_cast<const uint32_t*>(sb + (size_t)(g0 + j) * 8u * (size_t)W + voff);
-                    }
-                    #pragma unroll
-                    for (int j = 0; j < 16; j++) {
-                        if (g0 + j < nfull) { const uint32_t rm = __ballot(v[j] + 1u > 1u) != 0ull ? remap4(v[j], 0u) : 0u; t0[(g0 + j) * 8 * DWp] = rm; wany |= rm; }
-                    }
-                }
-                if (ty < tail) { const uint32_t rm = remap4(*reinterpret_cast<const uint32_t*>(sb + (size_t)nfull * 8u * (size_t)W + voff), 0u); t0[nfull * 8 * DWp] = rm; wany |= rm; }
-            }
-        } else
-        for (int cw = tx; cw < DW; cw += 32) {
-            const int gx0 = a0 + 4 * cw;
-            const bool fast_col = gx0 >= 0 && gx0 + 3 < W;
-            int gxr[4];
-            uint32_t colkeep = 0u;
-            #pragma unroll
-            for (int k2 = 0; k2 < 4; k2++) {
-                gxr[k2] = reflect_idx(gx0 + k2, W);
-                if (gxr[k2] == 0) colkeep |= 0xffu << (8 * k2);
-            }
-            for (int rb = 0; rb < IH; rb += 8 * 16) {
-                uint32_t v[16];
-                #pragma unroll
-                for (int j = 0; j < 16; j++) {
-                    const int r = rb + ty + 8 * j;
-                    v[j] = 0u;
-                    if (r < IH) {
-                        const int gy = reflect_idx(r0 + r, H);
-                        const size_t off = (size_t)gy * W + gx0;
-                        if (fast_col && (off & 3) == 0) v[j] = *reinterpret_cast<const uint32_t*>(src + off);
-                        else {
-                            const uint8_t* row = src + (size_t)gy * W;
-                            v[j] = (uint32_t)row[gxr[0]] | ((uint32_t)row[gxr[1]] << 8) | ((uint32_t)row[gxr[2]] << 16) | ((uint32_t)row[gxr[3]] << 24);
-                        }
-                    }
-                }
-                #pragma unroll
-                for (int j = 0; j < 16; j++) {
-                    const int r = rb + ty + 8 * j;
-                    if (r < IH) {
-                        const uint32_t x = v[j];
-                        const uint32_t rm = x != 0u ? remap4(x, reflect_idx(r0 + r, H) == 0 ? 0xffffffffu : colkeep) : 0u;
-                        tile32[r * DWp + cw] = rm; wany |= rm;
-                    }
-                }
-            }
-        }
-    }
+    const uint32_t wany = stage_window(src, tile, W, H, r0, r1, a0, c1, IWp, tid, keep_all);
     const int X = tid & (TW - 1);
     const int gX = X0 + X;
     if (!__syncthreads_or((int)(wany != 0u))) {
@@ -137,28 +58,15 @@
         const int cb = (gX < w ? centre_of[gX] : 0) - tapR - a0;
         const double* ker = taps + (gX % 3) * hSize;
         if (gX < w) {
-            if (HS > 0) {
-                static_assert(HS <= 17, "the x-pass reads 5 words = 17 bytes at any byte offset");
-                double kr[HS > 0 ? HS : 1];
+            if constexpr (HS > 0) {
+                static_assert(HS == 17, "the x-pass reads 5 words = 17 bytes at any byte offset (k1_stage.h: xpass17)");
+                double kr[17];
                 #pragma unroll
                 for (int i = 0; i < HS; i++) kr[i] = ker[i];
                 const uint32_t* trow = reinterpret_cast<const uint32_t*>(tile) + (cb >> 2);
                 const uint32_t sh = (uint32_t)(cb & 3);
                 const int DWp = IWp >> 2;
-                for (int r = tid / TW; r < IH; r += NT / TW) {
-                    const uint32_t* t4 = trow + r * DWp;
-                    const uint32_t d0 = t4[0], d1 = t4[1], d2 = t4[2], d3 = t4[3], d4 = t4[4];
-                    if (__ballot((d0 | d1 | d2 | d3 | d4) != 0u) == 0ull) { aux[r * TW + X] = 0.0; continue; }
-                    uint32_t wv[5];
-                    wv[0] = __builtin_amdgcn_alignbyte(d1, d0, sh); wv[1] = __builtin_amdgcn_alignbyte(d2, d1, sh);
-                    wv[2] = __builtin_amdgcn_alignbyte(d3, d2, sh); wv[3] = __builtin_amdgcn_alignbyte(d4, d3, sh);
-                    wv[4] = d4 >> (8u * sh);
-                    double v = 0;
-                    #pragma unroll
-                    for (int i = 0; i < HS; i++) v += (double)(int)((wv[i >> 2] >> (8 * (i & 3))) & 0xffu) * kr[i];
-
-                    aux[r * TW + X] = v;
-                }
+                for (int r = tid / TW; r < IH; r += NT / TW) aux[r * TW + X] = xpass17(trow + r * DWp, sh, kr);
             } else {
                 for (int r = tid / TW; r < IH; r += NT / TW) {
                     const uint8_t* t = tile + r * IWp + cb;
@@ -195,13 +103,6 @@
     }
 }
 
-__device__ __forceinline__ uint32_t remap_word(uint32_t x, uint32_t keep) {
-    uint32_t t1 = x ^ 0x01010101u, t2 = ~x;
-    t1 = ~(((t1 & 0x7f7f7f7fu) + 0x7f7f7f7fu) | t1 | 0x7f7f7f7fu);
-    t2 = ~(((t2 & 0x7f7f7f7fu) + 0x7f7f7f7fu) | t2 | 0x7f7f7f7fu);
-    const uint32_t m1 = (t1 | (t1 - (t1 >> 7))) & ~keep, m255 = (t2 | (t2 - (t2 >> 7))) & ~keep;
-    return (x | m1) & ~m255;
-}
 __global__ __launch_bounds__(256) void k_remap_inplace16(uint8_t* __restrict__ img, uint32_t W, uint32_t H, size_t units) {
     typedef uint32_t u32x4 __attribute__((ext_vector_type(4)));
     u32x4* const v = reinterpret_cast<u32x4*>(img);
@@ -213,8 +114,8 @@
         const uint32_t row = (uint32_t)(u / upr), col = (uint32_t)(u - (size_t)row * upr);
         if (row % H == 0u) continue;
         u32x4 r;
-        r.x = remap_word(x.x, col == 0u ? 0xffu : 0u);
-        r.y = remap_word(x.y, 0u); r.z = remap_word(x.z, 0u); r.w = remap_word(x.w, 0u);
+        r.x = remap4(x.x, col == 0u ? 0xffu : 0u);
+        r.y = remap4(x.y, 0u); r.z = remap4(x.z, 0u); r.w = remap4(x.w, 0u);
         if ((r.x ^ x.x) | (r.y ^ x.y) | (r.z ^ x.z) | (r.w ^ x.w)) v[u] = r;
     }
 }
@@ -240,11 +141,11 @@
     return hipFuncSetAttribute(reinterpret_cast<const void*>(gauss_kernel(g)), hipFuncAttributeMaxDynamicSharedMemorySize, (int)L.bytes);
 }
 
-void launch_gauss(const Geom& g, const Buffers& b, int n, uint8_t* clr, hipStream_t s) {
+void launch_gauss(const Geom& g, const Buffers& b, int n, uint8_t* clr, bool remapped, hipStream_t s) {
     const K1Lds L = k1_lds(g.sca, g.tapR);
     const unsigned gx = (g.w + TW - 1) / TW, gy = (g.h + TH - 1) / TH, tiles = gx * gy * (unsigned)n;
     hipLaunchKernelGGL(gauss_kernel(g), dim3(((tiles + 7u) >> 3) * 8u), dim3(NT), L.bytes, s, b.in, b.gauss, b.taps, b.centres, g.W, g.H, g.w, g.h, g.gp,
-                       g.tapR, L.IWp, L.IHmax, gx, gy, tiles, clr);
+                       g.tapR, L.IWp, L.IHmax, gx, gy, tiles, clr, remapped ? 0xffffffffu : 0u);
 }
 
 void launch_remap_writeback(const Geom& g, const Buffers& b, int n, hipStream_t s) {
diff --git a/linesegmentdetector-slam_amd/csrc/k_grad.hip b/linesegmentdetector-slam_amd/csrc/k_grad.hip
--- a/linesegmentdetector-slam_amd/csrc/k_grad.hip
+++ b/linesegmentdetector-slam_amd/csrc/k_grad.hip
@@ -1,14 +1,10 @@
 #include "lsd_internal.h"
-#include "devmath.h"
+#include "grad_px.h"
 
 namespace lsdhip {
 
 constexpr int GX = 64;
 constexpr int GR = 8;
-
-__device__ __forceinline__ uint32_t pack_pw(double d, uint32_t code) {
-    return (__float_as_uint(__double2float_rn(d)) & ~3u) | code;
-}
 
 constexpr int CAP = 256;
 
@@ -40,17 +36,12 @@
         for (int i = lane; i < cnt; i += GX) {
             const uint32_t e = l_px[i];
             const double2 gr = l_g[i];
-            double d;
-            if (!crm::atan2_fast(gr.x, -gr.y, d)) d = atan2_g(gr.x, -gr.y);
-            if (fabs(fabs(d - kPi) - 0.000001) <= 1e-14) atomicAdd(&ties[img], 1);
-            if (fabs(d - kPi) < 0.000001) d = 0;
+            const double d = grad_angle(gr.x, gr.y, &ties[img]);
             l_g[i] = make_double2(d, 0.0);
             if (e & 1u) {
                 const int lt = (int)(e >> 1);
                 const size_t p = base + (size_t)(y0 + lt / GX) * w + ((int)bx * GX + lt % GX);
-                double sv, cv;
-                if (!crm::sincos_fast(d, sv, cv)) sincos_g(d, sv, cv);
-                sc[p] = make_double2(sv, cv);
+                sc[p] = grad_sincos(d);
             }
         }
         #pragma unroll
@@ -90,19 +81,10 @@
             if (lane != 0) B = t;
         }
         const double C = up, D = upl;
-        double m = 0, d = 0, gradX = 0, gradY = 0;
-        uint32_t u = 0;
-        bool heavy = false;
-        if (colok && x >= 1 && y >= 1) {
-            gradX = (B + D - A - C) / 2.0;
-            gradY = (C + D - A - B) / 2.0;
-            m = sqrt(gradX * gradX + gradY * gradY);
-            if (m < gradThre) u = 1;
-            if (gradX == 0.0 && gradY == 0.0) {
-                if (signbit(-gradY)) d = signbit(gradX) ? -kPi : 0.0;
-                else d = gradX;
-            } else heavy = true;
-        }
+        const GradPx px = grad_pixel(A, B, C, D, colok && x >= 1 && y >= 1, gradThre);
+        const double m = px.m, d = px.d, gradX = px.gradX, gradY = px.gradY;
+        const uint32_t u = px.u;
+        const bool heavy = px.heavy;
         if (colok) {
             const size_t p = base + (size_t)y * w + x;
             mag[p] = m;
diff --git a/linesegmentdetector-slam_amd/csrc/lsd_ctx.hip b/linesegmentdetector-slam_amd/csrc/lsd_ctx.hip
--- a/linesegmentdetector-slam_amd/csrc/lsd_ctx.hip
+++ b/linesegmentdetector-slam_amd/csrc/lsd_ctx.hip
@@ -93,11 +93,15 @@
     int tun_groups = -1;
     DevBuf<int> pcount;
     bool trace = false;
+    bool fused_front = true;
     int host_max_lines = 8192;
     Geom geom{};
     int last_n = 0;
     int last_max_lines = 0;
     int32_t* last_counts = nullptr;
+    bool last_fused = false, last_remapped = false;
+    const uint8_t* last_in = nullptr;
+    DevBuf<double> dbg_gauss;
     hipEvent_t ev[7]{};
     bool ev_valid = false;
     hipEvent_t ev_done = nullptr;
@@ -254,6 +258,11 @@
     const int now = c->tun_help < 0 ? 24 : c->tun_help;
     return pool_for(c, n, now > 24 ? now : 24);
 }
+
+static bool use_front(const lsd_ctx* c, const Geom& g) {
+    return c->fused_front && !c->trace && (c->stop_after == 0 || c->stop_after >= LSD_STAGE_GRAD) && front_fits(g, c->max_lds);
+}
+static size_t gauss_elems(const lsd_ctx* c, const Geom& g) { return use_front(c, g) ? 0 : (size_t)g.gp * g.h; }
 
 static size_t tm_words(size_t npx) { return npx / 16 + 4 * 8200; }
 
@@ -474,6 +483,12 @@
     return LSD_OK;
 }
 
+int lsd_set_fused_front(lsd_ctx* c, int on) {
+    if (!c) return LSD_ERR_INVALID;
+    c->fused_front = on != 0;
+    return LSD_OK;
+}
+
 int lsd_reserve(lsd_ctx* c, int n, int cols, int rows) {
     if (!c || n <= 0) return LSD_ERR_INVALID;
     lsd_params p; lsd_default_params(&p);
@@ -481,7 +496,7 @@
     int st = make_geom(c, &p, cols, rows, &g);
     if (st != LSD_OK) return st;
     HIPCHK(c, hipSetDevice(c->device));
-    st = ensure_workspace(c, (size_t)n, (size_t)g.npx, (size_t)g.gp * g.h, c->ws.cap_max_lines, c->trace);
+    st = ensure_workspace(c, (size_t)n, (size_t)g.npx, gauss_elems(c, g), c->ws.cap_max_lines, c->trace);
     if (st != LSD_OK) return st;
     return ensure_tables(c, &p, g, nullptr);
 }
@@ -495,11 +510,12 @@
     if (st != LSD_OK) return st;
     HIPCHK(c, hipSetDevice(c->device));
     hipStream_t s = (hipStream_t)stream;
-    st = ensure_workspace(c, (size_t)n, (size_t)g.npx, (size_t)g.gp * g.h, max_lines, c->trace);
+    st = ensure_workspace(c, (size_t)n, (size_t)g.npx, gauss_elems(c, g), max_lines, c->trace);
     if (st != LSD_OK) return st;
     st = ensure_tables(c, p, g, s);
     if (st != LSD_OK) return st;
-    HIPCHK(c, prepare_gauss(g));
+    const bool fused = use_front(c, g);
+    if (!fused) HIPCHK(c, prepare_gauss(g));
     if (c->done_valid && c->last_stream != s) HIPCHK(c, hipStreamWaitEvent(s, c->ev_done, 0));
 
     Workspace& w = c->ws;
@@ -535,10 +551,11 @@
     HIPCHK(c, hipEventRecord(c->ev[0], s));
     const bool fused_clear = d_line_ims && (((size_t)cols * rows) & 15) == 0 && (reinterpret_cast<uintptr_t>(d_line_ims) & 15) == 0;
     if (d_line_ims && !fused_clear) launch_clear(d_line_ims, (size_t)n * cols * rows, c->num_cus, s);
-    launch_gauss(g, b, n, fused_clear ? d_line_ims : nullptr, s);
+    if (fused) launch_front(g, b, n, fused_clear ? d_line_ims : nullptr, s);
+    else launch_gauss(g, b, n, fused_clear ? d_line_ims : nullptr, false, s);
     if (b.in_rw) launch_remap_writeback(g, b, n, s);
     HIPCHK(c, hipEventRecord(c->ev[1], s));
-    if (c->stop_after == 0 || c->stop_after >= LSD_STAGE_GRAD) launch_gradient(g, b, n, s);
+    if (!fused && (c->stop_after == 0 || c->stop_after >= LSD_STAGE_GRAD)) launch_gradient(g, b, n, s);
     HIPCHK(c, hipEventRecord(c->ev[2], s));
     if (c->stop_after == 0 || c->stop_after >= LSD_STAGE_SORT) { launch_sort(g, b, n, s); launch_order(b, n, g.npx, (c->cost_history && c->hist_n == n && !c->trace) ? w.stats.get() : nullptr, s); }
     HIPCHK(c, hipEventRecord(c->ev[3], s));
@@ -571,6 +588,7 @@
     c->ev_valid = true;
     c->hist_n = (c->stop_after == 0 || c->stop_after >= LSD_STAGE_REGION) ? n : 0;
     c->geom = g; c->last_n = n; c->last_max_lines = max_lines; c->last_counts = d_counts; c->last_stream = s;
+    c->last_fused = fused; c->last_in = d_maps; c->last_remapped = b.in_rw != nullptr;
     return LSD_OK;
 }
 
@@ -587,6 +605,7 @@
     HIPCHK(c, hipEventSynchronize(c->ev[5]));
     for (int i = 0; i < 5; i++) HIPCHK(c, hipEventElapsedTime(&ms[i], c->ev[i], c->ev[i + 1]));
     HIPCHK(c, hipEventElapsedTime(&ms[5], c->ev[0], c->ev[5]));
+    if (c->last_fused) ms[1] = 0.0f;
     return LSD_OK;
 }
 
@@ -749,6 +768,19 @@
     switch (what) {
         case LSD_DBG_GAUSS:
             if (bytes < npx * 8) return LSD_ERR_INVALID;
+            if (c->last_fused) {
+                const Geom& g = c->geom;
+                HIPCHK(c, c->dbg_gauss.reserve((size_t)g.gp * g.h));
+                HIPCHK(c, prepare_gauss(g));
+                Buffers b{};
+                b.in = c->last_in + (size_t)image * g.W * g.H; b.gauss = c->dbg_gauss.get();
+                b.taps = c->d_taps.get(); b.centres = c->d_centres.get();
+                launch_gauss(g, b, 1, nullptr, c->last_remapped, c->last_stream);
+                HIPCHK(c, hipGetLastError());
+                HIPCHK(c, hipStreamSynchronize(c->last_stream));
+                HIPCHK(c, hipMemcpy2D(out, (size_t)g.w * 8, c->dbg_gauss.get(), (size_t)g.gp * 8, (size_t)g.w * 8, (size_t)g.h, hipMemcpyDeviceToHost));
+                return LSD_OK;
+            }
             HIPCHK(c, hipMemcpy2D(out, (size_t)c->geom.w * 8, w.gauss.get() + (size_t)image * c->geom.gp * c->geom.h, (size_t)c->geom.gp * 8,
                                   (size_t)c->geom.w * 8, (size_t)c->geom.h, hipMemcpyDeviceToHost));
             return LSD_OK;
@@ -872,7 +904,7 @@
     lsd_params p; lsd_default_params(&p);
     st = make_geom(c, &p, cols, rows, &g);
     if (st != LSD_OK) return st;
-    st = ensure_workspace(c, 1, (size_t)g.npx, (size_t)g.gp * g.h, std::max(c->ws.cap_max_lines, c->host_max_lines), c->trace);
+    st = ensure_workspace(c, 1, (size_t)g.npx, gauss_elems(c, g), std::max(c->ws.cap_max_lines, c->host_max_lines), c->trace);
     if (st != LSD_OK) return st;
     return reserve_map_cache(c, 1, (size_t)cols * rows);
 }
diff --git a/linesegmentdetector-slam_amd/csrc/lsd_internal.h b/linesegmentdetector-slam_amd/csrc/lsd_internal.h
--- a/linesegmentdetector-slam_amd/csrc/lsd_internal.h
+++ b/linesegmentdetector-slam_amd/csrc/lsd_internal.h
@@ -101,7 +101,9 @@
 };
 
 hipError_t prepare_gauss(const Geom& g);
-void launch_gauss(const Geom& g, const Buffers& b, int n, uint8_t* clr, hipStream_t s);
+void launch_gauss(const Geom& g, const Buffers& b, int n, uint8_t* clr, bool remapped, hipStream_t s);
+bool front_fits(const Geom& g, size_t max_lds);
+void launch_front(const Geom& g, const Buffers& b, int n, uint8_t* clr, hipStream_t s);
 void launch_remap_writeback(const Geom& g, const Buffers& b, int n, hipStream_t s);
 void launch_gradient(const Geom& g, const Buffers& b, int n, hipStream_t s);
 void launch_sort(const Geom& g, const Buffers& b, int n, hipStream_t s);
```

Measured after the change: 70020 Mpix/s (median of 6 runs). 1.04x the previous value.
